# Nicholasli1995/SNVC

Hardware: AMD Instinct MI355X
Metric: stereo-pairs/sec (cost-volume build + 3D CNN fwd) (higher is better)
Workload: dtype f32 (split f16x3 operands, fp32 accumulate)

## Files before the change

snvc_amd/csrc/conv3d_f16.hip:

```cpp
#include <type_traits>

#include "common.hpp"
#include "elementwise_internal.hpp"

namespace snvc {
namespace {

typedef _Float16 h8 __attribute__((ext_vector_type(8)));
typedef float f32x16 __attribute__((ext_vector_type(16)));
typedef float f32x4 __attribute__((ext_vector_type(4)));

__device__ const unsigned g_zero16h[4] __attribute__((aligned(16))) = {0u, 0u, 0u, 0u};

struct F16Args {
    const _Float16 *x;
    const _Float16 *wp;
    const float *scale, *bias;
    const _Float16 *res;
    _Float16 *y;
    float *y_f32;
    const _Float16 *x_lo, *res_lo;
    _Float16 *y_lo;
    const float *head;
    float *y_head;
    float head_mul;
    float res_mul;
    int *overflow;
    const _Float16 *tail_w;
    float *t_out;
    float tail_mul;
    int64_t t_bs;
    const float *res_f32;
    double *stats;
    const float *x_mul;
    int CGin;
    int Cout;
    int Din, Hin, Win;
    int Dout, Hout, Wout;
    int nd, nh, nw;
    int osd, osh, osw, offd, offh, offw;
    int pad_d, pad_h, pad_w;
    int isd, ish, iod, ioh;
    int tiles_d, tiles_h, tiles_w;
    int nchunks, flags;
    int N, cls_mode;
    int64_t cls_wstride;
    int64_t x_bs, y_bs, r_bs, yf_bs;
};


template <int KD_, int KH_, int KW_, int STRIDE_, int DIL_, int MI_, int TD_, int TH_, int KCG_, int MODE_, bool DB_, int OCC_,
          int DILW_ = DIL_, int PL_ = 1, bool DYN_ = false>
struct F16Cfg {
    static constexpr bool DYN = DYN_;
    static constexpr int PL = PL_;
    static constexpr bool SPLIT = PL_ >= 2, SERIAL = PL_ == 3;
    static constexpr int RES_PL = PL_ == 2 ? 2 : 1;
    static constexpr int PASSES = SERIAL ? 2 : 1;
    static constexpr int PF = DYN_ ? 2 : (SPLIT ? 3 : 6);
    static constexpr int KD = KD_, KH = KH_, KW = KW_, STRIDE = STRIDE_, DIL = DIL_, DILW = DILW_, MI = MI_, TD = TD_, TH = TH_;
    static constexpr int KCG = KCG_, MODE = MODE_, OCC = OCC_;
    static constexpr bool DB = DB_;
    static constexpr int IN_D = (TD - 1) * STRIDE + (KD - 1) * DIL + 1;
    static constexpr int IN_H = (TH - 1) * STRIDE + (KH - 1) * DIL + 1;
    static constexpr int IN_W = 31 * STRIDE + (KW - 1) * DILW + 1;
    static constexpr int VOX = IN_D * IN_H * IN_W;
    static constexpr int GB = VOX * 16;
    static constexpr int ITEMS = RES_PL * KCG * VOX;
    static constexpr int PLANE_BYTES = KCG * GB;
    static constexpr int NIT = (ITEMS + 255) / 256;
    static constexpr int IMG_BYTES = NIT * 256 * 16;
    static constexpr int LDS_BYTES = IMG_BYTES * (DB ? 2 : 1);
    static constexpr int NB = TD * TH / 4;
    static constexpr bool UNROLL_D = KD <= 3;
    static constexpr int SEGS = UNROLL_D ? 1 : KD;
    static constexpr int TSEG = UNROLL_D ? KD * KH * KW : KH * KW;
    static constexpr int NPS = (TSEG + 1) / 2;
    static constexpr int NS = MODE == 0 ? TSEG * (KCG / 2) : NPS * KCG;
    static constexpr int STEPS = SEGS * NS;
    static constexpr int SEG_BYTES = DIL * IN_H * IN_W * 16;
    static_assert(TD * TH % 4 == 0, "rows split over 4 waves");
    static_assert(MODE == 1 || KCG % 2 == 0, "MODE 0 pairs channel groups");
    static_assert(NIT <= 32, "validity mask is one register");
    static_assert((TD * TH / 4) * 4 == TD * TH, "whole rows per wave");
    static constexpr int tapoff(int t) {
        const int kd = UNROLL_D ? t / (KH * KW) : 0, kh = (t / KW) % KH, kw = t % KW;
        return ((kd * DIL) * IN_H + kh * DIL) * IN_W + kw * DILW;
    }
};

__host__ __device__ constexpr int f16_row_channel(int i) { return 16 * ((i >> 2) & 1) + 4 * (i >> 3) + (i & 3); }

__device__ __forceinline__ int xcd_remap16(int b, int n) {
    const int q = n >> 3, r = n & 7, xcd = b & 7, k = b >> 3;
    const int base = xcd < r ? xcd * (q + 1) : r * (q + 1) + (xcd - r) * q;
    return base + k;
}

template <class Cfg, int EPI>
__global__ void __launch_bounds__(256, Cfg::OCC)
conv3d_f16_kernel(const F16Args a_) {
    F16Args a = a_;
    int cls = blockIdx.z / a.N;
    int tile_raw = blockIdx.x, tiles_launch = a.tiles_d * a.tiles_h * a.tiles_w;
    if (a.cls_mode == 1) {
        tiles_launch *= 2;
        tile_raw = xcd_remap16(blockIdx.x, tiles_launch);
        cls = (cls << 1) | (tile_raw & 1);
        tile_raw >>= 1;
        a.offd = (cls >> 2) & 1; a.offh = (cls >> 1) & 1; a.offw = cls & 1;
        a.wp += cls * a.cls_wstride;
    } else if (a.cls_mode == 2) {
        const int pd = (cls >> 1) & 1, ph = cls & 1;
        a.offd = a.iod = pd; a.offh = a.ioh = ph;
        a.nd = (a.Dout - pd + 1) / 2; a.nh = (a.Hout - ph + 1) / 2;
    }
    constexpr int S = Cfg::STRIDE, MI = Cfg::MI, TD = Cfg::TD, TH = Cfg::TH, NB = Cfg::NB, KCG = Cfg::KCG;
    constexpr int IN_H = Cfg::IN_H, IN_W = Cfg::IN_W, VOX = Cfg::VOX, GB = Cfg::GB, NIT = Cfg::NIT, ITEMS = Cfg::ITEMS;
    constexpr int PF = Cfg::PF, PL = Cfg::PL;
    constexpr bool SPLIT = Cfg::SPLIT, SERIAL = Cfg::SERIAL;
    extern __shared__ __attribute__((aligned(16))) char lds[];

    const int tid = threadIdx.x, lane = tid & 63, wave = tid >> 6, half = lane >> 5;
    const int ntiles = a.tiles_d * a.tiles_h * a.tiles_w;
    const int t = a.cls_mode == 1 ? tile_raw : xcd_remap16(blockIdx.x, ntiles);
    const int tw = t % a.tiles_w, th = (t / a.tiles_w) % a.tiles_h, td = t / (a.tiles_w * a.tiles_h);
    const int cb = blockIdx.y;
    const int64_t n = blockIdx.z % a.N;
    const int od0 = td * TD, oh0 = th * TH, ow0 = tw * 32;
    if (od0 >= a.nd || oh0 >= a.nh) return;
    const int id0 = od0 * S - a.pad_d, ih0 = oh0 * S - a.pad_h, iw0 = ow0 * S - a.pad_w;

    f32x16 acc[NB][MI];
#pragma unroll
    for (int nb = 0; nb < NB; ++nb)
#pragma unroll
        for (int m = 0; m < MI; ++m)
#pragma unroll
            for (int r = 0; r < 16; ++r) acc[nb][m][r] = 0.0f;

    const int in_hw = a.Hin * a.Win, in_dhw = in_hw * a.Din;
    unsigned off[NIT];
    unsigned vmask = 0, gmask = 0, pmask = 0;
#pragma unroll
    for (int it = 0; it < NIT; ++it) {
        const int i = it * 256 + tid;
        const int pg = i / VOX, r = i - pg * VOX;
        const int plane = pg / KCG, g = pg - plane * KCG;
        gmask |= (unsigned)(g & 1) << it;
        pmask |= (unsigned)(plane & 1) << it;
        const int dd = r / (IN_H * IN_W), r2 = r - dd * (IN_H * IN_W);
        const int hh = r2 / IN_W, ww = r2 - hh * IN_W;
        const int gd = (id0 + dd) * a.isd + a.iod, gh = (ih0 + hh) * a.ish + a.ioh, gw = iw0 + ww;
        const bool ok = i < ITEMS && (unsigned)gd < (unsigned)a.Din && (unsigned)gh < (unsigned)a.Hin &&
                        (unsigned)gw < (unsigned)a.Win;
        off[it] = ok ? (unsigned)(g * in_dhw + gd * in_hw + gh * a.Win + gw) : 0u;
        vmask |= (ok ? 1u : 0u) << it;
    }
    static_assert(KCG <= 2, "gmask holds one bit per piece");
    const _Float16 *xn = a.x + n * a.x_bs, *xn_lo = SPLIT ? a.x_lo + n * a.x_bs : nullptr;
    const int wbase = tid & ~63;
    auto issue = [&](int pass, int buf) {
        const int chunk = SERIAL ? pass >> 1 : pass;
        const bool lo_pass = SERIAL && (pass & 1);
        const int64_t coff = (int64_t)chunk * KCG * in_dhw * 8;
        const int cg_left = a.CGin - chunk * KCG;
        char *const ibuf = lds + buf * Cfg::IMG_BYTES;
#pragma unroll
        for (int it = 0; it < NIT; ++it) {
            const int i = it * 256 + tid;
            const bool ok = ((vmask >> it) & 1u) && (KCG == 1 || (int)((gmask >> it) & 1u) < cg_left);
            const _Float16 *xc = (((PL == 2 && ((pmask >> it) & 1u)) || lo_pass) ? xn_lo : xn) + coff;
            const void *src = ok ? static_cast<const void *>(xc + (size_t)off[it] * 8) : static_cast<const void *>(g_zero16h);
            if (ITEMS % 256 == 0 || i < ITEMS)
                __builtin_amdgcn_global_load_lds(static_cast<const float *>(src),
                                                 reinterpret_cast<float *>(ibuf + (it * 256 + wbase) * 16), 16, 0, 0);
        }
    };

    const int lanebase = (lane & 31) * S * 16;
    int rowoff[NB];
#pragma unroll
    for (int nb = 0; nb < NB; ++nb) {
        const int row = wave * NB + nb;
        rowoff[nb] = ((row / TH) * S * IN_H + (row % TH) * S) * IN_W * 16;
    }
    constexpr int D_SAME = Cfg::DILW;
    constexpr int D_ROW = Cfg::DIL * IN_W - (Cfg::KW - 1) * Cfg::DILW;
    constexpr int D_SLICE = Cfg::DIL * IN_H * IN_W - (Cfg::KH - 1) * Cfg::DIL * IN_W - (Cfg::KW - 1) * Cfg::DILW;
    const int b_grp = lanebase + half * GB;
    const int b_same = lanebase + half * D_SAME * 16;
    const int b_row = lanebase + half * D_ROW * 16;
    const int b_slice = lanebase + half * D_SLICE * 16;
    const int b_none = lanebase;

    constexpr int MA = MI * (SPLIT ? 2 : 1);
    int dyn_np = 0, dyn_toff[4] = {0, 0, 0, 0}, dyn_base[4] = {0, 0, 0, 0};
    if constexpr (Cfg::DYN) {
        const int nw = 1 + (cls & 1), nh = 1 + ((cls >> 1) & 1), ndp = 1 + ((cls >> 2) & 1);
        const int T = nw * nh * ndp;
// ... 238 lines not shown
                    }
                    tacc = __builtin_amdgcn_mfma_f32_32x32x16_f16(tw[m][j][1], o, tacc, 0, 0, 0);
                    tacc = __builtin_amdgcn_mfma_f32_32x32x16_f16(tw[m][j][0], ol, tacc, 0, 0, 0);
                    tacc = __builtin_amdgcn_mfma_f32_32x32x16_f16(tw[m][j][0], o, tacc, 0, 0, 0);
                }
            }
            if (okv[nb]) {
                const int64_t spc = ((int64_t)pd * a.nh + ph) * a.nw + pw_;
#pragma unroll
                for (int r = 0; r < 16; ++r) {
                    const int tap = (r & 3) + 8 * (r >> 2) + 4 * half;
                    if (tap < 27) tn[(int64_t)tap * 8 * cls_vox + spc] = tacc[r] * a.tail_mul;
                }
            }
        }
        if (vmax >= kHalfMax && a.overflow) atomicOr(a.overflow, 1);
    } else {
        const _Float16 *rn = a.res ? a.res + n * a.r_bs : nullptr;
        const _Float16 *rn_lo = (SPLIT && a.res) ? a.res_lo + n * a.r_bs : nullptr;
        constexpr bool C8OUT = EPI == 0 || EPI == 3, side = EPI == 3 && SPLIT && MI == 1;
        _Float16 *yn = C8OUT ? a.y + n * a.y_bs : nullptr;
        _Float16 *yn_lo = (C8OUT && SPLIT) ? a.y_lo + n * a.y_bs : nullptr;
        float *yf = EPI == 2 ? a.y_f32 + n * a.yf_bs : nullptr;
        const float *__restrict__ rf = (EPI == 2 && a.res_f32) ? a.res_f32 + n * a.yf_bs : nullptr;
        constexpr float kHalfMax = 65504.0f;
        const float lo_bound = relu ? 0.0f : -kHalfMax;
        float vmax = 0.0f;
        const bool want_stats = EPI == 2 && a.stats != nullptr;
        const float x_inv = (EPI == 2 && a.x_mul) ? 1.0f / a.x_mul[0] : 1.0f;
        auto run = [&](auto has_res_tag) {
            constexpr bool HAS_RES = decltype(has_res_tag)::value;
#pragma unroll
            for (int m = 0; m < MI; ++m) {
                if ((cb * MI + m) * 32 >= a.Cout) break;
                const int c0 = (cb * MI + m) * 32 + 16 * half;
                float hsum[NB];
#pragma unroll
                for (int nb = 0; nb < NB; ++nb) hsum[nb] = 0.0f;
                float st_s[2][8], st_q[2][8];
                if constexpr (EPI == 2) {
#pragma unroll
                    for (int j = 0; j < 2; ++j)
#pragma unroll
                        for (int e = 0; e < 8; ++e) st_s[j][e] = st_q[j][e] = 0.0f;
                }
#pragma unroll
                for (int j = 0; j < 2; ++j) {
                    const int cj = c0 + 8 * j;
                    f32x4 sc[2], bi[2], hw4[2];
#pragma unroll
                    for (int k = 0; k < 2; ++k) {
                        sc[k] = (a.scale ? *reinterpret_cast<const f32x4 *>(a.scale + cj + 4 * k) : f32x4(1.0f)) * x_inv;
                        bi[k] = a.scale ? *reinterpret_cast<const f32x4 *>(a.bias + cj + 4 * k) : f32x4(0.0f);
                        if constexpr (side) hw4[k] = *reinterpret_cast<const f32x4 *>(a.head + cj + 4 * k);
                    }
                    const int64_t gj = (int64_t)(cj >> 3) * out_dhw;
#pragma unroll
                    for (int nb = 0; nb < NB; ++nb) {
                        h8 rv = h8((_Float16)0.0f), rl = h8((_Float16)0.0f);
                        if constexpr (HAS_RES) {
                            rv = *reinterpret_cast<const h8 *>(rn + (gj + sp[nb]) * 8);
                            if (rn_lo) rl = *reinterpret_cast<const h8 *>(rn_lo + (gj + sp[nb]) * 8);
                        }
                        h8 o, ol;
                        float rfv[8];
                        if constexpr (EPI == 2) {
                            if (rf && okv[nb]) {
#pragma unroll
                                for (int e = 0; e < 8; ++e) rfv[e] = rf[(int64_t)(cj + e) * out_dhw + sp[nb]];
                            }
                        }
#pragma unroll
                        for (int e = 0; e < 8; ++e) {
                            float v = __builtin_fmaf(acc[nb][m][8 * j + e], sc[e >> 2][e & 3], bi[e >> 2][e & 3]);
                            if constexpr (HAS_RES) {
                                const float rr = ((float)rv[e] + (float)rl[e]) * a.res_mul;
                                if (add_pre) v += rr;
                                if (relu) v = __builtin_fmaxf(v, 0.0f);
                                if (add_post) v += rr;
                            }
                            if constexpr (EPI == 2) {
                                if constexpr (!HAS_RES) { if (relu) v = __builtin_fmaxf(v, 0.0f); }
                                if (okv[nb]) {
                                    const int64_t at = (int64_t)(cj + e) * out_dhw + sp[nb];
                                    yf[at] = rf ? __builtin_fmaf(v, a.head_mul, rfv[e]) : v * a.head_mul;
                                    if (want_stats) {
                                        const float sv = v * a.head_mul;
                                        st_s[j][e] += sv;
                                        st_q[j][e] = __builtin_fmaf(sv, sv, st_q[j][e]);
                                    }
                                }
                            } else {
                                if constexpr (SPLIT) {
                                    v = __builtin_amdgcn_fmed3f(v, HAS_RES ? -kHalfMax : lo_bound, kHalfMax);
                                    vmax = __builtin_fmaxf(vmax, okv[nb] ? __builtin_fabsf(v) : 0.0f);
                                } else if constexpr (!HAS_RES) {
                                    if (relu) v = __builtin_fmaxf(v, 0.0f);
                                }
                                if constexpr (side) hsum[nb] += hw4[e >> 2][e & 3] * v;
                                o[e] = (_Float16)v;
                                if constexpr (SPLIT) ol[e] = (_Float16)(v - (float)o[e]);
                            }
                        }
                        if constexpr (C8OUT) {
                            if (okv[nb]) {
                                *reinterpret_cast<h8 *>(yn + (gj + sp[nb]) * 8) = o;
                                if constexpr (SPLIT) *reinterpret_cast<h8 *>(yn_lo + (gj + sp[nb]) * 8) = ol;
                            }
                        }
                    }
                }
                if constexpr (EPI == 2) {
                    if (want_stats) {
                        const int zc = blockIdx.z / a.N, groups = (a.Cout + 31) >> 5;
                        const int64_t slots = (int64_t)(gridDim.z / a.N) * gridDim.x * 4;
                        const int64_t slot = ((int64_t)zc * gridDim.x + blockIdx.x) * 4 + wave;
                        double *dst = a.stats + ((((int64_t)n * slots + slot) * groups + (cb * MI + m)) * 32 + 16 * half) * 2;
#pragma unroll
                        for (int j = 0; j < 2; ++j)
#pragma unroll
                            for (int e = 0; e < 8; ++e) {
                                float s0 = st_s[j][e], s1 = st_q[j][e];
#pragma unroll
                                for (int o = 16; o >= 1; o >>= 1) {
                                    s0 += __shfl_xor(s0, o, 64);
                                    s1 += __shfl_xor(s1, o, 64);
                                }
                                if ((lane & 31) == 0) {
                                    dst[(8 * j + e) * 2] = (double)s0;
                                    dst[(8 * j + e) * 2 + 1] = (double)s1;
                                }
                            }
                    }
                }
                if constexpr (side) {
#pragma unroll
                    for (int nb = 0; nb < NB; ++nb) {
                        const float tot = hsum[nb] + __shfl_xor(hsum[nb], 32, 64);
                        if (okv[nb] && half == 0) a.y_head[n * out_dhw + sp[nb]] = tot * a.head_mul;
                    }
                }
            }
        };
        if (rn) run(std::true_type{});
        else run(std::false_type{});
        const bool clamped = vmax >= kHalfMax;
        if constexpr (C8OUT && SPLIT) {
            if (clamped && a.overflow) atomicOr(a.overflow, 1);
        }
    }
}

typedef float f32x4q __attribute__((ext_vector_type(4)));

struct X3QCfg {
    static constexpr int TD = 4, TH = 4, NB = 4, IN_D = 6, IN_H = 6, IN_W = 34, VOX = IN_D * IN_H * IN_W, GB = VOX * 16;
    static constexpr int ITEMS = 2 * VOX, PLANE_BYTES = GB, NIT = (ITEMS + 255) / 256;
    static constexpr int IMG_BYTES = NIT * 256 * 16, LDS_BYTES = 2 * IMG_BYTES;
    static constexpr int NQ = 7, PF = 2, FILL_STEP = NQ - PF;
};

template <int IMM>
__device__ __forceinline__ void lds_read_b128_to(h8 &v, unsigned addr) {
    asm volatile("ds_read_b128 %0, %1 offset:%2" : "=v"(v) : "v"(addr), "n"(IMM) : "memory");
}

template <int N>
__device__ __forceinline__ void wait_lgkm_for(h8 (&b)[8]) {
    asm volatile("s_waitcnt lgkmcnt(%8)"
                 : "+v"(b[0]), "+v"(b[1]), "+v"(b[2]), "+v"(b[3]), "+v"(b[4]), "+v"(b[5]), "+v"(b[6]), "+v"(b[7])
                 : "n"(N)
                 : "memory");
}

template <int EPI>
__global__ void __launch_bounds__(256, 2)
conv3d_x3q_kernel(const F16Args a) {
    using Cfg = X3QCfg;
    constexpr int NB = Cfg::NB, TH = Cfg::TH, IN_H = Cfg::IN_H, IN_W = Cfg::IN_W, VOX = Cfg::VOX, NIT = Cfg::NIT, NQ = Cfg::NQ;
    constexpr int ITEMS = Cfg::ITEMS, PF = Cfg::PF;
    extern __shared__ __attribute__((aligned(16))) char lds[];
    const int tid = threadIdx.x, lane = tid & 63, wave = tid >> 6, kb = lane >> 4, col = lane & 15;
    const int ntiles = a.tiles_d * a.tiles_h * a.tiles_w, cblocks = a.Cout >> 5;
    const int job = xcd_remap16(blockIdx.x, ntiles * cblocks);
    const int t = job / cblocks, cb = job - t * cblocks;
    const int tw = t % a.tiles_w, th = (t / a.tiles_w) % a.tiles_h, td = t / (a.tiles_w * a.tiles_h);
    const int64_t n = blockIdx.z;
    const int od0 = td * Cfg::TD, oh0 = th * TH, ow0 = tw * 32;
    const int id0 = od0 - a.pad_d, ih0 = oh0 - a.pad_h, iw0 = ow0 - a.pad_w;

    f32x4q acc[NB][2][2];
#pragma unroll
    for (int nb = 0; nb < NB; ++nb)
#pragma unroll
        for (int ph = 0; ph < 2; ++ph)
#pragma unroll
            for (int h = 0; h < 2; ++h) acc[nb][ph][h] = f32x4q{0.0f, 0.0f, 0.0f, 0.0f};

    const int in_hw = a.Hin * a.Win, in_dhw = in_hw * a.Din;
    unsigned off[NIT];
    unsigned vmask = 0, pmask = 0;
#pragma unroll
    for (int it = 0; it < NIT; ++it) {
        const int i = it * 256 + tid;
        const int plane = i / VOX, r = i - plane * VOX;
        pmask |= (unsigned)(plane & 1) << it;
        const int dd = r / (IN_H * IN_W), r2 = r - dd * (IN_H * IN_W);
        const int hh = r2 / IN_W, ww = r2 - hh * IN_W;
        const int gd = id0 + dd, gh = ih0 + hh, gw = iw0 + ww;
        const bool ok = i < ITEMS && (unsigned)gd < (unsigned)a.Din && (unsigned)gh < (unsigned)a.Hin && (unsigned)gw < (unsigned)a.Win;
        off[it] = ok ? (unsigned)(gd * in_hw + gh * a.Win + gw) : 0u;
        vmask |= (ok ? 1u : 0u) << it;
    }
    const _Float16 *xn = a.x + n * a.x_bs, *xn_lo = a.x_lo + n * a.x_bs;
    const int wbase = tid & ~63;
    auto issue = [&](int chunk, int buf) {
        const int64_t coff = (int64_t)chunk * in_dhw * 8;
        char *const ibuf = lds + buf * Cfg::IMG_BYTES;
#pragma unroll
        for (int it = 0; it < NIT; ++it) {
            const _Float16 *xc = (((pmask >> it) & 1u) ? xn_lo : xn) + coff;
            const void *src = ((vmask >> it) & 1u) ? static_cast<const void *>(xc + (size_t)off[it] * 8) : static_cast<const void *>(g_zero16h);
            __builtin_amdgcn_global_load_lds(static_cast<const float *>(src), reinterpret_cast<float *>(ibuf + (it * 256 + wbase) * 16), 16, 0, 0);
        }
    };
    int qoff[NQ];
#pragma unroll
    for (int q = 0; q < NQ; ++q) {
        int tp = 4 * q + kb;
        tp = tp < 27 ? tp : 26;
        qoff[q] = (((tp / 9) * IN_H + (tp / 3) % 3) * IN_W + tp % 3 + col) * 16;
    }
    int rowoff[NB];
#pragma unroll
    for (int nb = 0; nb < NB; ++nb) {
        const int row = wave * NB + nb;
        rowoff[nb] = ((row / TH) * IN_H + (row % TH)) * IN_W * 16;
    }
    const int64_t steps_total = (int64_t)a.nchunks * NQ;
    const h8 *wq = reinterpret_cast<const h8 *>(a.wp) + ((int64_t)cb * steps_total * 4) * 64 + lane;
    const int c0 = cb * 32 + 8 * kb;
    const bool has_aff = a.scale != nullptr;
    h8 q_[PF][4];
#pragma unroll
    for (int i = 0; i < PF; ++i) {
#pragma unroll
        for (int m = 0; m < 4; ++m) q_[i][m] = wq[m * 64];
        wq += 4 * 64;
    }

    const unsigned lds_base = (unsigned)(uintptr_t)(__attribute__((address_space(3))) char *)lds;
    issue(0, 0);
    __syncthreads();
    h8 epc[6];
    auto run_chunk = [&](const int chunk, auto last_tag) {
        constexpr bool LAST = decltype(last_tag)::value;
        const unsigned img = lds_base + (unsigned)((chunk & 1) * Cfg::IMG_BYTES);
        h8 bfr[2][8];
        auto load_b = [&](int buf, int hs) {
#pragma unroll
            for (int rr = 0; rr < 2; ++rr) {
                const unsigned addr = img + (unsigned)(qoff[hs >> 1] + rowoff[2 * (hs & 1) + rr]);
                lds_read_b128_to<0>(bfr[buf][rr * 4 + 0], addr);
                lds_read_b128_to<Cfg::PLANE_BYTES>(bfr[buf][rr * 4 + 1], addr);
                lds_read_b128_to<256>(bfr[buf][rr * 4 + 2], addr);
                lds_read_b128_to<Cfg::PLANE_BYTES + 256>(bfr[buf][rr * 4 + 3], addr);
            }
        };
        load_b(0, 0);
        h8 af[4];
#pragma unroll
        for (int hs = 0; hs < 2 * NQ; ++hs) {
            const int cur = hs & 1, nx = cur ^ 1;
            if ((hs & 1) == 0) {
                if (hs == 2 * Cfg::FILL_STEP) {
#pragma unroll
                    for (int i = 0; i < PF; ++i) asm volatile("" ::"v"(q_[i][0]), "v"(q_[i][1]), "v"(q_[i][2]), "v"(q_[i][3]));
                    if constexpr (!LAST) issue(chunk + 1, (chunk + 1) & 1);
                }
#pragma unroll
                for (int m = 0; m < 4; ++m) af[m] = q_[0][m];
#pragma unroll
                for (int i = 0; i + 1 < PF; ++i)
#pragma unroll
                    for (int m = 0; m < 4; ++m) q_[i][m] = q_[i + 1][m];
                if constexpr (!LAST) {
#pragma unroll
                    for (int m = 0; m < 4; ++m) q_[PF - 1][m] = wq[m * 64];
                    wq += 4 * 64;
                } else if (hs < 2 * Cfg::FILL_STEP) {
#pragma unroll
                    for (int m = 0; m < 4; ++m) q_[PF - 1][m] = wq[m * 64];
                    wq += 4 * 64;
                } else if (hs == 2 * Cfg::FILL_STEP) {
                    if (has_aff) {
#pragma unroll
                        for (int k = 0; k < 2; ++k) {
                            epc[k] = *reinterpret_cast<const h8 *>(a.scale + c0 + 4 * k);
                            epc[2 + k] = *reinterpret_cast<const h8 *>(a.bias + c0 + 4 * k);
                        }
                    }
                    if constexpr (EPI == 3) {
#pragma unroll
                        for (int k = 0; k < 2; ++k) epc[4 + k] = *reinterpret_cast<const h8 *>(a.head + c0 + 4 * k);
                    }
                }
            }
            if (hs + 1 < 2 * NQ) {
                load_b(nx, hs + 1);
                wait_lgkm_for<8>(bfr[cur]);
            } else {
                wait_lgkm_for<0>(bfr[cur]);
            }
            __builtin_amdgcn_sched_barrier(0);
#pragma unroll
            for (int term = 0; term < 3; ++term)
#pragma unroll
                for (int rr = 0; rr < 2; ++rr)
#pragma unroll
                    for (int ph = 0; ph < 2; ++ph)
#pragma unroll
                        for (int h = 0; h < 2; ++h) {
                            const h8 aw = term == 0 ? af[2 * h + 1] : af[2 * h];
                            const h8 bx = bfr[cur][rr * 4 + ph * 2 + (term == 1 ? 1 : 0)];
                            acc[2 * (hs & 1) + rr][ph][h] =
                                __builtin_amdgcn_mfma_f32_16x16x32_f16(aw, bx, acc[2 * (hs & 1) + rr][ph][h], 0, 0, 0);
                        }
            __builtin_amdgcn_sched_barrier(0);
        }
        __syncthreads();
    };
    for (int chunk = 0; chunk + 1 < a.nchunks; ++chunk) run_chunk(chunk, std::false_type{});
    run_chunk(a.nchunks - 1, std::true_type{});
    if (has_aff) asm volatile("" ::"v"(epc[0]), "v"(epc[1]), "v"(epc[2]), "v"(epc[3]));
    if constexpr (EPI == 3) asm volatile("" ::"v"(epc[4]), "v"(epc[5]));

    const int out_hw = a.Hout * a.Wout;
    const int64_t out_dhw = (int64_t)out_hw * a.Dout;
    const bool relu = (a.flags & SNVC_EPI_RELU) != 0;
    float sc[8], bi[8], hw8[8];
    const float x_inv = (EPI == 2 && a.x_mul) ? 1.0f / a.x_mul[0] : 1.0f;
#pragma unroll
    for (int e = 0; e < 8; ++e) {
        sc[e] = (has_aff ? __builtin_bit_cast(f32x4q, epc[e >> 2])[e & 3] : 1.0f) * x_inv;
        bi[e] = has_aff ? __builtin_bit_cast(f32x4q, epc[2 + (e >> 2)])[e & 3] : 0.0f;
        hw8[e] = (EPI == 3) ? __builtin_bit_cast(f32x4q, epc[4 + (e >> 2)])[e & 3] : 0.0f;
    }
    if constexpr (EPI == 2) {
        float *yf = a.y_f32 + n * a.yf_bs + (int64_t)c0 * out_dhw;
        const float *__restrict__ rf = a.res_f32 ? a.res_f32 + n * a.yf_bs + (int64_t)c0 * out_dhw : nullptr;
        const bool want_stats = a.stats != nullptr;
        float st_s[8], st_q[8];
#pragma unroll
        for (int e = 0; e < 8; ++e) st_s[e] = st_q[e] = 0.0f;
#pragma unroll
        for (int nb = 0; nb < NB; ++nb) {
            const int row = wave * NB + nb;
            const int pd = od0 + row / TH, phh = oh0 + row % TH;
#pragma unroll
            for (int ph = 0; ph < 2; ++ph) {
                const int pw = ow0 + 16 * ph + col;
                const bool ok = pd < a.nd && phh < a.nh && pw < a.nw;
                const int64_t sp = ok ? ((int64_t)pd * out_hw + phh * a.Wout + pw) : 0;
                float rfv[8];
                if (rf && ok) {
#pragma unroll
                    for (int e = 0; e < 8; ++e) rfv[e] = rf[(int64_t)e * out_dhw + sp];
                }
#pragma unroll
                for (int e = 0; e < 8; ++e) {
                    float v = __builtin_fmaf(acc[nb][ph][e >> 2][e & 3], sc[e], bi[e]);
                    if (relu) v = __builtin_fmaxf(v, 0.0f);
                    const float sv = v * a.head_mul;
                    if (ok) {
                        yf[(int64_t)e * out_dhw + sp] = rf ? sv + rfv[e] : sv;
                        if (want_stats) {
                            st_s[e] += sv;
                            st_q[e] = __builtin_fmaf(sv, sv, st_q[e]);
                        }
                    }
                }
            }
        }
        if (want_stats) {
            const int groups = a.Cout >> 5;
            double *dst = a.stats + ((((int64_t)n * ntiles * 4 + (int64_t)t * 4 + wave) * groups + cb) * 32 + 8 * kb) * 2;
#pragma unroll
            for (int e = 0; e < 8; ++e) {
                float s0 = st_s[e], s1 = st_q[e];
#pragma unroll
                for (int o = 8; o >= 1; o >>= 1) {
                    s0 += __shfl_xor(s0, o, 64);
                    s1 += __shfl_xor(s1, o, 64);
                }
                if (col == 0) {
                    dst[e * 2] = (double)s0;
                    dst[e * 2 + 1] = (double)s1;
                }
            }
        }
        return;
    }
    _Float16 *yn = a.y + n * a.y_bs + (int64_t)(cb * 4 + kb) * out_dhw * 8;
    _Float16 *yn_lo = a.y_lo + n * a.y_bs + (int64_t)(cb * 4 + kb) * out_dhw * 8;
    constexpr float kHalfMax = 65504.0f;
    const float lo_bound = relu ? 0.0f : -kHalfMax;
    float vmax = 0.0f;
#pragma unroll
    for (int nb = 0; nb < NB; ++nb) {
        const int row = wave * NB + nb;
        const int pd = od0 + row / TH, phh = oh0 + row % TH;
#pragma unroll
        for (int ph = 0; ph < 2; ++ph) {
            const int pw = ow0 + 16 * ph + col;
            const bool ok = pd < a.nd && phh < a.nh && pw < a.nw;
            const int64_t sp = ok ? ((int64_t)pd * out_hw + phh * a.Wout + pw) : 0;
            h8 o, ol;
            float hsum = 0.0f;
#pragma unroll
            for (int e = 0; e < 8; ++e) {
                float v = __builtin_fmaf(acc[nb][ph][e >> 2][e & 3], sc[e], bi[e]);
                v = __builtin_amdgcn_fmed3f(v, lo_bound, kHalfMax);
                vmax = __builtin_fmaxf(vmax, ok ? __builtin_fabsf(v) : 0.0f);
                if constexpr (EPI == 3) hsum += hw8[e] * v;
                o[e] = (_Float16)v;
                ol[e] = (_Float16)(v - (float)o[e]);
            }
            if (ok) {
                *reinterpret_cast<h8 *>(yn + sp * 8) = o;
                *reinterpret_cast<h8 *>(yn_lo + sp * 8) = ol;
            }
            if constexpr (EPI == 3) {
                float tot = hsum + __shfl_xor(hsum, 16, 64);
                tot += __shfl_xor(tot, 32, 64);
                if (ok && kb == 0) a.y_head[n * out_dhw + sp] = tot * a.head_mul;
            }
        }
    }
    if (vmax >= kHalfMax && a.overflow) atomicOr(a.overflow, 1);
}

template <int KH_, int KW_>
struct X2QCfg {
    static constexpr int KH = KH_, KW = KW_, TH = 16, NB = 4, IN_H = TH + KH - 1, IN_W = 32 + KW - 1, VOX = IN_H * IN_W, GB = VOX * 16;
    static constexpr int ITEMS = 2 * VOX, PLANE_BYTES = GB, NIT = (ITEMS + 255) / 256;
    static constexpr int IMG_BYTES = NIT * 256 * 16, LDS_BYTES = 2 * IMG_BYTES;
    static constexpr int TAPS = KH * KW, NQ = (TAPS + 3) / 4, PF = 2, FILL_STEP = NQ - PF;
    static_assert(NQ > PF, "the refill is issued PF k-steps before the chunk ends");
};

template <class Cfg>
__global__ void __launch_bounds__(256, 2)
conv2d_x3q_kernel(const F16Args a) {
    constexpr int NB = Cfg::NB, IN_W = Cfg::IN_W, VOX = Cfg::VOX, NIT = Cfg::NIT, NQ = Cfg::NQ;
    constexpr int ITEMS = Cfg::ITEMS, PF = Cfg::PF;
    extern __shared__ __attribute__((aligned(16))) char lds[];
    const int tid = threadIdx.x, lane = tid & 63, wave = tid >> 6, kb = lane >> 4, col = lane & 15;
    const int ntiles = a.tiles_h * a.tiles_w, cblocks = a.Cout >> 5;
    const int job = xcd_remap16(blockIdx.x, ntiles * cblocks);
    const int t = job / cblocks, cb = job - t * cblocks;
    const int tw = t % a.tiles_w, th = t / a.tiles_w;
    const int64_t n = blockIdx.z;
    const int oh0 = th * Cfg::TH, ow0 = tw * 32;
    const int ih0 = oh0 - a.pad_h, iw0 = ow0 - a.pad_w;

    f32x4q acc[NB][2][2];
#pragma unroll
    for (int nb = 0; nb < NB; ++nb)
#pragma unroll
        for (int ph = 0; ph < 2; ++ph)
#pragma unroll
            for (int h = 0; h < 2; ++h) acc[nb][ph][h] = f32x4q{0.0f, 0.0f, 0.0f, 0.0f};

    const int in_hw = a.Hin * a.Win;
    unsigned off[NIT];
    unsigned vmask = 0, pmask = 0;
#pragma unroll
    for (int it = 0; it < NIT; ++it) {
        const int i = it * 256 + tid;
        const int plane = i / VOX, r = i - plane * VOX;
        pmask |= (unsigned)(plane & 1) << it;
        const int hh = r / IN_W, ww = r - hh * IN_W;
        const int gh = ih0 + hh, gw = iw0 + ww;
        const bool ok = i < ITEMS && (unsigned)gh < (unsigned)a.Hin && (unsigned)gw < (unsigned)a.Win;
        off[it] = ok ? (unsigned)(gh * a.Win + gw) : 0u;
        vmask |= (ok ? 1u : 0u) << it;
    }
    const _Float16 *xn = a.x + n * a.x_bs, *xn_lo = a.x_lo + n * a.x_bs;
    const int wbase = tid & ~63;
    auto issue = [&](int chunk, int buf) {
        const int64_t coff = (int64_t)chunk * in_hw * 8;
        char *const ibuf = lds + buf * Cfg::IMG_BYTES;
#pragma unroll
        for (int it = 0; it < NIT; ++it) {
            const _Float16 *xc = (((pmask >> it) & 1u) ? xn_lo : xn) + coff;
            const void *src = ((vmask >> it) & 1u) ? static_cast<const void *>(xc + (size_t)off[it] * 8) : static_cast<const void *>(g_zero16h);
            __builtin_amdgcn_global_load_lds(static_cast<const float *>(src), reinterpret_cast<float *>(ibuf + (it * 256 + wbase) * 16), 16, 0, 0);
        }
    };
    int qoff[NQ];
#pragma unroll
    for (int q = 0; q < NQ; ++q) {
        int tp = 4 * q + kb;
        tp = tp < Cfg::TAPS ? tp : Cfg::TAPS - 1;
        qoff[q] = ((tp / Cfg::KW) * IN_W + tp % Cfg::KW + col) * 16;
    }
    int rowoff[NB];
#pragma unroll
    for (int nb = 0; nb < NB; ++nb) rowoff[nb] = (wave * NB + nb) * IN_W * 16;
    const int64_t steps_total = (int64_t)a.nchunks * NQ;
    const h8 *wq = reinterpret_cast<const h8 *>(a.wp) + ((int64_t)cb * steps_total * 4) * 64 + lane;
    h8 q_[PF][4];
#pragma unroll
    for (int i = 0; i < PF; ++i) {
#pragma unroll
        for (int m = 0; m < 4; ++m) q_[i][m] = wq[m * 64];
        wq += 4 * 64;
    }

    const unsigned lds_base = (unsigned)(uintptr_t)(__attribute__((address_space(3))) char *)lds;
    issue(0, 0);
    __syncthreads();
    for (int chunk = 0; chunk < a.nchunks; ++chunk) {
        const unsigned img = lds_base + (unsigned)((chunk & 1) * Cfg::IMG_BYTES);
        const bool more = chunk + 1 < a.nchunks;
        h8 bfr[2][8];
        auto load_b = [&](int buf, int hs) {
#pragma unroll
            for (int rr = 0; rr < 2; ++rr) {
                const unsigned addr = img + (unsigned)(qoff[hs >> 1] + rowoff[2 * (hs & 1) + rr]);
                lds_read_b128_to<0>(bfr[buf][rr * 4 + 0], addr);
                lds_read_b128_to<Cfg::PLANE_BYTES>(bfr[buf][rr * 4 + 1], addr);
                lds_read_b128_to<256>(bfr[buf][rr * 4 + 2], addr);
                lds_read_b128_to<Cfg::PLANE_BYTES + 256>(bfr[buf][rr * 4 + 3], addr);
            }
        };
        load_b(0, 0);
        h8 af[4];
#pragma unroll
        for (int hs = 0; hs < 2 * NQ; ++hs) {
            const int cur = hs & 1, nx = cur ^ 1;
            if ((hs & 1) == 0) {
                if (hs == 2 * Cfg::FILL_STEP) {
#pragma unroll
                    for (int i = 0; i < PF; ++i) asm volatile("" ::"v"(q_[i][0]), "v"(q_[i][1]), "v"(q_[i][2]), "v"(q_[i][3]));
                    if (more) issue(chunk + 1, (chunk + 1) & 1);
                }
#pragma unroll
                for (int m = 0; m < 4; ++m) af[m] = q_[0][m];
#pragma unroll
                for (int i = 0; i + 1 < PF; ++i)
#pragma unroll
                    for (int m = 0; m < 4; ++m) q_[i][m] = q_[i + 1][m];
#pragma unroll
                for (int m = 0; m < 4; ++m) q_[PF - 1][m] = wq[m * 64];
                wq += 4 * 64;
            }
            if (hs + 1 < 2 * NQ) {
                load_b(nx, hs + 1);
                wait_lgkm_for<8>(bfr[cur]);
            } else {
                wait_lgkm_for<0>(bfr[cur]);
            }
            __builtin_amdgcn_sched_barrier(0);
#pragma unroll
            for (int term = 0; term < 3; ++term)
#pragma unroll
                for (int rr = 0; rr < 2; ++rr)
#pragma unroll
                    for (int ph = 0; ph < 2; ++ph)
#pragma unroll
                        for (int h = 0; h < 2; ++h) {
                            const h8 aw = term == 0 ? af[2 * h + 1] : af[2 * h];
                            const h8 bx = bfr[cur][rr * 4 + ph * 2 + (term == 1 ? 1 : 0)];
                            acc[2 * (hs & 1) + rr][ph][h] =
                                __builtin_amdgcn_mfma_f32_16x16x32_f16(aw, bx, acc[2 * (hs & 1) + rr][ph][h], 0, 0, 0);
                        }
            __builtin_amdgcn_sched_barrier(0);
        }
        __syncthreads();
    }

    const int64_t out_hw = (int64_t)a.Hout * a.Wout;
    const bool relu = (a.flags & SNVC_EPI_RELU) != 0;
    const int c0 = cb * 32 + 8 * kb;
    const float xm = a.x_mul ? a.head_mul / a.x_mul[0] : a.head_mul;
    float sc[8], bi[8];
#pragma unroll
    for (int e = 0; e < 8; ++e) {
        sc[e] = (a.scale ? a.scale[c0 + e] : 1.0f) * xm;
        bi[e] = a.scale ? a.bias[c0 + e] : 0.0f;
    }
    float *yn = a.y_f32 + n * a.yf_bs + (int64_t)c0 * out_hw;
#pragma unroll
    for (int nb = 0; nb < NB; ++nb) {
        const int phh = oh0 + wave * NB + nb;
#pragma unroll
        for (int ph = 0; ph < 2; ++ph) {
            const int pw = ow0 + 16 * ph + col;
            if (phh < a.nh && pw < a.nw) {
                float *yp = yn + (int64_t)phh * a.Wout + pw;
#pragma unroll
                for (int e = 0; e < 8; ++e) {
                    float v = __builtin_fmaf(acc[nb][ph][e >> 2][e & 3], sc[e], bi[e]);
                    if (relu) v = __builtin_fmaxf(v, 0.0f);
                    yp[e * out_hw] = v;
                }
            }
        }
    }
}

struct X3S2Cfg {
    static constexpr int TD = 2, TH = 4, NB = 2, IN_D = 5, IN_H = 9, IN_W = 65, VOX = IN_D * IN_H * IN_W;
    static constexpr int THREADS = 512, NIT = (VOX + THREADS - 1) / THREADS, SLOT_BYTES = NIT * THREADS * 16, LDS_BYTES = 3 * SLOT_BYTES;
    static constexpr int NQ = 7;
};

template <int N>
__device__ __forceinline__ void wait_lgkm_for4(h8 (&b)[4]) {
    asm volatile("s_waitcnt lgkmcnt(%4)" : "+v"(b[0]), "+v"(b[1]), "+v"(b[2]), "+v"(b[3]) : "n"(N) : "memory");
}

__global__ void __launch_bounds__(512, 1)
conv3d_x3s2q_kernel(const F16Args a, const int total_jobs) {
    using Cfg = X3S2Cfg;
    constexpr int NB = Cfg::NB, TH = Cfg::TH, IN_H = Cfg::IN_H, IN_W = Cfg::IN_W, VOX = Cfg::VOX, NIT = Cfg::NIT, NQ = Cfg::NQ;
    extern __shared__ __attribute__((aligned(16))) char lds[];
    const int tid = threadIdx.x, lane = tid & 63, wave = (tid >> 6) & 3, chalf = tid >> 8, kb = lane >> 4, col = lane & 15;
    const int ntiles = a.tiles_d * a.tiles_h * a.tiles_w, cblocks = a.Cout >> 6;
    const int in_hw = a.Hin * a.Win, in_dhw = in_hw * a.Din;
    const int wbase = tid & ~63;

    struct Job { int od0, oh0, ow0, cb; int64_t n; };
    auto decode = [&](int b) {
        const int j = xcd_remap16(b, total_jobs);
        const int cb = j % cblocks, r = j / cblocks, t = r % ntiles;
        Job jb;
        jb.n = r / ntiles; jb.cb = cb;
        const int tw = t % a.tiles_w, th = (t / a.tiles_w) % a.tiles_h, td = t / (a.tiles_w * a.tiles_h);
        jb.od0 = td * Cfg::TD; jb.oh0 = th * TH; jb.ow0 = tw * 32;
        return jb;
    };
    unsigned off[NIT];
    unsigned vmask = 0;
    auto geometry = [&](const Job &jb) {
        const int id0 = 2 * jb.od0 - a.pad_d, ih0 = 2 * jb.oh0 - a.pad_h, iw0 = 2 * jb.ow0 - a.pad_w;
        vmask = 0;
        int tid_ = tid;
        asm volatile("" : "+v"(tid_));
#pragma unroll
        for (int it = 0; it < NIT; ++it) {
            const int i = it * 512 + tid_;
            const int dd = i / (IN_H * IN_W), r2 = i - dd * (IN_H * IN_W);
            const int hh = r2 / IN_W, pp = r2 - hh * IN_W;
            const int blk = pp >> 5, rr_ = pp & 31;
            const int ww = pp == 64 ? 64 : (rr_ < 16 ? 2 * (16 * blk + rr_) : 2 * (16 * blk + rr_ - 16) + 1);
            const int gd = id0 + dd, gh = ih0 + hh, gw = iw0 + ww;
            const bool ok = i < VOX && (unsigned)gd < (unsigned)a.Din && (unsigned)gh < (unsigned)a.Hin && (unsigned)gw < (unsigned)a.Win;
            off[it] = ok ? (unsigned)(gd * in_hw + gh * a.Win + gw) : 0u;
            vmask |= (ok ? 1u : 0u) << it;
        }
    };
    auto issue = [&](int64_t n, int chunk, bool lo_plane, int slot) {
        const _Float16 *xc = (lo_plane ? a.x_lo : a.x) + n * a.x_bs + (int64_t)chunk * in_dhw * 8;
        char *const ibuf = lds + slot * Cfg::SLOT_BYTES;
#pragma unroll
        for (int it = 0; it < NIT; ++it) {
            const void *src = ((vmask >> it) & 1u) ? static_cast<const void *>(xc + (size_t)off[it] * 8) : static_cast<const void *>(g_zero16h);
            __builtin_amdgcn_global_load_lds(static_cast<const float *>(src), reinterpret_cast<float *>(ibuf + (it * 512 + wbase) * 16), 16, 0, 0);
        }
    };
    int qoff[NQ];
#pragma unroll
    for (int q = 0; q < NQ; ++q) {
        int tp = 4 * q + kb;
        tp = tp < 27 ? tp : 26;
        const int kd = tp / 9, kh = (tp / 3) % 3, kw = tp % 3;
        const int pos = kw == 0 ? col : (kw == 1 ? 16 + col : (col == 15 ? 32 : col + 1));
        qoff[q] = ((kd * IN_H + kh) * IN_W + pos) * 16;
    }
    int rowoff[NB];
#pragma unroll
    for (int nb = 0; nb < NB; ++nb) {
        const int row = wave * NB + nb;
        rowoff[nb] = ((2 * (row / TH)) * IN_H + 2 * (row % TH)) * IN_W * 16;
    }
    const h8 *const wall = reinterpret_cast<const h8 *>(a.wp);
    const int64_t wchunk = (int64_t)NQ * 8 * 64;

    int b = blockIdx.x;
    Job cur = decode(b);
    geometry(cur);
    h8 WH[NQ][2], WL[NQ][2];
    {
        const h8 *wc = wall + (int64_t)cur.cb * a.nchunks * wchunk;
#pragma unroll
        for (int q = 0; q < NQ; ++q)
#pragma unroll
            for (int h = 0; h < 2; ++h) {
                WH[q][h] = wc[(q * 8 + (2 * chalf + h) * 2) * 64 + lane];
                WL[q][h] = wc[(q * 8 + (2 * chalf + h) * 2 + 1) * 64 + lane];
            }
    }
    f32x4q acc[NB][2][2];
#pragma unroll
    for (int nb = 0; nb < NB; ++nb)
#pragma unroll
        for (int ph = 0; ph < 2; ++ph)
#pragma unroll
            for (int h = 0; h < 2; ++h) acc[nb][ph][h] = f32x4q{0.0f, 0.0f, 0.0f, 0.0f};

    const unsigned lds_base = (unsigned)(uintptr_t)(__attribute__((address_space(3))) char *)lds;
    int s_hi = 0, s_sp = 2;
    issue(cur.n, 0, false, 0);
    issue(cur.n, 0, true, 1);
    __syncthreads();
    const int gstride = gridDim.x;
    constexpr float kHalfMax = 65504.0f;
    const bool has_aff = a.scale != nullptr;
    float vmax = 0.0f;
    int chunk = 0;
    while (true) {
        const bool last_chunk = chunk + 1 == a.nchunks;
        const bool next_job = last_chunk && b + gstride < total_jobs;
        const bool more = !last_chunk || next_job;
        Job nxt = cur;
        if (next_job) {
            nxt = decode(b + gstride);
            geometry(nxt);
        }
        const int nchunk = last_chunk ? 0 : chunk + 1;
        if (more) issue(nxt.n, nchunk, false, s_sp);
        h8 bfr[2][4];
        auto load_b = [&](int buf, unsigned img, int q) {
#pragma unroll
            for (int rr = 0; rr < 2; ++rr) {
                const unsigned addr = img + (unsigned)(qoff[q] + rowoff[rr]);
                lds_read_b128_to<0>(bfr[buf][rr * 2 + 0], addr);
                lds_read_b128_to<512>(bfr[buf][rr * 2 + 1], addr);
            }
        };
        {
            const unsigned img = lds_base + (unsigned)Cfg::SLOT_BYTES;
            load_b(0, img, 0);
#pragma unroll
            for (int q = 0; q < NQ; ++q) {
                const int cb_ = q & 1, nx = cb_ ^ 1;
                if (q + 1 < NQ) {
                    load_b(nx, img, q + 1);
                    wait_lgkm_for4<4>(bfr[cb_]);
                } else {
                    wait_lgkm_for4<0>(bfr[cb_]);
                }
                __builtin_amdgcn_sched_barrier(0);
#pragma unroll
                for (int rr = 0; rr < 2; ++rr)
#pragma unroll
                    for (int ph = 0; ph < 2; ++ph)
// ... 754 lines not shown
            weight, reinterpret_cast<_Float16 *>(packed), d->Cout, d->Cin, 27, 1, 4 * X3S2Cfg::NQ, X3S2Cfg::NQ, p.nchunks, 4, 2, 1, wmul, p.block_halves);
        return check_launch(who);
    }
    if (p.kind == FK3XQ) {
        pack_q16s_weights_kernel<<<(unsigned)ceil_div<int64_t>(p.block_halves, 256), 256, 0, as_stream(stream)>>>(
            weight, reinterpret_cast<_Float16 *>(packed), d->Cout, d->Cin, 27, 1, 4 * X3QCfg::NQ, X3QCfg::NQ, p.nchunks, 2, 2, 1, wmul, p.block_halves);
        return check_launch(who);
    }
    for (int c = 0; c < classes; ++c) {
        PackArgs a;
        a.w = weight;
        a.out = reinterpret_cast<_Float16 *>(packed) + c * f16_class_stride(p);
        a.Cout = d->Cout; a.Cin = d->Cin; a.K = d->ksize;
        a.transposed = d->transposed; a.pd = (c >> 2) & 1; a.ph = (c >> 1) & 1; a.pw = c & 1;
        a.KD = p.KD; a.KH = p.KH; a.KW = p.KW; a.KCG = p.KCG; a.MODE = p.MODE; a.MI = p.MI; a.SEGS = p.SEGS;
        a.TSEG = p.TSEG; a.NPS = p.NPS; a.NS = p.NS; a.unroll_d = p.unroll_d;
        a.nchunks = p.nchunks; a.cblocks = p.cblocks; a.total = p.block_halves;
        a.PL = p.PL; a.PASSES = p.PASSES; a.wmul = wmul;
        a.dyn = p.dyn;
        if (p.dyn) {
            const int T = (1 + a.pd) * (1 + a.ph) * (1 + a.pw);
            a.NS = 2 * (T > 1 ? T / 2 : 1);
            a.total = (int64_t)p.cblocks * p.nchunks * a.NS * p.MI * 2 * 64 * 8;
        }
        pack_f16_weights_kernel<<<(unsigned)ceil_div<int64_t>(a.total, 256), 256, 0, as_stream(stream)>>>(a);
    }
    return check_launch(who);
}

int snvc_f16_conv3d_pack_weights(const snvc_conv3d_desc *d, const float *weight, void *packed, void *stream) {
    return f16_pack_common(d, weight, packed, false, 1.0f, stream, "snvc_f16_conv3d_pack_weights");
}

int64_t snvc_f16x3_conv3d_packed_weight_bytes(const snvc_conv3d_desc *d) {
    using namespace snvc;
    F16Plan p;
    if (!d || make_f16_plan(*d, p, true) != SNVC_OK) return -1;
    return 2 * f16_class_stride(p) * (d->transposed ? 8 : 1);
}

int snvc_f16x3_conv3d_pack_weights(const snvc_conv3d_desc *d, const float *weight, void *packed, float wmul, void *stream) {
    return f16_pack_common(d, weight, packed, true, wmul, stream, "snvc_f16x3_conv3d_pack_weights");
}

int snvc_f16_conv3d_forward(const snvc_conv3d_desc *d, const void *x, const void *packed_weight, const float *scale,
                            const float *bias, const void *residual, void *y, float *y_f32, void *stream) {
    using namespace snvc;
    F16Plan p;
    if (!d) return fail(SNVC_ERR_INVALID_ARGUMENT, "snvc_f16_conv3d_forward: null desc");
    int rc = make_f16_plan(*d, p);
    if (rc) return rc;
    if (d->N == 0) return SNVC_OK;
    const bool plane = d->Cout == 1;
    if (!x || !packed_weight || (plane ? !y_f32 : !y))
        return fail(SNVC_ERR_INVALID_ARGUMENT, "snvc_f16_conv3d_forward: null pointer");
    if ((scale == nullptr) != (bias == nullptr))
        return fail(SNVC_ERR_INVALID_ARGUMENT, "snvc_f16_conv3d_forward: scale and bias must both be given or both be NULL");
    const int resflags = d->flags & (SNVC_EPI_ADD_PRE | SNVC_EPI_ADD_POST);
    if (resflags && (!residual || plane))
        return fail(SNVC_ERR_INVALID_ARGUMENT, "snvc_f16_conv3d_forward: residual flag without a C8 residual");
    if (resflags == (SNVC_EPI_ADD_PRE | SNVC_EPI_ADD_POST))
        return fail(SNVC_ERR_INVALID_ARGUMENT, "snvc_f16_conv3d_forward: ADD_PRE and ADD_POST are exclusive");
    if (!plane && (d->flags & SNVC_EPI_SIGMOID))
        return fail(SNVC_ERR_UNSUPPORTED, "snvc_f16_conv3d_forward: Sigmoid is built for the one-channel fp32 output only");
    const int64_t in_sp = (int64_t)d->Din * d->Hin * d->Win, out_sp = (int64_t)d->Dout * d->Hout * d->Wout;
    if ((int64_t)(d->Cin / 8 + 2) * in_sp >= ((int64_t)1 << 31) || out_sp >= ((int64_t)1 << 31))
        return fail(SNVC_ERR_UNSUPPORTED, "snvc_f16_conv3d_forward: one sample must stay below 2^31 pieces");
    if ((reinterpret_cast<uintptr_t>(x) | reinterpret_cast<uintptr_t>(y) | reinterpret_cast<uintptr_t>(residual) |
         reinterpret_cast<uintptr_t>(packed_weight)) & 15)
        return fail(SNVC_ERR_INVALID_ARGUMENT, "snvc_f16_conv3d_forward: C8 tensors must be 16-byte aligned");
    if ((d->x_batch_stride | d->y_batch_stride | d->res_batch_stride) % 8)
        return fail(SNVC_ERR_INVALID_ARGUMENT, "snvc_f16_conv3d_forward: batch strides must be multiples of 8 elements");

    F16Args a{};
    a.x = reinterpret_cast<const _Float16 *>(x);
    a.scale = scale; a.bias = bias;
    a.res = resflags ? reinterpret_cast<const _Float16 *>(residual) : nullptr;
    a.y = reinterpret_cast<_Float16 *>(y); a.y_f32 = y_f32;
    a.res_mul = 1.0f;
    a.CGin = d->Cin / 8;
    a.Cout = d->Cout;
    a.Din = d->Din; a.Hin = d->Hin; a.Win = d->Win;
    a.Dout = d->Dout; a.Hout = d->Hout; a.Wout = d->Wout;
    a.nchunks = p.nchunks; a.flags = d->flags;
    a.x_bs = d->x_batch_stride ? d->x_batch_stride : (int64_t)d->Cin * in_sp;
    a.y_bs = d->y_batch_stride ? d->y_batch_stride : (int64_t)d->Cout * out_sp;
    a.r_bs = d->res_batch_stride ? d->res_batch_stride : (int64_t)d->Cout * out_sp;
    a.yf_bs = out_sp;
    hipStream_t st = as_stream(stream);
    const bool subgrid = p.kind == FK5D2 || p.kind == FK5D2N || p.kind == FK5D2Q || p.kind == FK5D2QN;
    const int classes = d->transposed ? 8 : (subgrid ? 4 : 1);
    a.wp = reinterpret_cast<const _Float16 *>(packed_weight);
    a.N = d->N; a.cls_mode = d->transposed ? 1 : (subgrid ? 2 : 0); a.cls_wstride = f16_class_stride(p);
    a.isd = a.ish = 1; a.iod = a.ioh = 0; a.offd = a.offh = a.offw = 0;
    if (d->transposed) {
        a.nd = d->Din; a.nh = d->Hin; a.nw = d->Win;
        a.osd = a.osh = a.osw = 2;
        a.pad_d = a.pad_h = a.pad_w = 0;
    } else if (subgrid) {
        a.nd = (d->Dout + 1) / 2; a.nh = (d->Hout + 1) / 2; a.nw = d->Wout;
        a.osd = a.osh = 2; a.osw = 1;
        a.isd = a.ish = 2;
        a.pad_d = a.pad_h = d->pad / 2; a.pad_w = d->pad;
    } else {
        a.nd = d->Dout; a.nh = d->Hout; a.nw = d->Wout;
        a.osd = a.osh = a.osw = 1;
        a.pad_d = a.pad_h = a.pad_w = d->pad;
    }
    a.tiles_d = ceil_div(a.nd, p.TD); a.tiles_h = ceil_div(a.nh, p.TH); a.tiles_w = ceil_div(a.nw, 32);
    const int64_t ntiles = (int64_t)a.tiles_d * a.tiles_h * a.tiles_w;
    if (ntiles >= ((int64_t)1 << 30) || (int64_t)d->N * classes > 65535)
        return fail(SNVC_ERR_UNSUPPORTED, "snvc_f16_conv3d_forward: too many tiles or samples");
    dim3 grid((unsigned)(d->transposed ? 2 * ntiles : ntiles), (unsigned)p.cblocks, (unsigned)(d->N * (d->transposed ? 4 : classes)));
    switch (p.kind) {
        case FK7QN: case FK5D2QN: case FK5QN: {
            using C7 = Q16SCfg<7, 1, 1, 1>; using C5D = Q16SCfg<5, 2, 1, 1>; using C5 = Q16SCfg<5, 1, 1, 1>;
            if (p.kind == FK7QN) launch_lds<conv3d_q16s_kernel<C7>>(grid, 256, C7::LDS_BYTES, st, a);
            else if (p.kind == FK5QN) launch_lds<conv3d_q16s_kernel<C5>>(grid, 256, C5::LDS_BYTES, st, a);
            else launch_lds<conv3d_q16s_kernel<C5D>>(grid, 256, C5D::LDS_BYTES, st, a);
            break;
        }
        case FK7Q: case FK5D2Q: case FK5Q: {
            if (plane) return fail(SNVC_ERR_UNSUPPORTED, "snvc_f16_conv3d_forward: the 16x16x32 form writes C8 tensors");
            using C7 = Q16SCfg<7, 1, 1, 2>; using C5D = Q16SCfg<5, 2, 1, 2>; using C5 = Q16SCfg<5, 1, 1, 2>;
            if (p.kind == FK7Q) launch_lds<conv3d_q16s_kernel<C7>>(grid, 256, C7::LDS_BYTES, st, a);
            else if (p.kind == FK5Q) launch_lds<conv3d_q16s_kernel<C5>>(grid, 256, C5::LDS_BYTES, st, a);
            else launch_lds<conv3d_q16s_kernel<C5D>>(grid, 256, C5D::LDS_BYTES, st, a);
            break;
        }
        case FK1: launch_f16<F16K1, 0>(a, grid, st); break;
        case FK3: launch_f16<F16K3, 0>(a, grid, st); break;
        case FK3H: launch_f16<F16K3H, 1>(a, grid, st); break;
        case FK3S2: launch_f16<F16K3S2, 0>(a, grid, st); break;
        case FK5: launch_f16<F16K5, 0>(a, grid, st); break;
        case FK5D2: launch_f16<F16K5D2, 0>(a, grid, st); break;
        case FK7: launch_f16<F16K7, 0>(a, grid, st); break;
        case FDC: launch_f16<F16DC, 0>(a, grid, st); break;
        case FK1N: launch_f16<F16K1N, 0>(a, grid, st); break;
        case FK3N: launch_f16<F16K3H, 0>(a, grid, st); break;
        case FK3S2N: launch_f16<F16K3S2N, 0>(a, grid, st); break;
        case FK5N: launch_f16<F16K5N, 0>(a, grid, st); break;
        case FK5D2N: launch_f16<F16K5D2N, 0>(a, grid, st); break;
        case FK7N: launch_f16<F16K7N, 0>(a, grid, st); break;
        case FDCN: launch_f16<F16DCN, 0>(a, grid, st); break;
        default: return fail(SNVC_ERR_UNSUPPORTED, "snvc_f16_conv3d_forward: no kernel");
    }
    return check_launch("snvc_f16_conv3d_forward");
}

static int f16x3_forward(const snvc_conv3d_desc *d, const void *x_hi, const void *x_lo, const void *packed_weight,
                         const float *scale, const float *bias, const void *res_hi, const void *res_lo, void *y_hi,
                         void *y_lo, float *y_f32, const float *head, float *y_head, float head_mul, float res_mul,
                         int *overflow, const void *tail_w, float *t_out, float tail_mul, void *stream, double *stats = nullptr,
                         int64_t *stats_slots = nullptr, const float *x_mul = nullptr) {
    using namespace snvc;
    F16Plan p;
    if (!d) return fail(SNVC_ERR_INVALID_ARGUMENT, "snvc_f16x3_conv3d_forward: null desc");
    int rc = make_f16_plan(*d, p, true);
    if (rc) return rc;
    if (d->N == 0) return SNVC_OK;
    const bool tail = tail_w != nullptr;
    if (tail && (!t_out || !d->transposed || p.cblocks != 1 || d->Cout != 32 * p.MI || (reinterpret_cast<uintptr_t>(tail_w) & 15)))
        return fail(SNVC_ERR_UNSUPPORTED, "snvc_f16x3_deconv3d_tail_forward: a transposed split layer whose 32 or 64 output channels sit in one block");
    const bool plane = d->Cout == 1;
    const bool to_f32 = y_f32 != nullptr;
    if (plane && !to_f32) return fail(SNVC_ERR_INVALID_ARGUMENT, "snvc_f16x3_conv3d_forward: a one-channel layer writes y_f32");
    if (!x_hi || !x_lo || !packed_weight || (!tail && !to_f32 && (!y_hi || !y_lo)))
        return fail(SNVC_ERR_INVALID_ARGUMENT, "snvc_f16x3_conv3d_forward: null pointer");
    if ((scale == nullptr) != (bias == nullptr))
        return fail(SNVC_ERR_INVALID_ARGUMENT, "snvc_f16x3_conv3d_forward: scale and bias must both be given or both be NULL");
    int resflags = d->flags & (SNVC_EPI_ADD_PRE | SNVC_EPI_ADD_POST);
    const float *res_f32 = nullptr;
    if (resflags == SNVC_EPI_ADD_POST && to_f32 && !plane && res_hi && !res_lo && !tail_w) {
        if (d->res_batch_stride && d->res_batch_stride != (d->y_batch_stride ? d->y_batch_stride : (int64_t)d->Cout * d->Dout * d->Hout * d->Wout))
            return fail(SNVC_ERR_INVALID_ARGUMENT, "snvc_f16x3_conv3d_forward: a float32 residual shares the result's batch stride");
        res_f32 = reinterpret_cast<const float *>(res_hi);
        res_hi = nullptr;
        resflags = 0;
    }
    if (resflags && (!res_hi || !res_lo || plane))
        return fail(SNVC_ERR_INVALID_ARGUMENT, "snvc_f16x3_conv3d_forward: residual flag without a split residual");
    if (resflags == (SNVC_EPI_ADD_PRE | SNVC_EPI_ADD_POST))
        return fail(SNVC_ERR_INVALID_ARGUMENT, "snvc_f16x3_conv3d_forward: ADD_PRE and ADD_POST are exclusive");
    if (d->flags & ~(SNVC_EPI_RELU | SNVC_EPI_ADD_PRE | SNVC_EPI_ADD_POST | (plane ? SNVC_EPI_SIGMOID : 0)))
        return fail(SNVC_ERR_UNSUPPORTED, "snvc_f16x3_conv3d_forward: RELU / ADD_PRE / ADD_POST only (SIGMOID with the one-channel output)");
    if ((head != nullptr) != (y_head != nullptr))
        return fail(SNVC_ERR_INVALID_ARGUMENT, "snvc_f16x3_conv3d_forward: head and y_head go together");
    if (head && ((p.kind != FK3X && p.kind != FK3XS && p.kind != FK3XT && p.kind != FK3XQ) || d->Cout != 32 || to_f32))
        return fail(SNVC_ERR_UNSUPPORTED, "snvc_f16x3_conv3d_forward: the side head is built for 32-channel stride-1 layers with a split output");
    const int64_t in_sp = (int64_t)d->Din * d->Hin * d->Win, out_sp = (int64_t)d->Dout * d->Hout * d->Wout;
    if ((int64_t)(d->Cin / 8 + 2) * in_sp >= ((int64_t)1 << 31) || out_sp >= ((int64_t)1 << 31))
        return fail(SNVC_ERR_UNSUPPORTED, "snvc_f16x3_conv3d_forward: one sample must stay below 2^31 pieces");
    if ((reinterpret_cast<uintptr_t>(x_hi) | reinterpret_cast<uintptr_t>(x_lo) | reinterpret_cast<uintptr_t>(y_hi) |
         reinterpret_cast<uintptr_t>(y_lo) | reinterpret_cast<uintptr_t>(res_hi) | reinterpret_cast<uintptr_t>(res_lo) |
         reinterpret_cast<uintptr_t>(packed_weight) | reinterpret_cast<uintptr_t>(scale) | reinterpret_cast<uintptr_t>(bias) |
         reinterpret_cast<uintptr_t>(head)) & 15)
        return fail(SNVC_ERR_INVALID_ARGUMENT, "snvc_f16x3_conv3d_forward: C8 tensors and the per-channel vectors must be 16-byte aligned");
    if ((d->x_batch_stride | (res_f32 ? 0 : d->res_batch_stride)) % 8 || (!to_f32 && d->y_batch_stride % 8))
        return fail(SNVC_ERR_INVALID_ARGUMENT, "snvc_f16x3_conv3d_forward: batch strides must be multiples of 8 elements");
    F16Args a{};
    a.x = reinterpret_cast<const _Float16 *>(x_hi); a.x_lo = reinterpret_cast<const _Float16 *>(x_lo);
    a.scale = scale; a.bias = bias;
    a.res = resflags ? reinterpret_cast<const _Float16 *>(res_hi) : nullptr;
    a.res_lo = resflags ? reinterpret_cast<const _Float16 *>(res_lo) : nullptr;
    a.y = reinterpret_cast<_Float16 *>(y_hi); a.y_lo = reinterpret_cast<_Float16 *>(y_lo); a.y_f32 = y_f32;
    a.head = head; a.y_head = y_head; a.head_mul = head_mul; a.res_mul = res_mul; a.overflow = overflow;
    a.res_f32 = res_f32;
    a.stats = stats;
    a.x_mul = to_f32 ? x_mul : nullptr;
    a.tail_w = reinterpret_cast<const _Float16 *>(tail_w); a.t_out = t_out; a.tail_mul = tail_mul;
    a.t_bs = (int64_t)27 * 8 * d->Din * d->Hin * d->Win;
    a.CGin = d->Cin / 8; a.Cout = d->Cout;
    a.Din = d->Din; a.Hin = d->Hin; a.Win = d->Win;
    a.Dout = d->Dout; a.Hout = d->Hout; a.Wout = d->Wout;
    a.nchunks = p.nchunks; a.flags = res_f32 ? (d->flags & ~SNVC_EPI_ADD_POST) : d->flags;
    a.x_bs = d->x_batch_stride ? d->x_batch_stride : 2 * (int64_t)d->Cin * in_sp;
    a.y_bs = d->y_batch_stride ? d->y_batch_stride : 2 * (int64_t)d->Cout * out_sp;
    a.r_bs = d->res_batch_stride ? d->res_batch_stride : 2 * (int64_t)d->Cout * out_sp;
    a.yf_bs = plane ? out_sp : (d->y_batch_stride ? d->y_batch_stride : (int64_t)d->Cout * out_sp);
    a.wp = reinterpret_cast<const _Float16 *>(packed_weight);
    const bool subgrid = p.kind == FK5D2X || p.kind == FK5D2XQ;
    const int classes = d->transposed ? 8 : (subgrid ? 4 : 1);
    a.N = d->N; a.cls_mode = d->transposed ? 1 : (subgrid ? 2 : 0); a.cls_wstride = f16_class_stride(p);
    a.isd = a.ish = 1; a.iod = a.ioh = 0; a.offd = a.offh = a.offw = 0;
    if (d->transposed) {
        a.nd = d->Din; a.nh = d->Hin; a.nw = d->Win;
        a.osd = a.osh = a.osw = 2;
        a.pad_d = a.pad_h = a.pad_w = 0;
    } else if (subgrid) {
        a.nd = (d->Dout + 1) / 2; a.nh = (d->Hout + 1) / 2; a.nw = d->Wout;
        a.osd = a.osh = 2; a.osw = 1;
        a.isd = a.ish = 2;
        a.pad_d = a.pad_h = d->pad / 2; a.pad_w = d->pad;
    } else {
        a.nd = d->Dout; a.nh = d->Hout; a.nw = d->Wout;
        a.osd = a.osh = a.osw = 1;
        a.pad_d = a.pad_h = a.pad_w = d->pad;
    }
    a.tiles_d = ceil_div(a.nd, p.TD); a.tiles_h = ceil_div(a.nh, p.TH); a.tiles_w = ceil_div(a.nw, 32);
    const int64_t ntiles = (int64_t)a.tiles_d * a.tiles_h * a.tiles_w;
    if (ntiles >= ((int64_t)1 << 30) || (int64_t)d->N * classes > 65535)
        return fail(SNVC_ERR_UNSUPPORTED, "snvc_f16x3_conv3d_forward: too many tiles or samples");
    dim3 grid((unsigned)(d->transposed ? 2 * ntiles : ntiles), (unsigned)p.cblocks, (unsigned)(d->N * (d->transposed ? 4 : classes)));
    hipStream_t st = as_stream(stream);
    if (stats_slots) {
        const bool form_ok = to_f32 && !plane && !tail && (p.kind == FK3XQ || p.kind == FK3X || p.kind == FK3X2 || p.kind == FK3XS || p.kind == FK3X2S || p.kind == FK3XT ||
                                                            p.kind == FK3S2X || p.kind == FK3S2XT || p.kind == FDCX || p.kind == FDCXT || p.kind == FDCXN);
        if (!form_ok) return fail(SNVC_ERR_UNSUPPORTED, "snvc_f16x3_conv3d_forward_stats: this layer's kernel form has no statistics epilogue");
        *stats_slots = p.kind == FK3XQ ? ntiles * 4 : (int64_t)(grid.z / d->N) * grid.x * 4;
        if (!stats) return fail(SNVC_ERR_INVALID_ARGUMENT, "snvc_f16x3_conv3d_forward_stats: null workspace");
        if (classes > 1) {
            const hipError_t e = hipMemsetAsync(stats, 0, (size_t)d->N * *stats_slots * ((d->Cout + 31) / 32) * 64 * sizeof(double), st);
            if (e != hipSuccess) return fail(SNVC_ERR_HIP, "snvc_f16x3_conv3d_forward_stats: hipMemsetAsync failed");
        }
    }
#define SNVC_X3_LAUNCH(CFG) do { if (to_f32) launch_f16<CFG, 2>(a, grid, st); else launch_f16<CFG, 0>(a, grid, st); } while (0)
    switch (p.kind) {
        case FK3X:
            if (to_f32) launch_f16<F16K3X, 2>(a, grid, st);
            else if (head) launch_f16<F16K3X, 3>(a, grid, st);
            else launch_f16<F16K3X, 0>(a, grid, st);
            break;
        case FK3X2: SNVC_X3_LAUNCH(F16K3X2); break;
        case FK3XS:
            if (to_f32) launch_f16<F16K3XS, 2>(a, grid, st);
            else if (head) launch_f16<F16K3XS, 3>(a, grid, st);
            else launch_f16<F16K3XS, 0>(a, grid, st);
            break;
        case FK3X2S: SNVC_X3_LAUNCH(F16K3X2S); break;
        case FK3XT:
            if (to_f32) launch_f16<F16K3XT, 2>(a, grid, st);
            else if (head) launch_f16<F16K3XT, 3>(a, grid, st);
            else launch_f16<F16K3XT, 0>(a, grid, st);
            break;
        case FK3S2X: SNVC_X3_LAUNCH(F16K3S2X); break;
        case FK3S2XT: SNVC_X3_LAUNCH(F16K3S2XT); break;
        case FDCX: if (tail) launch_f16<F16DCX, 4>(a, grid, st); else SNVC_X3_LAUNCH(F16DCX); break;
        case FDCXT: if (tail) launch_f16<F16DCXT, 4>(a, grid, st); else SNVC_X3_LAUNCH(F16DCXT); break;
        case FDCXN: if (tail) launch_f16<F16DCXN, 4>(a, grid, st); else SNVC_X3_LAUNCH(F16DCXN); break;
        case FK1X: SNVC_X3_LAUNCH(F16K1X); break;
        case FK5X: SNVC_X3_LAUNCH(F16K5X); break;
        case FK5D2X: SNVC_X3_LAUNCH(F16K5D2X); break;
        case FK7X: SNVC_X3_LAUNCH(F16K7X); break;
        case FK3XH: launch_f16<F16K3X, 1>(a, grid, st); break;
        case FK5XQ: case FK5D2XQ: case FK7XQ: {
            if (to_f32 || head) return fail(SNVC_ERR_UNSUPPORTED, "snvc_f16x3_conv3d_forward: the 16x16x32 form writes a split C8 tensor, no side head");
            using C5 = Q16SCfg<5, 1>; using C5D = Q16SCfg<5, 2>; using C7 = Q16SCfg<7, 1>;
            if (p.kind == FK5XQ) launch_lds<conv3d_q16s_kernel<C5>>(grid, 256, C5::LDS_BYTES, st, a);
            else if (p.kind == FK5D2XQ) launch_lds<conv3d_q16s_kernel<C5D>>(grid, 256, C5D::LDS_BYTES, st, a);
            else launch_lds<conv3d_q16s_kernel<C7>>(grid, 256, C7::LDS_BYTES, st, a);
            break;
        }
        case FK3S2XQ: {
            if (to_f32 || resflags || head) return fail(SNVC_ERR_UNSUPPORTED, "snvc_f16x3_conv3d_forward: the stride-2 16x16x32 form writes a split C8 tensor, no residual / head");
            const int64_t total = ntiles * p.cblocks * d->N;
            if (total >= ((int64_t)1 << 30)) return fail(SNVC_ERR_UNSUPPORTED, "snvc_f16x3_conv3d_forward: too many tiles");
            int g = device_cu_count();
            if (g <= 0) g = 256;
            if (total < g) g = total >= 8 ? (int)(total & ~(int64_t)7) : (int)total;
            launch_lds<conv3d_x3s2q_kernel>(dim3((unsigned)g), X3S2Cfg::THREADS, X3S2Cfg::LDS_BYTES, st, a, (int)total);
            break;
        }
        case FK3XQ: {
            if (resflags || (to_f32 && head)) return fail(SNVC_ERR_UNSUPPORTED, "snvc_f16x3_conv3d_forward: the 16x16x32 form has no split residual, no side head beside a float32 result");
            if (ntiles * p.cblocks >= ((int64_t)1 << 30)) return fail(SNVC_ERR_UNSUPPORTED, "snvc_f16x3_conv3d_forward: too many tiles");
            grid = dim3((unsigned)(ntiles * p.cblocks), 1, (unsigned)d->N);
            if (to_f32) launch_lds<conv3d_x3q_kernel<2>>(grid, 256, X3QCfg::LDS_BYTES, st, a);
            else if (head) launch_lds<conv3d_x3q_kernel<3>>(grid, 256, X3QCfg::LDS_BYTES, st, a);
            else launch_lds<conv3d_x3q_kernel<0>>(grid, 256, X3QCfg::LDS_BYTES, st, a);
            break;
        }
        default: return fail(SNVC_ERR_UNSUPPORTED, "snvc_f16x3_conv3d_forward: no kernel");
    }
#undef SNVC_X3_LAUNCH
    return check_launch("snvc_f16x3_conv3d_forward");
}

int snvc_f16x3_conv3d_forward(const snvc_conv3d_desc *d, const void *x_hi, const void *x_lo, const void *packed_weight,
                              const float *scale, const float *bias, const void *res_hi, const void *res_lo, void *y_hi,
                              void *y_lo, float *y_f32, const float *head, float *y_head, float head_mul, float res_mul,
                              int *overflow, void *stream) {
    return f16x3_forward(d, x_hi, x_lo, packed_weight, scale, bias, res_hi, res_lo, y_hi, y_lo, y_f32, head, y_head, head_mul, res_mul,
                         overflow, nullptr, nullptr, 0.0f, stream);
}

static int64_t f16x3_stats_slots(const snvc_conv3d_desc &d, const snvc::F16Plan &p) {
    using namespace snvc;
    const bool subgrid = p.kind == FK5D2X || p.kind == FK5D2XQ;
    int nd, nh, nw;
    if (d.transposed) { nd = d.Din; nh = d.Hin; nw = d.Win; }
    else if (subgrid) { nd = (d.Dout + 1) / 2; nh = (d.Hout + 1) / 2; nw = d.Wout; }
    else { nd = d.Dout; nh = d.Hout; nw = d.Wout; }
    const int64_t ntiles = (int64_t)ceil_div(nd, p.TD) * ceil_div(nh, p.TH) * ceil_div(nw, 32);
    if (p.kind == FK3XQ) return ntiles * 4;
    return (d.transposed ? 4 * 2 * ntiles : (subgrid ? 4 : 1) * ntiles) * 4;
}

int64_t snvc_f16x3_conv3d_stats_workspace_bytes(const snvc_conv3d_desc *d) {
    using namespace snvc;
    F16Plan p;
    if (!d || d->N < 0 || make_f16_plan(*d, p, true)) return -1;
    const int64_t groups = (d->Cout + 31) / 32;
    const int64_t slots = f16x3_stats_slots(*d, p);
    return (d->N * slots * groups * 64 + conv_stats_fold_scratch_doubles(d->N, (int)groups, slots) + d->N * (int64_t)d->Cout * 2) * (int64_t)sizeof(double);
}

int snvc_f16x3_conv3d_forward_f32(const snvc_conv3d_desc *d, const void *x_hi, const void *x_lo, const void *packed_weight,
                                  const float *scale, const float *bias, const float *x_mul, const float *res_f32, float *y_f32,
                                  float out_mul, void *stream) {
    using namespace snvc;
    if (!d || !y_f32) return fail(SNVC_ERR_INVALID_ARGUMENT, "snvc_f16x3_conv3d_forward_f32: null pointer");
    if (d->flags & (SNVC_EPI_ADD_PRE | SNVC_EPI_ADD_POST)) return fail(SNVC_ERR_INVALID_ARGUMENT, "snvc_f16x3_conv3d_forward_f32: the residual is res_f32 (added after the activation), no flag");
    snvc_conv3d_desc dd = *d;
    if (res_f32) dd.flags |= SNVC_EPI_ADD_POST;
    return f16x3_forward(&dd, x_hi, x_lo, packed_weight, scale, bias, res_f32, nullptr, nullptr, nullptr, y_f32, nullptr, nullptr, out_mul, 1.0f,
                         nullptr, nullptr, nullptr, 0.0f, stream, nullptr, nullptr, x_mul);
}

int snvc_f16x3_conv3d_forward_stats(const snvc_conv3d_desc *d, const void *x_hi, const void *x_lo, const void *packed_weight,
                                    const float *scale, const float *bias, const float *x_mul, float *y_f32, float head_mul, const float *gamma,
                                    const float *beta, float *bn_scale, float *bn_shift, float *mean, float *var, void *workspace,
                                    float eps, void *stream) {
    using namespace snvc;
    if (!d || !y_f32 || !bn_scale || !bn_shift || !workspace)
        return fail(SNVC_ERR_INVALID_ARGUMENT, "snvc_f16x3_conv3d_forward_stats: null pointer");
    if (d->N <= 0 || d->flags || d->Cout % 32) return fail(SNVC_ERR_UNSUPPORTED, "snvc_f16x3_conv3d_forward_stats: whole 32-channel groups, no epilogue flags");
    double *stats = static_cast<double *>(workspace);
    int64_t slots = 0;
    int rc = f16x3_forward(d, x_hi, x_lo, packed_weight, scale, bias, nullptr, nullptr, nullptr, nullptr, y_f32, nullptr, nullptr, head_mul, 1.0f,
                           nullptr, nullptr, nullptr, 0.0f, stream, stats, &slots, x_mul);
    if (rc) return rc;
    const int groups = d->Cout / 32;
    double *scratch = stats + d->N * slots * groups * 64;
    double *partial = scratch + conv_stats_fold_scratch_doubles(d->N, groups, slots);
    launch_conv_stats_fold(stats, scratch, partial, d->N, d->Cout, groups, slots, as_stream(stream));
    rc = check_launch("snvc_f16x3_conv3d_forward_stats(fold)");
    if (rc) return rc;
    launch_norm_finalize(partial, gamma, beta, bn_scale, bn_shift, mean, var, d->N, d->Cout, (int64_t)d->Dout * d->Hout * d->Wout, 1, eps,
                         as_stream(stream));
    return check_launch("snvc_f16x3_conv3d_forward_stats(finalize)");
}

int snvc_f16x3_split_scale(const float *x, int64_t n, void *scratch8, float *out_mul, void *stream) {
    using namespace snvc;
    if (n < 0) return fail(SNVC_ERR_INVALID_ARGUMENT, "snvc_f16x3_split_scale: negative size");
    if (!out_mul || !scratch8 || (n > 0 && !x)) return fail(SNVC_ERR_INVALID_ARGUMENT, "snvc_f16x3_split_scale: null pointer");
    if (reinterpret_cast<uintptr_t>(x) & 15) return fail(SNVC_ERR_INVALID_ARGUMENT, "snvc_f16x3_split_scale: x must be 16-byte aligned");
    int blocks = (int)ceil_div<int64_t>(n > 0 ? n : 1, 256 * 4 * 16);
    blocks = blocks < 1 ? 1 : (blocks > 48 ? 48 : blocks);
    split_scale_kernel<<<blocks, 256, 0, as_stream(stream)>>>(x, n, reinterpret_cast<unsigned *>(scratch8), out_mul);
    return check_launch("snvc_f16x3_split_scale");
}

static int x2q_nq(int kh, int kw) { return (kh * kw + 3) / 4; }

int64_t snvc_f16x3_conv2d_packed_weight_bytes(int cout, int cin, int kh, int kw) {
    if (cout <= 0 || cin <= 0 || cout % 32 || cin % 8 || kh != 3 || (kw != 3 && kw != 7)) return -1;
    return 2 * ((int64_t)(cout / 32) * (cin / 8) * x2q_nq(kh, kw) + 2) * 4 * 64 * 8;
}

int snvc_f16x3_conv2d_pack_weights(const float *weight, int cout, int cin, int kh, int kw, void *packed, float wmul, void *stream) {
    using namespace snvc;
    const int64_t bytes = snvc_f16x3_conv2d_packed_weight_bytes(cout, cin, kh, kw);
    if (bytes < 0) return fail(SNVC_ERR_UNSUPPORTED, "snvc_f16x3_conv2d: 3x7 or 3x3 kernels, Cin % 8 == 0, Cout % 32 == 0");
    if (!weight || !packed) return fail(SNVC_ERR_INVALID_ARGUMENT, "snvc_f16x3_conv2d_pack_weights: null pointer");
    if (hipMemsetAsync(packed, 0, (size_t)bytes, as_stream(stream)) != hipSuccess)
        return fail(SNVC_ERR_HIP, "snvc_f16x3_conv2d_pack_weights: hipMemsetAsync failed");
    const int nq = x2q_nq(kh, kw);
    const int64_t total = (int64_t)(cout / 32) * (cin / 8) * nq * 4 * 64 * 8;
    pack_q16s_weights_kernel<<<(unsigned)ceil_div<int64_t>(total, 256), 256, 0, as_stream(stream)>>>(
        weight, reinterpret_cast<_Float16 *>(packed), cout, cin, kh * kw, 1, 4 * nq, nq, cin / 8, 2, 2, 1, wmul, total);
    return check_launch("snvc_f16x3_conv2d_pack_weights");
}

int snvc_f16x3_conv2d_forward(const void *x_hi, const void *x_lo, const void *packed_weight, const float *scale, const float *bias,
                              float *y, int64_t N, int64_t Cin, int64_t Cout, int64_t H, int64_t W, int kh, int kw, float out_mul,
                              const float *x_mul_dev, int flags, void *stream) {
    using namespace snvc;
    if (N < 0 || H <= 0 || W <= 0 || snvc_f16x3_conv2d_packed_weight_bytes((int)Cout, (int)Cin, kh, kw) < 0)
        return fail(SNVC_ERR_UNSUPPORTED, "snvc_f16x3_conv2d_forward: 3x7 or 3x3 kernels, Cin % 8 == 0, Cout % 32 == 0");
    if (N == 0) return SNVC_OK;
    if (!x_hi || !x_lo || !packed_weight || !y) return fail(SNVC_ERR_INVALID_ARGUMENT, "snvc_f16x3_conv2d_forward: null pointer");
    if ((scale == nullptr) != (bias == nullptr))
        return fail(SNVC_ERR_INVALID_ARGUMENT, "snvc_f16x3_conv2d_forward: scale and bias must both be given or both be NULL");
    if (flags & ~SNVC_EPI_RELU) return fail(SNVC_ERR_UNSUPPORTED, "snvc_f16x3_conv2d_forward: only SNVC_EPI_RELU");
    if ((reinterpret_cast<uintptr_t>(x_hi) | reinterpret_cast<uintptr_t>(x_lo) | reinterpret_cast<uintptr_t>(packed_weight)) & 15)
        return fail(SNVC_ERR_INVALID_ARGUMENT, "snvc_f16x3_conv2d_forward: C8 tensors must be 16-byte aligned");
    const int64_t hw = H * W;
    if ((Cin / 8 + 2) * hw >= ((int64_t)1 << 31) || N > 65535) return fail(SNVC_ERR_UNSUPPORTED, "snvc_f16x3_conv2d_forward: tensor too large");
    F16Args a{};
    a.x = reinterpret_cast<const _Float16 *>(x_hi); a.x_lo = reinterpret_cast<const _Float16 *>(x_lo);
    a.wp = reinterpret_cast<const _Float16 *>(packed_weight);
    a.scale = scale; a.bias = bias; a.y_f32 = y; a.head_mul = out_mul; a.x_mul = x_mul_dev;
    a.CGin = (int)(Cin / 8); a.Cout = (int)Cout; a.nchunks = (int)(Cin / 8); a.flags = flags;
    a.Din = a.Dout = 1; a.Hin = a.Hout = (int)H; a.Win = a.Wout = (int)W;
    a.nd = 1; a.nh = (int)H; a.nw = (int)W;
    a.pad_d = 0; a.pad_h = (kh - 1) / 2; a.pad_w = (kw - 1) / 2;
    a.tiles_d = 1; a.tiles_h = (int)ceil_div<int64_t>(H, 16); a.tiles_w = (int)ceil_div<int64_t>(W, 32);
    a.x_bs = 2 * Cin * hw; a.yf_bs = Cout * hw; a.N = (int)N;
    const int64_t jobs = (int64_t)a.tiles_h * a.tiles_w * (Cout / 32);
    if (jobs >= ((int64_t)1 << 30)) return fail(SNVC_ERR_UNSUPPORTED, "snvc_f16x3_conv2d_forward: too many tiles");
    const dim3 grid((unsigned)jobs, 1, (unsigned)N);
    hipStream_t st = as_stream(stream);
    if (kw == 7) {
        using C = X2QCfg<3, 7>;
        launch_lds<conv2d_x3q_kernel<C>>(grid, 256, C::LDS_BYTES, st, a);
    } else {
        using C = X2QCfg<3, 3>;
        launch_lds<conv2d_x3q_kernel<C>>(grid, 256, C::LDS_BYTES, st, a);
    }
    return check_launch("snvc_f16x3_conv2d_forward");
}

extern "C" int snvc_sheared_upsample_split(const float *, void *, void *, const float *, int64_t, int64_t, int64_t, int64_t, int, int64_t, int, void *);
int snvc_sheared_prep_x3(const float *right, int64_t N, int64_t C, int64_t H, int64_t W, int q, int64_t WU, int off, int64_t WU2, int off2,
                         const void *packed_g, const void *packed_col, int64_t Cout3, float out_mul_g, float out_mul_col, void *rq_split,
                         void *rq2_split, void *scratch8, float *mul_dev, float *g, float *gcol, void *stream) {
    using namespace snvc;
    if (!right || !packed_g || !packed_col || !rq_split || !rq2_split || !scratch8 || !mul_dev || !g || !gcol)
        return fail(SNVC_ERR_INVALID_ARGUMENT, "snvc_sheared_prep_x3: null pointer");
    if (N <= 0 || C % 8 || Cout3 % 32) return fail(SNVC_ERR_UNSUPPORTED, "snvc_sheared_prep_x3: C % 8 == 0, 3 * Cout % 32 == 0");
    int rc = snvc_f16x3_split_scale(right, N * C * H * W, scratch8, mul_dev, stream);
    if (rc) return rc;
    const int64_t G = C / 8;
    _Float16 *a = reinterpret_cast<_Float16 *>(rq_split), *b = reinterpret_cast<_Float16 *>(rq2_split);
    rc = snvc_sheared_upsample_split(right, a, a + G * H * WU * 8, mul_dev, N, C, H, W, q, WU, off, stream);
    if (rc) return rc;
    rc = snvc_f16x3_conv2d_forward(a, a + G * H * WU * 8, packed_g, nullptr, nullptr, g, N, C, Cout3, H, WU, 3, 7, out_mul_g, mul_dev, 0, stream);
    if (rc) return rc;
    rc = snvc_sheared_upsample_split(right, b, b + G * H * WU2 * 8, mul_dev, N, C, H, W, q, WU2, off2, stream);
    if (rc) return rc;
    return snvc_f16x3_conv2d_forward(b, b + G * H * WU2 * 8, packed_col, nullptr, nullptr, gcol, N, C, Cout3, H, WU2, 3, 7, out_mul_col, mul_dev, 0,
                                     stream);
}

extern "C" int snvc_f16x3_from_ncdhw(const float *, void *, void *, int64_t, int64_t, int64_t, int64_t, int64_t, float, const float *, void *);
int snvc_f16x3_conv2d_from_f32(const float *x, int64_t N, int64_t C, int64_t H, int64_t W, int kh, int kw, int n_layers,
                               const void *const *packed, const int64_t *cout, const float *out_mul, float *const *y, void *ws_split,
                               void *scratch8, float *mul_dev, void *stream) {
    using namespace snvc;
    if (!x || !packed || !cout || !out_mul || !y || !ws_split || !scratch8 || !mul_dev || n_layers < 1 || n_layers > 8)
        return fail(SNVC_ERR_INVALID_ARGUMENT, "snvc_f16x3_conv2d_from_f32: null pointer or layer count outside 1..8");
    if (N <= 0 || C % 8) return fail(SNVC_ERR_UNSUPPORTED, "snvc_f16x3_conv2d_from_f32: C % 8 == 0");
    int rc = snvc_f16x3_split_scale(x, N * C * H * W, scratch8, mul_dev, stream);
    if (rc) return rc;
    _Float16 *a = reinterpret_cast<_Float16 *>(ws_split);
    rc = snvc_f16x3_from_ncdhw(x, a, a + C * H * W, N, C, H * W, 0, 0, 1.0f, mul_dev, stream);
    if (rc) return rc;
    for (int i = 0; i < n_layers; ++i) {
        rc = snvc_f16x3_conv2d_forward(a, a + C * H * W, packed[i], nullptr, nullptr, y[i], N, C, cout[i], H, W, kh, kw, out_mul[i], mul_dev, 0, stream);
        if (rc) return rc;
    }
    return SNVC_OK;
}

int64_t snvc_f16x3_tail_packed_weight_bytes(int cin) {
    return cin > 0 && cin % 32 == 0 ? (int64_t)(cin / 32) * 2 * 2 * 64 * 8 * 2 : -1;
}

int snvc_f16x3_tail_pack_weights(const float *weight, int cin, void *packed, float wmul, void *stream) {
    using namespace snvc;
    if (!weight || !packed || cin <= 0 || cin % 32 != 0)
        return fail(SNVC_ERR_INVALID_ARGUMENT, "snvc_f16x3_tail_pack_weights: weight [Cin][27] with Cin % 32 == 0");
    const int total = (cin / 32) * 2 * 2 * 64 * 8;
    pack_tail_weights_kernel<<<(unsigned)ceil_div(total, 256), 256, 0, as_stream(stream)>>>(weight, reinterpret_cast<_Float16 *>(packed), cin, wmul, total);
    return check_launch("snvc_f16x3_tail_pack_weights");
}

int snvc_f16x3_deconv3d_tail_forward(const snvc_conv3d_desc *d, const void *x_hi, const void *x_lo, const void *packed_weight,
                                     const float *scale, const float *bias, const void *res_hi, const void *res_lo, float res_mul,
                                     const void *tail_packed, float *t_out, float tail_mul, int *overflow, void *stream) {
    using namespace snvc;
    if (!tail_packed || !t_out) return fail(SNVC_ERR_INVALID_ARGUMENT, "snvc_f16x3_deconv3d_tail_forward: null pointer");
    return f16x3_forward(d, x_hi, x_lo, packed_weight, scale, bias, res_hi, res_lo, nullptr, nullptr, nullptr, nullptr, nullptr, 1.0f, res_mul,
                         overflow, tail_packed, t_out, tail_mul, stream);
}

int snvc_deconv_tail_gather(const float *t, const float *bias, const float *residual, float *y, int64_t n, int64_t nd, int64_t nh,
                            int64_t nw, void *stream) {
    using namespace snvc;
    if (n < 0 || nd <= 0 || nh <= 0 || nw <= 0) return fail(SNVC_ERR_INVALID_ARGUMENT, "snvc_deconv_tail_gather: sizes must be positive");
    if (n == 0) return SNVC_OK;
    if (!t || !y) return fail(SNVC_ERR_INVALID_ARGUMENT, "snvc_deconv_tail_gather: null pointer");
    if ((reinterpret_cast<uintptr_t>(y) | reinterpret_cast<uintptr_t>(residual)) & 15)
        return fail(SNVC_ERR_INVALID_ARGUMENT, "snvc_deconv_tail_gather: y / residual must be 16-byte aligned");
    const int64_t threads = 16 * nd * nh * nw, out_vox = 64 * nd * nh * nw;
    if (threads >= ((int64_t)1 << 31) * 255 || n > 65535 || 27 * 8 * nd * nh * nw >= ((int64_t)1 << 40))
        return fail(SNVC_ERR_UNSUPPORTED, "snvc_deconv_tail_gather: tensor too large");
    const dim3 grid((unsigned)ceil_div<int64_t>(threads, 256), (unsigned)n);
    deconv_tail_gather_kernel<<<grid, 256, 0, as_stream(stream)>>>(t, bias, residual, y, (int)nd, (int)nh, (int)nw, 27 * 8 * nd * nh * nw,
                                                                   out_vox, out_vox);
    return check_launch("snvc_deconv_tail_gather");
}

}
```

snvc_amd/models/stereo_volume.py:

```python
import itertools
import warnings
import weakref

import torch
import torch.nn as nn

from ..extension.build_cost_volume import _BuildCostVolume, build_cost_volume
from .. import ops
from .._derived import derived, fresh, stamp
from .submodule import (_ROUTES, SCRATCH_ATTRS, WORKSPACE_ATTRS, X3_GROUP_NORM, ConvBNReLU3d, HipConv3d, SplitModePolicy, SplitOverflow,
                        SplitT, _FactoredFirstConvFn, _ShearedFirstConvBNFn, _ShearedFirstConvFn, _folded_bn,
                        _is_channel_head as _is_head_conv, _Plan, convbn_3d, folded_head_weights, hourglass, overflow_guard, plan_for,
                        sheared_geometry, sheared_kernels, x3_exponent, x3_norm_bound, EPI_RELU, SHEAR_CLASS_KDS)

_PREP_EPOCH = itertools.count(1)


def _factored_plans(conv: nn.Module, c: int) -> dict:
    plans = conv.__dict__.get("_snvc_factored")
    if plans is None or not fresh(plans["stamp"], (conv.weight,)):
        w = conv.weight
        plans = conv.__dict__["_snvc_factored"] = {"stamp": stamp((w,)), "plan": _Plan(),
                                                   "right": ops.Conv3dLayer(w.detach()[:, c:].contiguous(), 3, 1, 1, 1, False)}
    return plans


def _mark(timing, name, which):
    if timing is not None and name in timing:
        timing[name][which].record()


def _run(gen):
    try:
        while True:
            next(gen)
    except StopIteration as done:
        return done.value


class GlobalStack(SplitModePolicy, nn.Module):
    def __init__(self, c=32, gn=False):
        super().__init__()
        self.conv1 = ConvBNReLU3d(convbn_3d(2 * c, c, 3, 1, 1, gn=gn), nn.ReLU(inplace=True))
        self.conv2 = ConvBNReLU3d(convbn_3d(c, c, 3, 1, 1, gn=gn), nn.ReLU(inplace=True))
        self.hg_conv3d = hourglass(c, gn=gn)
        self.classifier = HipConv3d(c, 1, kernel_size=1, padding=0, stride=1, bias=False)
        for m in self.modules():
            if isinstance(m, nn.Conv3d):
                nn.init.kaiming_normal_(m.weight, mode="fan_out", nonlinearity="relu")
            elif isinstance(m, nn.BatchNorm3d):
                nn.init.constant_(m.weight, 1)
                nn.init.constant_(m.bias, 0)

    def _buffer(self, name, shape, device, dtype=torch.float32):
        ws = self.__dict__.setdefault("_snvc_ws", {})
        key = (name, tuple(shape), device)
        buf = ws.get(key)
        if buf is None:
            for k in [k for k in ws if k[0] == name and k[2] == device]:
                del ws[k]
            buf = ws[key] = torch.empty(shape, dtype=dtype, device=device)
        return buf

    prep_streams = False

    def _side_streams(self, device):
        st = self.__dict__.setdefault("_snvc_streams", {})
        if device not in st:
            st[device] = (torch.cuda.Stream(device), torch.cuda.Stream(device))
        return st[device]

    def last_first_layer(self) -> torch.Tensor:
        ws = self.__dict__.get("_snvc_ws", {})
        which = self.__dict__.get("_snvc_last_v1", "v1")
        for k, v in ws.items():
            if k[0] == which:
                return ops.from_split(v, self.__dict__["_snvc_x3"]["exp"]["v1"]) if which == "v1s" else v
        raise RuntimeError("no first-layer result in the workspace")

    def release_workspace(self):
        for name in WORKSPACE_ATTRS:
            self.__dict__.pop(name, None)

    def train(self, mode: bool = True):
        if mode:
            self.release_workspace()
        return super().train(mode)

    def __getstate__(self):
        state = self.__dict__.copy()
        for name in SCRATCH_ATTRS:
            state.pop(name, None)
        return state

    arithmetic = "auto"
    stream_out = False
    split_prep = True
    fused_tail = True

    def _x3_state(self, device):
        hg = self.hg_conv3d
        seqs = {"conv2": self.conv2[0], "h1": hg.conv1[0], "h2": hg.conv2, "h3": hg.conv3[0], "h4": hg.conv4[0], "h5": hg.conv5}
        c = self.conv2[0][0].out_channels
        if c != 32 or self.conv2[0][0].in_channels != 32 or not _is_head_conv(self.classifier, c):
            return None
        norms = [self.conv1[0][1]] + [sq[1] for sq in seqs.values()]
        for nm in norms:
            if not isinstance(nm, nn.BatchNorm3d) or nm.training or nm.running_mean is None:
                return None
        tensors = [t for sq in list(seqs.values()) + [hg.conv6] for t in (sq[0].weight, sq[1].weight, sq[1].bias, sq[1].running_mean, sq[1].running_var)]
        tensors.append(self.classifier.weight)
        tensors += [self.conv1[0][1].weight, self.conv1[0][1].bias, self.conv1[0][1].running_mean, self.conv1[0][1].running_var]
        st = self.__dict__.get("_snvc_x3")
        if st is not None and fresh(st["stamp"], tensors, (device,)):
            return st
        e = {k: x3_exponent(x3_norm_bound(sq[1], plan_for(sq[0], "_x3", device))) for k, sq in [("v1", self.conv1[0])] + list(seqs.items())}
        st = {"stamp": stamp(tensors, (device,)), "exp": e, "layers": {}, "affine": {}}
        geo = {"conv2": (1, False), "h1": (2, False), "h2": (1, False), "h3": (2, False), "h4": (1, False), "h5": (2, True)}
        for k, sq in seqs.items():
            w = sq[0].weight.detach().to(device)
            st["layers"][k] = ops.Conv3dLayerX3(w, 3, geo[k][0], 1, 1, geo[k][1])
            st["affine"][k] = _folded_bn(sq[1], plan_for(sq[0], "", device))
        w5 = hg.conv5[0].weight.detach().double().abs()
        sets = ([1], [0, 2])
        l1 = None
        for pd in range(2):
            for ph in range(2):
                for pw in range(2):
                    t = w5[:, :, sets[pd]][:, :, :, sets[ph]][:, :, :, :, sets[pw]].sum(dim=(0, 2, 3, 4))
                    l1 = t if l1 is None else torch.maximum(l1, t)
        sc5, bi5 = st["affine"]["h5"]
        hard = float(((sc5.double().abs() * l1.to(sc5.device) * (65504.0 / 2.0 ** st["exp"]["h4"]) + bi5.double().abs()).max()
                      + 65504.0 / 2.0 ** st["exp"]["h2"]).item())
        st["exp"]["post"] = min(x3_exponent(hard), st["exp"]["h2"])
        st["tail"] = st["tail_bias"] = None
        if isinstance(hg.conv6[1], nn.BatchNorm3d) and not hg.conv6[1].training and hg.conv6[0].in_channels % 32 == 0:
            wf, fb = folded_head_weights(hg.conv6[0], hg.conv6[1], self.classifier)
            st["tail"] = ops.TailWeightsX3(wf.float().to(device))
            st["tail_bias"] = fb.float().reshape(1).to(device)
        st["guard"] = overflow_guard(self, device)
        st["flag"] = st["guard"].flag
        self.__dict__["_snvc_x3"] = st
        return st

    @staticmethod
    def _x3_v1_affine(st, scale, bias):
        e1 = st["exp"]["v1"]
        return derived(st, "v1_affine", (scale, bias), lambda: ((scale * 2.0 ** e1).contiguous(), (bias * 2.0 ** e1).contiguous()))

    def _x3_select(self, device, arithmetic=None):
        mode = arithmetic or self.arithmetic
        if mode == "fp32" or torch.is_grad_enabled() or self.training or self.split_off:
            if mode == "x3":
                raise RuntimeError("arithmetic='x3' needs inference (no autograd, eval mode) and no earlier overflow")
            return None
        st = self._x3_state(device)
        if st is None:
            if mode == "x3":
                raise RuntimeError("arithmetic='x3': the stack does not qualify (32 channels, eval-mode BatchNorm3d everywhere)")
            return None
        return st if self.split_guard(device, mode) is not None else None

    def _tail_x3(self, st, v1s, timing=None):
        L, A, E, flag = st["layers"], st["affine"], st["exp"], st["flag"]
        n, dev = v1s.size(0), v1s.device
        d, h, w = v1s.shape[3:6]
        hg = self.hg_conv3d
        _mark(timing, "conv2", 0)
        v2s, hv = L["conv2"](v1s, E["v1"], *A["conv2"], flags=EPI_RELU, out_exp=E["conv2"], head=self.classifier.weight, overflow=flag,
                             out=self._buffer("v2s", (n, 2, 4, d, h, w, 8), dev, torch.float16))
        _mark(timing, "conv2", 1)
        _ROUTES["side_head"] += 1
        o = L["h1"](v2s, E["conv2"], *A["h1"], flags=EPI_RELU, out_exp=E["h1"], overflow=flag)
        pre = L["h2"](o, E["h1"], *A["h2"], flags=EPI_RELU, out_exp=E["h2"], overflow=flag)
        o = L["h3"](pre, E["h2"], *A["h3"], flags=EPI_RELU, out_exp=E["h3"], overflow=flag)
        o = L["h4"](o, E["h3"], *A["h4"], flags=EPI_RELU, out_exp=E["h4"], overflow=flag)
        st["guard"].post()
        if st["tail"] is not None and self.fused_tail:
            t = L["h5"].forward_tail(o, E["h4"], *A["h5"], st["tail"], residual=pre, res_exp=E["h2"], flags=EPI_RELU | ops.EPI_ADD_PRE,
                                     out_exp=E["post"], overflow=flag, out=self._buffer("tail_t", (n, 27, 8) + tuple(o.shape[3:6]), dev))
            cost = ops.deconv_tail_gather(t, st["tail_bias"], hv)
            _ROUTES["x3_fused_tail"] += 1
        else:
            post = L["h5"](o, E["h4"], *A["h5"], residual=pre, flags=EPI_RELU | ops.EPI_ADD_PRE, out_exp=E["h2"], to_f32=True)
            cost = hg.conv6.fused(post, residual=None, head=self.classifier, head_residual=hv)
        _ROUTES["x3_tail"] += 1
        if self.overflow_check == "call" and st["guard"].wait():
            raise SplitOverflow()
        return cost

    def _tail(self, v, hv=None):
        cost, _, _ = self.hg_conv3d(v, None, None, residual=v, head=self.classifier, head_residual=hv)
        return cost

    def _gn_qualifies(self, device, arithmetic=None):
        mode = arithmetic or self.arithmetic
        norms = [m for m in self.modules() if isinstance(m, (nn.GroupNorm, nn.modules.batchnorm._BatchNorm))]
        if (not norms or not all(isinstance(m, nn.GroupNorm) for m in norms) or not X3_GROUP_NORM[0] or mode == "fp32"
                or torch.is_grad_enabled() or self.training or self.split_off or device.type != "cuda"
                or self.conv1[0][0].out_channels % 32 != 0):
            return None
        return self.split_guard(device, mode)

    def _gn_tail_x3(self, v1, timing=None, arithmetic=None):
        if isinstance(v1, SplitT):
            v1s, guard = v1, self.__dict__["_snvc_x3_guard"][v1.t.device]
        else:
            if not (v1.is_cuda and v1.dtype == torch.float32):
                return None
            guard = self._gn_qualifies(v1.device, arithmetic)
            if guard is None:
                return None
            norm1 = self.conv1[0][1]
            b1 = x3_norm_bound(norm1, plan_for(self.conv1[0][0], "_x3", v1.device))
            e1 = x3_exponent(b1)
            n, c = v1.size(0), v1.size(1)
            v1s = SplitT(ops.to_split(v1, e1, out=self._buffer("v1s", (n, 2, c // 8) + tuple(v1.shape[2:]) + (8,), v1.device, torch.float16)), e1, b1)
        _mark(timing, "conv2", 0)
        v2 = self.conv2.fused_x3(v1s, flag=guard.flag)
        _mark(timing, "conv2", 1)
        out, _, _ = self.hg_conv3d.forward_x3(v2, residual=v2, flag=guard.flag)
        guard.post()
        cost = self.classifier(ops.from_split(out.t, out.exp))
        _ROUTES["x3_gn_tail"] += 1
        if self.overflow_check == "call" and guard.wait():
            raise SplitOverflow()
        return cost

    @staticmethod
    def _sheared_geometry4(m0: int, d: int, w: int):
        off = 8
        wu = (off + 4 * (w - 1) + 1 + 5 + 5 + 3) // 4 * 4
        u_lo = 4 * (w - 1) - (d - 1) - m0 - 5
        return off, wu, 8 - u_lo, (d + 10 + 8 + 3) // 4 * 4

    @staticmethod
    def _sheared_layer4(plans, wr):
        if "sheared4" not in plans:
            w = wr.detach().double()
            cout, c = w.shape[0], w.shape[1]
            k = torch.zeros((3, 3, cout, c, 3, 3), dtype=torch.float64, device=w.device)
            for cls, kds in enumerate(SHEAR_CLASS_KDS):
                for kd in kds:
                    for kw in (-1, 0, 1):
                        k[kw + 1, cls, :, :, :, 1 - kd] += w[:, :, kd + 1, :, kw + 1]
            plans["sheared4"] = ops.Conv3dLayer(k.reshape(9 * cout, c, 3, 3).float().contiguous(), 3, 1, 1, 1, False, planar=True)
        return plans["sheared4"]

    def _sheared4_inputs(self, plans, wr, rq_src, q_up, m0, d, w):
        lay = self._sheared_layer4(plans, wr)
        off, wu, off_col, wu_col = self._sheared_geometry4(m0, d, w)
        out = []
        for width, o_, last in ((wu, off, False), (wu_col, off_col, True)):
            p = lay(ops.sheared_upsample(rq_src, q_up, width, o_).unsqueeze(2)).squeeze(2)
            n, c9, h, _ = p.shape
            p = p.view(n, 3, c9 // 3, h, width)
            g = p[:, 1].clone()
            g[..., 4:] += p[:, 0][..., :-4]
            if not last:
                g[..., :-4] += p[:, 2][..., 4:]
            out.append(g.contiguous())
        return out[0], out[1], off, off_col

    def _ds_sheared_first_layer(self, left, right, shift, ds, arithmetic=None):
        conv, bn = self.conv1[0][0], self.conv1[0][1]
        nonneg, structure = self._shift_structure(shift)
        assert nonneg
        if structure is None or structure[0] * ds not in (2, 4):
            return None
        q_up, m0 = structure
        phases = q_up * ds
        n, c = left.size(0), left.size(1)
        h, w, d = left.size(2) // ds, left.size(3) // ds, shift.size(1)
        if w % 8 or w > 512:
            return None
        if phases == 2:
            if not self._sheared_fits(2, m0, d, w, False):
                return None
        else:
            _, wu4, _, _ = self._sheared_geometry4(m0, d, w)
            if 4 * ((wu4 + 3) // 4 * 4 + 16 + d) > 150 * 1024:
                return None
        st = self._x3_select(left.device, arithmetic)
        left_s = left[:, :, ::ds, ::ds].contiguous()
        right_r = right[:, :, ::ds, :].contiguous()
        wt = conv.weight
        plans = _factored_plans(conv, c)
        scale, bias = _folded_bn(bn, plans["plan"])
        planes = self._left_planes_layer(plans, wt.detach()[:, :c])(left_s.unsqueeze(2)).view(n, c, 3, h, w)
        if phases == 2:
            lay_g, lay_col = self._sheared_layers(plans, wt.detach()[:, c:], 2)
            off, wu, off_col, wu_col = sheared_geometry(2, m0, d, w)
            g = lay_g(ops.sheared_upsample(right_r, 1, wu, off).unsqueeze(2)).squeeze(2)
            gcol = lay_col(ops.sheared_upsample(right_r, 1, wu_col, off_col).unsqueeze(2)).squeeze(2)
        else:
            g, gcol, off, off_col = self._sheared4_inputs(plans, wt.detach()[:, c:], right_r, q_up, m0, d, w)
        shape = (n, c, d, h, w)
        try:
            if st is not None:
                v1s = self._buffer("v1s", (n, 2, c // 8, d, h, w, 8), left.device, torch.float16)
                ops.sheared_expand_split(g, gcol, planes, *self._x3_v1_affine(st, scale, bias), v1s, phases, m0, off, off_col, ops.EPI_RELU,
                                         st["flag"])
                _ROUTES["ds_sheared_first_conv"] += 1
                self.__dict__["_snvc_last_v1"] = "v1s"
                return self._tail_x3(st, v1s, None)
            v = self._buffer("v1", shape, left.device)
            ops.sheared_expand(g, gcol, planes, scale, bias, v, phases, m0, off, off_col, ops.EPI_RELU)
        except ops.Unsupported:
            return None
        _ROUTES["ds_sheared_first_conv"] += 1
        return self._conv2_tail(v, shape, None, arithmetic)

    def _gn_sheared_first_layer(self, left, right, shift, arithmetic=None):
        conv, norm = self.conv1[0][0], self.conv1[0][1]
        guard = self._gn_qualifies(left.device, arithmetic)
        if guard is None:
            return None
        nonneg, structure = self._shift_structure(shift)
        assert nonneg
        n, c, h, w = left.shape
        d = shift.size(1)
        if structure is None or not self._sheared_fits(structure[0], structure[1], d, w, True):
            return None
# ... 137 lines not shown
        return True

    def _sheared_layers(self, plans, wr, q):
        cache = plans.setdefault("sheared", {})
        if q not in cache:
            k = sheared_kernels(wr, q)
            cout, c = k.shape[2], k.shape[3]
            cache[q] = tuple(ops.Conv3dLayer(k[i].reshape(3 * cout, c, 3, 7).float().contiguous(), 7, 1, 3, 1, False, planar=True,
                                             ksize_h=3) for i in range(2))
        return cache[q]

    def _sheared_layers_x3(self, plans, wr, q):
        cache = plans.setdefault("sheared_x3", {})
        if q not in cache:
            k = sheared_kernels(wr, q)
            cout, c = k.shape[2], k.shape[3]
            cache[q] = tuple(ops.Conv2dLayerX3(k[i].reshape(3 * cout, c, 3, 7).float().contiguous()) for i in range(2))
        return cache[q]

    @staticmethod
    def _left_planes_weight(wl):
        w = wl.detach().double()
        k = torch.stack([w[:, :, 1:].sum(2), w.sum(2), w[:, :, :2].sum(2)], dim=1)
        return k.reshape(-1, w.shape[1], 3, 3).float().contiguous()

    @staticmethod
    def _left_planes_layer(plans, wl):
        if "left2d" not in plans:
            plans["left2d"] = ops.Conv3dLayer(GlobalStack._left_planes_weight(wl), 3, 1, 1, 1, False, planar=True)
        return plans["left2d"]

    @staticmethod
    def _commuted_weights(wr):
        w = wr.detach()
        cout, c = w.shape[0], w.shape[1]
        wk = w.permute(2, 0, 1, 3, 4).contiguous()
        kq = torch.zeros_like(wk)
        kq[..., 1] = wk[..., 2]
        ke = torch.zeros((3, 3, cout, c, 3, 3), dtype=w.dtype, device=w.device)
        for kw in range(3):
            ke[:, kw, :, :, :, 1] = wk[..., kw]
        return tuple(t.reshape(-1, c, 3, 3).contiguous() for t in (wk, kq, ke))

    @staticmethod
    def _commuted_layers_x3(plans, wr):
        if "commuted_x3" not in plans:
            plans["commuted_x3"] = tuple(ops.Conv2dLayerX3(t.float()) for t in GlobalStack._commuted_weights(wr))
        return plans["commuted_x3"]

    @staticmethod
    def _commuted_layers(plans, wr):
        if "commuted" not in plans:
            w = wr.detach()
            cout, c = w.shape[0], w.shape[1]
            wk = w.permute(2, 0, 1, 3, 4).contiguous()
            kq = torch.zeros_like(wk)
            kq[..., 1] = wk[..., 2]
            ke = torch.zeros((3, 3, cout, c, 3, 3), dtype=w.dtype, device=w.device)
            for kw in range(3):
                ke[:, kw, :, :, :, 1] = wk[..., kw]
            mk = lambda t: ops.Conv3dLayer(t.reshape(-1, c, 3, 3).contiguous(), 3, 1, 1, 1, False, planar=True)
            plans["commuted"] = (mk(wk), mk(kq), mk(ke))
        return plans["commuted"]

    def forward_pair(self, left, right, shift, downsample=1, factored=True, timing=None, shift_checked=False, sheared=True,
                     fused_bn=True, spacing="unknown", commuted=True, arithmetic=None):
        return self._checked(self._forward_pair_unchecked, arithmetic, left, right, shift, downsample, factored, timing, shift_checked,
                             sheared, fused_bn, spacing, commuted)
    forward_pair.__doc__ = "see _forward_pair_unchecked"

    def _forward_pair_unchecked(self, *args, **kw):
        return _run(self._forward_pair_steps(*args, **kw))

    def _forward_pair_steps(self, left, right, shift, downsample=1, factored=True, timing=None, shift_checked=False, sheared=True,
                            fused_bn=True, spacing="unknown", commuted=True, arithmetic=None, pause=False):
        conv, bn = self.conv1[0][0], self.conv1[0][1]
        training_graph = torch.is_grad_enabled() and (left.requires_grad or right.requires_grad or conv.weight.requires_grad)
        if (training_graph and factored and timing is None and downsample == 1 and left.dtype == torch.float32
                and left.size(3) % 4 == 0 and (left.size(2) * left.size(3)) % 4 == 0 and shift.size(1) >= 2):
            structure = None
            if sheared and left.size(0) > 0 and shift.size(1) >= 4 and shift.dtype == torch.float32 and left.size(1) <= 32:
                nonneg, structure = self._shift_structure(shift)
                assert nonneg
            else:
                assert torch.all(shift >= 0.)
            plan = plan_for(conv, "", left.device)
            if structure is not None and not self._sheared_fits(structure[0], structure[1], shift.size(1), left.size(3), True):
                structure = None
            if (structure is not None and isinstance(bn, nn.BatchNorm3d) and bn.training and left.size(3) % 8 == 0
                    and left.size(3) <= 512 and fused_bn):
                v = _ShearedFirstConvBNFn.apply(left, right, conv.weight, bn.weight, bn.bias, conv, bn, plan, structure[0], structure[1],
                                                shift.size(1))
                return self._tail(self.conv2(v))
            if structure is not None:
                v = _ShearedFirstConvFn.apply(left, right, conv.weight, bn.weight, bn.bias, conv, bn, EPI_RELU, plan, structure[0],
                                              structure[1], shift.size(1))
                return self._tail(self.conv2(v))
            v = _FactoredFirstConvFn.apply(left, right, shift, conv.weight, bn.weight, bn.bias, conv, bn, EPI_RELU, plan, commuted)
            return self._tail(self.conv2(v))
        usable = (factored and downsample == 1 and not torch.is_grad_enabled() and isinstance(bn, nn.BatchNorm3d)
                  and not bn.training and left.dtype == torch.float32 and left.size(3) % 4 == 0 and shift.size(1) >= 2)
        if (downsample in (2, 4) and factored and sheared and timing is None and not torch.is_grad_enabled() and isinstance(bn, nn.BatchNorm3d)
                and not bn.training and left.is_cuda and left.dtype == torch.float32 and left.size(2) % downsample == 0
                and left.size(3) % downsample == 0 and shift.size(1) >= 4 and shift.dtype == torch.float32 and left.size(0) > 0
                and left.size(1) % 8 == 0 and left.size(1) * 2 == conv.in_channels and left.shape == right.shape):
            cost = self._ds_sheared_first_layer(left, right, shift, downsample, arithmetic)
            if cost is not None:
                return cost
        if (not usable and factored and sheared and downsample == 1 and timing is None and not torch.is_grad_enabled() and not self.training
                and isinstance(bn, nn.GroupNorm) and bn.num_groups == conv.out_channels and left.is_cuda and left.dtype == torch.float32
                and left.size(3) % 8 == 0 and left.size(3) <= 512 and shift.size(1) >= 4 and shift.dtype == torch.float32
                and left.size(0) > 0 and left.size(1) % 8 == 0 and left.size(1) * 2 == conv.in_channels):
            cost = self._gn_sheared_first_layer(left, right, shift, arithmetic)
            if cost is not None:
                return cost
        if not usable:
            if timing is None:
                vol = _BuildCostVolume.apply(left, right, shift, downsample)
                if torch.is_grad_enabled() or not vol.is_cuda:
                    return self.forward(vol)
                return self._forward_volume(vol, None, arithmetic, scale_from=(left, right) if downsample == 1 else None)
            assert torch.all(shift >= 0.)
            _mark(timing, "volume", 0)
            vol = ops.cost_volume_forward(left, right, shift, downsample)
            _mark(timing, "volume", 1)
            if torch.is_grad_enabled():
                _mark(timing, "conv1", 0)
                v = self.conv1(vol)
                _mark(timing, "conv1", 1)
                del vol
                return self._tail(self.conv2(v))
            return self._forward_volume(vol, timing, arithmetic, scale_from=(left, right))
        ticket = None
        known = shift_checked and spacing != "unknown"
        if known and not sheared:
            spacing = None
        if not known and left.size(0) > 0 and shift.size(1) >= 4 and shift.dtype == torch.float32:
            ticket = ops.shift_structure_begin(shift.detach())
        elif not shift_checked:
            assert torch.all(shift >= 0.)
        c = left.size(1)
        w = conv.weight
        plans = _factored_plans(conv, c)
        scale, bias = _folded_bn(bn, plans["plan"])
        split_prep = bool(self.split_prep and c % 8 == 0 and (3 * conv.out_channels) % 32 == 0 and right.is_contiguous()
                          and (not left.is_contiguous() or left.data_ptr() % 16 == 0) and right.data_ptr() % 16 == 0
                          and self._x3_select(left.device, arithmetic) is not None)
        prep_ws = self.__dict__.setdefault("_snvc_prep_ws", {})
        epoch = self.__dict__["_snvc_prep_epoch"] = next(_PREP_EPOCH)
        if split_prep:
            lx = plans.get("left2d_x3")
            if lx is None:
                lx = plans["left2d_x3"] = ops.Conv2dLayerX3(self._left_planes_weight(w.detach()[:, :c]))
            planes = ops.conv2d_x3_from_f32(left, [lx], prep_ws.setdefault("planes", {}))[0]
        else:
            planes = self._left_planes_layer(plans, w.detach()[:, :c])(left.unsqueeze(2))
        planes = planes.view(left.size(0), c, 3, left.size(2), left.size(3))
        shape = (left.size(0), c, shift.size(1)) + tuple(left.shape[2:])

        def sheared_inputs(q, m0):
            off, wu, off_col, wu_col = sheared_geometry(q, m0, shift.size(1), left.size(3))
            if split_prep:
                lx_g, lx_col = self._sheared_layers_x3(plans, w.detach()[:, c:], q)
                g, gcol = ops.sheared_prep_x3(right, q, wu, off, wu_col, off_col, lx_g, lx_col, prep_ws.setdefault("sheared", {}))
                _ROUTES["sheared_prep_x3"] += 1
                return g, gcol, off, off_col
            lay_g, lay_col = self._sheared_layers(plans, w.detach()[:, c:], q)
            if not self.prep_streams:
                g = lay_g(ops.sheared_upsample(right, q, wu, off).unsqueeze(2)).squeeze(2)
                gcol = lay_col(ops.sheared_upsample(right, q, wu_col, off_col).unsqueeze(2)).squeeze(2)
                return g, gcol, off, off_col
            cur = torch.cuda.current_stream(left.device)
            s1, s2 = self._side_streams(left.device)
            start = torch.cuda.Event()
            start.record(cur)
            out = []
            for st_, lay, wu_, off_ in ((s1, lay_g, wu, off), (s2, lay_col, wu_col, off_col)):
                with torch.cuda.stream(st_):
                    st_.wait_event(start)
                    t = lay(ops.sheared_upsample(right, q, wu_, off_).unsqueeze(2)).squeeze(2)
                    t.record_stream(cur)
                    done = torch.cuda.Event()
                    done.record(st_)
                out.append((t, done))
            for _, done in out:
                cur.wait_event(done)
            return out[0][0], out[1][0], off, off_col

        def commuted_inputs():
            if split_prep and (9 * conv.out_channels) % 32 == 0:
                lx_p, lx_q, lx_e = self._commuted_layers_x3(plans, w.detach()[:, c:])
                p_, q_ = ops.conv2d_x3_from_f32(right, [lx_p, lx_q], prep_ws.setdefault("commuted", {}))
                e_ = ops.conv2d_x3_from_f32(right[:, :, :, :4], [lx_e], prep_ws.setdefault("commuted_e", {}))[0]
                _ROUTES["commuted_prep_x3"] += 1
            else:
                lay_p, lay_q, lay_e = self._commuted_layers(plans, w.detach()[:, c:])
                r5 = right.unsqueeze(2)
                p_, q_ = lay_p(r5).squeeze(2), lay_q(r5).squeeze(2)
                e_ = lay_e(right[:, :, :, :4].contiguous().unsqueeze(2)).squeeze(2)
            return p_, q_, e_

        can_commute = commuted and shift.dtype == torch.float32 and left.size(3) <= 2048
        structure, guess, ready, ready_general = (spacing if known else None), None, None, None
        if ticket is not None:
            guess = plans.get("spacing_seen")
            _mark(timing, "volume", 0)
            dims = (shift.size(1), left.size(3))
            if sheared and guess is not None and guess[0] != "general" and guess[2:] == dims:
                ready = sheared_inputs(guess[0], guess[1])
            elif can_commute and (not sheared or (guess is not None and guess[0] == "general" and guess[1:] == dims)):
                ready_general = commuted_inputs()
            nonneg, structure = self._shift_structure_end(ticket, shift.size(1))
            assert nonneg
            if sheared:
                plans["spacing_seen"] = structure + dims if structure is not None else ("general",) + dims
            else:
                structure = None
        if pause:
            yield "shift checked; planes and speculative prep queued"
            if not (self.__dict__.get("_snvc_prep_epoch") == epoch and conv.__dict__.get("_snvc_factored") is plans
                    and fresh(plans["stamp"], (conv.weight,)) and all(a is b for a, b in zip(_folded_bn(bn, plans["plan"]), (scale, bias)))):
                _ROUTES["lazy_prefetch_stale"] += 1
                return (yield from self._forward_pair_steps(left, right, shift, downsample, factored, timing, True, sheared, fused_bn,
                                                            structure, commuted, arithmetic, pause=False))
        if structure is not None and not self._sheared_fits(structure[0], structure[1], shift.size(1), left.size(3), False):
            structure = None
        if structure is not None:
            q, m0 = structure
            if ready is None or tuple(guess[:2]) != tuple(structure):
                _mark(timing, "volume", 0)
                ready = sheared_inputs(q, m0)
            g, gcol, off, off_col = ready
            _mark(timing, "volume", 1)
            _mark(timing, "conv1", 0)
            st = self._x3_select(left.device, arithmetic)
            if st is not None and c % 8 == 0:
                v1s = self._buffer("v1s", (shape[0], 2, c // 8) + tuple(shape[2:]) + (8,), left.device, torch.float16)
                try:
                    ops.sheared_expand_split(g, gcol, planes, *self._x3_v1_affine(st, scale, bias), v1s, q, m0, off, off_col,
                                             ops.EPI_RELU | (ops.EPI_STREAM_OUT if self.stream_out else 0), st["flag"])
                except ops.Unsupported:
                    st = None
                else:
                    _mark(timing, "conv1", 1)
                    _ROUTES["sheared_first_conv"] += 1
                    self.__dict__["_snvc_last_v1"] = "v1s"
                    return self._tail_x3(st, v1s, timing)
            v = self._buffer("v1", shape, left.device)
            try:
                ops.sheared_expand(g, gcol, planes, scale, bias, v, q, m0, off, off_col, ops.EPI_RELU)
            except ops.Unsupported:
                structure = None
            else:
                _mark(timing, "conv1", 1)
                _ROUTES["sheared_first_conv"] += 1
                return self._conv2_tail(v, shape, timing, arithmetic)
        if can_commute:
            if ready_general is None:
                _mark(timing, "volume", 0)
                ready_general = commuted_inputs()
            p_, q_, e_ = ready_general
            _mark(timing, "volume", 1)
            _mark(timing, "conv1", 0)
            st = self._x3_select(left.device, arithmetic)
            if st is not None and c % 8 == 0:
                v1s = self._buffer("v1s", (shape[0], 2, c // 8) + tuple(shape[2:]) + (8,), left.device, torch.float16)
                try:
                    ops.warped_expand_split(p_, q_, e_, planes, shift, *self._x3_v1_affine(st, scale, bias), v1s,
                                            ops.EPI_RELU | (ops.EPI_STREAM_OUT if self.stream_out else 0), st["flag"])
                except ops.Unsupported:
                    pass
                else:
                    _mark(timing, "conv1", 1)
                    _ROUTES["commuted_first_conv"] += 1
                    self.__dict__["_snvc_last_v1"] = "v1s"
                    return self._tail_x3(st, v1s, timing)
            v = self._buffer("v1", shape, left.device)
            try:
                ops.warped_expand(p_, q_, e_, planes, shift, scale, bias, v, ops.EPI_RELU)
            except ops.Unsupported:
                pass
            else:
                _mark(timing, "conv1", 1)
                _ROUTES["commuted_first_conv"] += 1
                return self._conv2_tail(v, shape, timing, arithmetic)
        _mark(timing, "volume", 0)
        try:
            vol_r = ops.cost_volume_forward_right(right, shift, out=self._buffer("vol_r", shape, left.device))
        except ops.Unsupported:
            return self.forward_pair(left, right, shift, downsample, factored=False, timing=timing, arithmetic=arithmetic)
        _mark(timing, "volume", 1)
        _mark(timing, "conv1", 0)
        v = plans["right"](vol_r, scale, bias, None, ops.EPI_RELU, self._buffer("v1", shape, left.device), depth_planes=planes)
        _mark(timing, "conv1", 1)
        return self._conv2_tail(v, shape, timing, arithmetic)
```

snvc_amd/ops.py:

```python
import contextlib
import ctypes
import math
import threading
import time
from typing import Optional, Tuple

import torch

from . import _derived, _lib
from ._lib import (EPI_ADD_POST, EPI_ADD_PRE, EPI_RELU, EPI_SIGMOID, EPI_STREAM_OUT, F32, F64, Conv3dDesc,
                   Unsupported, check)

__all__ = [
    "cost_volume_forward", "cost_volume_forward_right", "cost_volume_backward", "cost_volume_backward_right", "depth_class_sums", "voxel_gather_forward", "voxel_gather_backward",
    "Conv3dLayer", "conv_variant", "conv3d_wgrad", "Conv3dLayerF16", "to_c8", "from_c8", "voxel_gather_forward_f16",
    "mul_broadcast_c8", "avgpool_depth4_c8", "volume_resample", "rect_to_psv_grid", "act_backward_reduce", "act_backward_apply", "bn_backward_coefs", "norm_stats", "affine_act", "mul_broadcast", "avgpool_depth4", "zero_stuff2x",
    "disparity_regression", "argmax_rows", "roiaware_pool3d_forward", "roiaware_pool3d_backward",
    "points_in_boxes_gpu", "points_in_boxes_cpu",
    "EPI_RELU", "EPI_ADD_PRE", "EPI_ADD_POST", "EPI_SIGMOID", "EPI_STREAM_OUT",
]


_variant_bits = 0


@contextlib.contextmanager
def conv_variant(algo_bits: int):
    global _variant_bits
    prev = _variant_bits
    _variant_bits = int(algo_bits)
    try:
        yield
    finally:
        _variant_bits = prev


def _algo(exact: bool = False) -> int:
    return (_variant_bits | _lib.ALGO_DIRECT) if exact else _variant_bits


def _gpu(t: torch.Tensor, name: str):
    if not t.is_cuda:
        raise RuntimeError(f"{name} must be a GPU tensor: Not implemented on the CPU")


def _ptr(t: Optional[torch.Tensor]):
    return ctypes.c_void_p(t.data_ptr()) if t is not None and t.numel() > 0 else ctypes.c_void_p(0)


def _stream(t: torch.Tensor):
    return ctypes.c_void_p(torch.cuda.current_stream(t.device).cuda_stream)


def _dtype_tag(t: torch.Tensor, what: str) -> int:
    if t.dtype == torch.float32:
        return F32
    if t.dtype == torch.float64:
        return F64
    raise RuntimeError(f'"{what}" not implemented for {t.dtype}')


def cost_volume_forward(left, right, shift, downsample: int):
    _gpu(left, "left"); _gpu(right, "right"); _gpu(shift, "shift")
    if left.dim() != 4 or tuple(left.shape) != tuple(right.shape):
        raise RuntimeError("Left image and right image should match their size.")
    if shift.dim() != 2 or left.size(0) != shift.size(0):
        raise RuntimeError("Image and shift should of same batch.")
    tag = _dtype_tag(left, "BuildCostVolume_forward")
    if right.dtype != left.dtype or shift.dtype != left.dtype:
        raise RuntimeError("left, right and shift must share one dtype")
    downsample = int(downsample)
    if downsample < 1:
        raise RuntimeError("downsample must be >= 1")
    n, c, hi, wi = left.shape
    d = shift.size(1)
    if hi % downsample or wi % downsample:
        raise RuntimeError("feature height and width must be multiples of downsample")
    out = torch.empty((n, 2 * c, d, hi // downsample, wi // downsample), dtype=left.dtype, device=left.device)
    if out.numel() == 0:
        return out
    left, right, shift = left.contiguous(), right.contiguous(), shift.contiguous()
    with torch.cuda.device(left.device):
        check(_lib.lib().snvc_cost_volume_forward(_ptr(left), _ptr(right), _ptr(shift), _ptr(out), n, c, hi, wi, d,
                                                  downsample, tag, _stream(left)), "build_cost_volume_forward")
    return out


def cost_volume_forward_right(right, shift, out=None):
    _gpu(right, "right"); _gpu(shift, "shift")
    if right.dtype != torch.float32 or shift.dtype != torch.float32:
        raise RuntimeError("cost_volume_forward_right is fp32 only")
    n, c, h, w = right.shape
    d = shift.size(1)
    if out is None:
        out = torch.empty((n, c, d, h, w), dtype=torch.float32, device=right.device)
    elif tuple(out.shape) != (n, c, d, h, w) or out.dtype != torch.float32 or not out.is_contiguous():
        raise RuntimeError("cost_volume_forward_right `out` must be a contiguous float32 [N,C,D,H,W] tensor")
    else:
        _written(out)
    if out.numel() == 0:
        return out
    right, shift = right.contiguous(), shift.contiguous()
    with torch.cuda.device(right.device):
        check(_lib.lib().snvc_cost_volume_forward_right(_ptr(right), _ptr(shift), _ptr(out), n, c, h, w, d, 1,
                                                        _stream(right)), "snvc_cost_volume_forward_right")
    return out


def cost_volume_backward(grad, shift, downsample: int):
    _gpu(grad, "grad"); _gpu(shift, "shift")
    tag = _dtype_tag(grad, "BuildCostVolume_backward")
    if shift.dtype != grad.dtype:
        raise RuntimeError("grad and shift must share one dtype")
    downsample = int(downsample)
    n, c2, _, h, w = grad.shape
    c, d = c2 // 2, shift.size(1)
    if grad.numel() != n * c * 2 * d * h * w:
        raise RuntimeError("grad shape is wrong")
    gl = torch.empty((n, c, h * downsample, w * downsample), dtype=grad.dtype, device=grad.device)
    gr = torch.empty_like(gl)
    if gl.numel() == 0:
        return gl, gr
    grad, shift = grad.contiguous(), shift.contiguous()
    with torch.cuda.device(grad.device):
        check(_lib.lib().snvc_cost_volume_backward(_ptr(grad), _ptr(shift), _ptr(gl), _ptr(gr), n, c, h, w, d,
                                                   downsample, tag, _stream(grad)), "build_cost_volume_backward")
    return gl, gr


def cost_volume_backward_right(grad_r, shift):
    _gpu(grad_r, "grad"); _gpu(shift, "shift")
    if grad_r.dtype != torch.float32 or shift.dtype != torch.float32 or grad_r.dim() != 5:
        raise RuntimeError("cost_volume_backward_right needs float32 [N,C,D,H,W]")
    grad_r, shift = grad_r.contiguous(), shift.contiguous()
    n, c, d, h, w = grad_r.shape
    out = torch.empty((n, c, h, w), dtype=torch.float32, device=grad_r.device)
    with torch.cuda.device(grad_r.device):
        check(_lib.lib().snvc_cost_volume_backward_right(_ptr(grad_r), _ptr(shift), _ptr(out), n, c, h, w, d, _stream(grad_r)),
              "snvc_cost_volume_backward_right")
    return out


def depth_class_sums(g):
    _gpu(g, "g")
    g = g.contiguous()
    n, c, d, h, w = g.shape
    out = torch.empty((n, c, 3, h, w), dtype=torch.float32, device=g.device)
    with torch.cuda.device(g.device):
        check(_lib.lib().snvc_depth_class_sums(_ptr(g), _ptr(out), n * c, d, h * w, _stream(g)), "snvc_depth_class_sums")
    return out


def _check_gather(left, right, l_pts, r_pts):
    for t, nm in ((left, "left"), (right, "right"), (l_pts, "grid_proj_left"), (r_pts, "grid_proj_right")):
        _gpu(t, nm)
        if t.dtype != torch.float32:
            raise RuntimeError(f"{nm} must be float32")
    if left.dim() != 4 or tuple(left.shape) != tuple(right.shape):
        raise RuntimeError("left and right feature maps must have the same [N,F,H,W] shape")
    if l_pts.dim() != 3 or l_pts.size(1) != 2 or tuple(l_pts.shape) != tuple(r_pts.shape) or l_pts.size(0) != left.size(0):
        raise RuntimeError("grid projections must be [N,2,V] for the same batch as the features")

# ... 1108 lines not shown
        if tuple(residual.shape) != shape:
            raise RuntimeError("residual must have the result's shape (split C8)")
    for t in (scale, shift):
        if t.dtype != torch.float32 or tuple(t.shape) != ((n if per_sample else 1), c) or not t.is_contiguous():
            raise RuntimeError("scale / shift must be contiguous float32 [N or 1, C]")
    if raw.numel() == 0:
        return out
    null = ctypes.c_void_p(0)
    with torch.cuda.device(raw.device):
        check(_lib.lib().snvc_f16x3_affine_from_ncdhw(
            _ptr(raw), _ptr(scale), _ptr(shift), _ptr(residual) if residual is not None else null,
            _lo_ptr(residual) if residual is not None else null, _ptr(out), _lo_ptr(out), _ptr(overflow), n, c, math.prod(sp),
            _batch_stride(raw), _batch_stride(out), _batch_stride(residual) if residual is not None else 0, 1 if per_sample else 0,
            int(flags), float(2.0 ** out_exp), float(2.0 ** -res_exp), _stream(raw)), "snvc_f16x3_affine_from_ncdhw")
    return out


def split_scale_for(*tensors) -> torch.Tensor:
    if tensors and all(t.is_cuda and t.dtype == torch.float32 and t.is_contiguous() and t.data_ptr() % 16 == 0 and t.numel() > 0
                       for t in tensors):
        out = None
        for t in tensors:
            s_ = split_scale_of(t.detach())
            out = s_ if out is None else torch.minimum(out, s_)
        return out
    amax = None
    for t in tensors:
        lo, hi = torch.aminmax(t.detach())
        a = torch.maximum(-lo, hi)
        amax = a if amax is None else torch.maximum(amax, a)
    amax = amax.float().reshape(1)
    e = torch.floor(torch.log2(16384.0 / amax))
    e = torch.where(torch.isfinite(e), e, torch.zeros_like(e)).clamp_(-24, 40)
    return torch.exp2(e)


_SCALE_SCRATCH = {}
_SCALE_SCRATCH_LOCK = threading.Lock()


def _scale_scratch(device) -> torch.Tensor:
    key = (device, torch.cuda.current_stream(device).cuda_stream)
    scratch = _SCALE_SCRATCH.get(key)
    if scratch is None:
        with _SCALE_SCRATCH_LOCK:
            scratch = _SCALE_SCRATCH.get(key)
            if scratch is None:
                scratch = _SCALE_SCRATCH[key] = torch.zeros(2, dtype=torch.int32, device=device)
    return scratch


def split_scale_of(t: torch.Tensor) -> torch.Tensor:
    _gpu(t, "t")
    if t.dtype != torch.float32 or not t.is_contiguous() or t.data_ptr() % 16:
        return split_scale_for(t)
    scratch = _scale_scratch(t.device)
    out = torch.empty(1, dtype=torch.float32, device=t.device)
    with torch.cuda.device(t.device):
        check(_lib.lib().snvc_f16x3_split_scale(_ptr(t), t.numel(), _ptr(scratch), _ptr(out), _stream(t)), "snvc_f16x3_split_scale")
    return out


def sheared_upsample_split(right, q: int, wu: int, off: int, mul_dev: torch.Tensor):
    _gpu(right, "right")
    if right.dtype != torch.float32 or right.dim() != 4:
        raise RuntimeError("sheared_upsample_split needs a float32 [N,C,H,W] tensor")
    right = right.contiguous()
    n, c, h, w = right.shape
    out = torch.empty((n, 2, (c + 7) // 8, 1, h, wu, 8), dtype=torch.float16, device=right.device)
    if out.numel():
        with torch.cuda.device(right.device):
            check(_lib.lib().snvc_sheared_upsample_split(_ptr(right), _ptr(out), _lo_ptr(out), _ptr(mul_dev), n, c, h, w, int(q), int(wu), int(off),
                                                         _stream(right)), "snvc_sheared_upsample_split")
    return out


class Conv2dLayerX3:

    def __init__(self, weight: torch.Tensor):
        _gpu(weight, "weight")
        if weight.dtype != torch.float32 or weight.dim() != 4:
            raise RuntimeError("Conv2dLayerX3 needs a float32 [Cout,Cin,kh,kw] weight")
        self.cout, self.cin, self.kh, self.kw = (int(v) for v in weight.shape)
        nbytes = _lib.lib().snvc_f16x3_conv2d_packed_weight_bytes(self.cout, self.cin, self.kh, self.kw)
        if nbytes < 0:
            raise Unsupported("Conv2dLayerX3: 3x7 or 3x3 kernels, Cin % 8 == 0, Cout % 32 == 0")
        w = weight.detach().contiguous()
        wmax = float(w.abs().max().item()) if w.numel() else 1.0
        self.w_exp = 14 - math.frexp(wmax)[1] if wmax > 0 and math.isfinite(wmax) else 0
        self.packed = torch.empty(nbytes, dtype=torch.uint8, device=w.device)
        with torch.cuda.device(w.device):
            check(_lib.lib().snvc_f16x3_conv2d_pack_weights(_ptr(w), self.cout, self.cin, self.kh, self.kw, _ptr(self.packed),
                                                            float(2.0 ** self.w_exp), _stream(w)), "snvc_f16x3_conv2d_pack_weights")

    def __call__(self, x, x_mul_dev=None, scale=None, bias=None, flags: int = 0, x_exp: int = 0):
        _split_check(x, "x")
        if x.size(2) * 8 != self.cin or x.size(3) != 1:
            raise RuntimeError(f"Conv2dLayerX3 input must be a split pair [N,2,{self.cin // 8},1,H,W,8]")
        n, h, w = x.size(0), x.size(4), x.size(5)
        y = torch.empty((n, self.cout, h, w), dtype=torch.float32, device=x.device)
        if y.numel():
            with torch.cuda.device(x.device):
                check(_lib.lib().snvc_f16x3_conv2d_forward(_ptr(x), _lo_ptr(x), _ptr(self.packed), _ptr(scale), _ptr(bias), _ptr(y), n, self.cin,
                                                           self.cout, h, w, self.kh, self.kw, float(2.0 ** -(self.w_exp + x_exp)), _ptr(x_mul_dev),
                                                           int(flags), _stream(x)), "snvc_f16x3_conv2d_forward")
        return y


def sheared_prep_x3(right, q: int, wu: int, off: int, wu_col: int, off_col: int, lay_g: "Conv2dLayerX3", lay_col: "Conv2dLayerX3", ws: dict):
    _gpu(right, "right")
    right = right.contiguous()
    n, c, h, w = right.shape
    key = (n, c, h, w, wu, wu_col, right.device)
    if ws.get("key") != key:
        dev = right.device
        ws.clear()
        ws.update(key=key, rq=torch.empty(n * 2 * c * h * wu, dtype=torch.float16, device=dev),
                  rq2=torch.empty(n * 2 * c * h * wu_col, dtype=torch.float16, device=dev), mul=torch.empty(1, dtype=torch.float32, device=dev),
                  g=torch.empty((n, lay_g.cout, h, wu), dtype=torch.float32, device=dev),
                  gcol=torch.empty((n, lay_col.cout, h, wu_col), dtype=torch.float32, device=dev))
    scratch = _scale_scratch(right.device)
    with torch.cuda.device(right.device):
        check(_lib.lib().snvc_sheared_prep_x3(_ptr(right), n, c, h, w, int(q), int(wu), int(off), int(wu_col), int(off_col), _ptr(lay_g.packed),
                                              _ptr(lay_col.packed), lay_g.cout, float(2.0 ** -lay_g.w_exp), float(2.0 ** -lay_col.w_exp),
                                              _ptr(ws["rq"]), _ptr(ws["rq2"]), _ptr(scratch), _ptr(ws["mul"]), _ptr(ws["g"]), _ptr(ws["gcol"]),
                                              _stream(right)), "snvc_sheared_prep_x3")
    return ws["g"], ws["gcol"]


def conv2d_x3_from_f32(x, layers, ws: dict):
    _gpu(x, "x")
    x = x.contiguous()
    if x.dtype != torch.float32 or x.dim() != 4:
        raise RuntimeError("conv2d_x3_from_f32 needs a float32 [N,C,H,W] tensor")
    n, c, h, w = x.shape
    key = (n, c, h, w, tuple(id(l) for l in layers), x.device)
    if ws.get("key") != key:
        ws.clear()
        ws.update(key=key, split=torch.empty(n * 2 * c * h * w, dtype=torch.float16, device=x.device),
                  mul=torch.empty(1, dtype=torch.float32, device=x.device),
                  y=[torch.empty((n, l.cout, h, w), dtype=torch.float32, device=x.device) for l in layers])
        k = len(layers)
        ws["c_packed"] = (ctypes.c_void_p * k)(*[l.packed.data_ptr() for l in layers])
        ws["c_cout"] = (ctypes.c_int64 * k)(*[l.cout for l in layers])
        ws["c_mul"] = (ctypes.c_float * k)(*[2.0 ** -l.w_exp for l in layers])
        ws["c_y"] = (ctypes.c_void_p * k)(*[t.data_ptr() for t in ws["y"]])
        ws["layers"] = list(layers)
    scratch = _scale_scratch(x.device)
    with torch.cuda.device(x.device):
        check(_lib.lib().snvc_f16x3_conv2d_from_f32(_ptr(x), n, c, h, w, layers[0].kh, layers[0].kw, len(layers), ws["c_packed"], ws["c_cout"],
                                                    ws["c_mul"], ws["c_y"], _ptr(ws["split"]), _ptr(scratch), _ptr(ws["mul"]), _stream(x)),
              "snvc_f16x3_conv2d_from_f32")
    return ws["y"]


def from_split(x: torch.Tensor, exp: int = 0, channels: Optional[int] = None) -> torch.Tensor:
    _split_check(x, "x")
    n, g = x.shape[0], x.shape[2]
    sp = tuple(x.shape[3:6])
    c = channels if channels is not None else 8 * g
    y = torch.empty((n, c) + sp, dtype=torch.float32, device=x.device)
    if y.numel() == 0:
        return y
    with torch.cuda.device(x.device):
        check(_lib.lib().snvc_f16x3_to_ncdhw(_ptr(x), _lo_ptr(x), _ptr(y), n, c, math.prod(sp), _batch_stride(x), 0, float(2.0 ** -exp),
                                             _stream(x)), "snvc_f16x3_to_ncdhw")
    return y


X3_SMALL_BELOW = {"stride2": 0, "transposed": 4096}


_ONES_ZEROS = {}


def _ones_zeros(c: int, device):
    key = (c, device)
    hit = _ONES_ZEROS.get(key)
    if hit is None:
        hit = _ONES_ZEROS[key] = (torch.ones(c, device=device), torch.zeros(c, device=device))
    return hit


def x3_form(cout: int, ksize: int, stride: int, dilation: int, transposed: bool, n: int, out_sp, plain: bool, split_out: bool,
            forced: Optional[int]) -> int:
    if forced is None and stride == 1 and not transposed and ksize in (5, 7) and cout % 32 == 0:
        tiles5 = n * -(-out_sp[0] // 4) * -(-out_sp[1] // 4) * -(-out_sp[2] // 32) * (cout // 32)
        q16 = X3_Q16[0] and split_out and tiles5 >= 512 and (ksize == 7 or dilation == 2 or X3_Q16_K5[0])
        return _lib.ALGO_X3_Q16 if q16 else 0
    if forced is None and ksize == 3 and cout % 64 == 0 and (stride == 2 or transposed):
        if transposed:
            wgs = 8 * n * -(-out_sp[0] // 8) * -(-out_sp[1] // 8) * -(-out_sp[2] // 64)
            return _lib.ALGO_X3_SMALL if wgs < X3_SMALL_BELOW["transposed"] else 0
        wgs = n * -(-out_sp[0] // 2) * -(-out_sp[1] // 4) * -(-out_sp[2] // 32)
        if X3_Q16_S2[0] and plain and split_out:
            return _lib.ALGO_X3_Q16
        return _lib.ALGO_X3_SMALL if wgs < X3_SMALL_BELOW["stride2"] else 0
    if forced is not None or stride != 1 or transposed or ksize != 3 or cout == 1:
        return forced if forced is not None else 0
    tiles = n * -(-out_sp[0] // 4) * -(-out_sp[1] // 4) * -(-out_sp[2] // 32)
    if plain and X3_Q16[0] and cout % 32 == 0 and tiles * (cout // 32) >= X3_Q16_MIN_JOBS[0]:
        return _lib.ALGO_X3_Q16
    if cout % 64 == 0 and tiles * (cout // 64) >= 1024:
        return _lib.ALGO_X3_SERIAL
    if tiles * (cout // 32) >= 1024 or cout == 32 and tiles >= 512:
        return _lib.ALGO_X3_NARROW if cout != 32 else 0
    return _lib.ALGO_X3_SMALL


def _residual_f32_check(residual_f32, y) -> None:
    if (residual_f32.dtype != torch.float32 or tuple(residual_f32.shape) != tuple(y.shape) or not _dense_inner(residual_f32)
            or _batch_stride(residual_f32) != _batch_stride(y)):
        raise RuntimeError("residual_f32 must be a float32 tensor of the result's shape and layout")


class Conv3dLayerX3(_ConvGeometry):

    def __init__(self, weight: torch.Tensor, ksize: int = 3, stride: int = 1, pad: int = 1, dilation: int = 1, transposed: bool = False,
                 algo: Optional[int] = None, w_mul_dev: Optional[torch.Tensor] = None):
        _gpu(weight, "weight")
        if weight.dtype != torch.float32:
            raise RuntimeError("conv3d weights must be float32")
        super().__init__(weight, ksize, stride, pad, dilation, transposed)
        self.forced_algo = algo
        self.algo = int(algo or 0)
        self.w_mul_dev = w_mul_dev
        self._sc_w = self._bi_0 = None
        if w_mul_dev is not None:
            self.weight = (weight.detach() * w_mul_dev).contiguous()
            self.w_exp = 0
        else:
            self.weight = weight.detach().contiguous()
            wmax = float(self.weight.abs().max().item()) if weight.numel() else 1.0
            self.w_exp = 14 - math.frexp(wmax)[1] if wmax > 0 and math.isfinite(wmax) else 0
        self._packed = {}
        self.packed = self._pack(self.algo) if w_mul_dev is None else None
        self._affine = {}

    def _pack(self, algo: int):
        hit = self._packed.get(algo)
        if hit is None:
            probe = self._desc(1, (16, 16, 32), 0, algo)
            nbytes = _lib.lib().snvc_f16x3_conv3d_packed_weight_bytes(ctypes.byref(probe))
            if nbytes < 0:
                check(2, "snvc_f16x3_conv3d_packed_weight_bytes")
            hit = torch.empty(nbytes, dtype=torch.uint8, device=self.weight.device)
            with torch.cuda.device(self.weight.device):
                check(_lib.lib().snvc_f16x3_conv3d_pack_weights(ctypes.byref(probe), _ptr(self.weight), _ptr(hit), float(2.0 ** self.w_exp),
                                                                _stream(self.weight)), "snvc_f16x3_conv3d_pack_weights")
            self._packed[algo] = hit
        return hit

    def _launch(self, x, plain: bool = False, split_out: bool = False):
        n, in_sp = x.size(0), tuple(x.shape[3:6])
        out_sp = self.out_spatial(in_sp)
        algo = self.algo = x3_form(self.cout, self.ksize, self.stride, self.dilation, self.transposed, n, out_sp, plain, split_out,
                                   self.forced_algo)
        return n, in_sp, out_sp, algo, self._pack(algo)

    def _unit_affine(self, device):
        if self._sc_w is None:
            self._sc_w, self._bi_0 = _ones_zeros(self.cout, device)[0] / self.w_mul_dev, _ones_zeros(self.cout, device)[1]
        return self._sc_w, self._bi_0

    def folded(self, scale, bias, x_exp: int, out_exp: int):
        def build():
            dev = self.weight.device
            sc = (scale.detach().float() if scale is not None else torch.ones(self.cout, device=dev)) * (2.0 ** (out_exp - x_exp - self.w_exp))
            bi = (bias.detach().float() if bias is not None else torch.zeros(self.cout, device=dev)) * (2.0 ** out_exp)
            return sc.contiguous(), bi.contiguous()
        return _derived.derived(self._affine, (x_exp, out_exp), (scale, bias), build)

    def __call__(self, x, x_exp: int = 0, scale=None, bias=None, residual=None, flags: int = 0, out=None, out_exp: int = 0,
                 out_f32=None, to_f32: bool = False, head=None, overflow=None, x_mul_dev=None, res_exp: Optional[int] = None,
                 residual_f32: Optional[torch.Tensor] = None):
        _split_check(x, "x")
        if x.size(2) * 8 != self.cin:
            raise RuntimeError(f"conv3d input must have {self.cin} channels (split C8), got {x.size(2) * 8}")
        f32 = to_f32 or out_f32 is not None or self.cout == 1
        n, in_sp, out_sp, algo, packed = self._launch(x, plain=residual is None and (not f32 or (self.w_mul_dev is not None and head is None)),
                                                      split_out=not f32 and head is None)
        split_shape = (n, 2, self.cout // 8) + out_sp + (8,)
        if f32:
            out_f32 = _result(out_f32, (n, self.cout) + out_sp, torch.float32, x.device,
                              "out_f32 must be a float32 [N,Cout,D,H,W] tensor, dense below dim 0")
        else:
            out = _result(out, split_shape, torch.float16, x.device, "conv3d `out` must be a split C8 tensor of the output shape", _split_check)
        residual = _residual(residual, split_shape, "residual must have the output's shape (split C8)", _split_check)
        if residual_f32 is not None:
            if not f32 or residual is not None or flags & (EPI_ADD_PRE | EPI_ADD_POST) or self.cout == 1:
                raise RuntimeError("residual_f32 goes with a float32 result and no other residual")
            _residual_f32_check(residual_f32, out_f32)
            flags = flags | EPI_ADD_POST
        y_head = None
        if head is not None:
            head = head.detach().reshape(-1).float().contiguous()
            y_head = torch.empty((n, 1) + out_sp, dtype=torch.float32, device=x.device)
        if self.w_mul_dev is not None and scale is None and bias is None and x_exp == 0 and out_exp == 0:
            sc, bi = self._unit_affine(x.device)
            if x_mul_dev is not None:
                sc = sc / x_mul_dev
        else:
            sc, bi = self.folded(scale, bias, x_exp, out_exp)
            if x_mul_dev is not None:
                sc = (sc / x_mul_dev).contiguous()
            if self.w_mul_dev is not None:
                sc = (sc / self.w_mul_dev).contiguous()
        if n == 0:
            return out_f32 if f32 else ((out, y_head) if head is not None else out)
        d = self._desc(n, in_sp, flags, algo, _batch_stride(x), _batch_stride(out_f32 if f32 else out),
                       _batch_stride(residual) if residual is not None else 0)
        null = ctypes.c_void_p(0)
        with torch.cuda.device(x.device):
            check(_lib.lib().snvc_f16x3_conv3d_forward(ctypes.byref(d), _ptr(x), _lo_ptr(x), _ptr(packed), _ptr(sc), _ptr(bi),
                                                       _ptr(residual if residual_f32 is None else residual_f32),
                                                       _lo_ptr(residual) if residual is not None else null,
                                                       null if f32 else _ptr(out), null if f32 else _lo_ptr(out),
                                                       _ptr(out_f32) if f32 else null, _ptr(head), _ptr(y_head), float(2.0 ** -out_exp),
                                                       float(2.0 ** (out_exp - (out_exp if res_exp is None else res_exp))),
                                                       _ptr(overflow), _stream(x)), "snvc_f16x3_conv3d_forward")
        if f32:
            return out_f32
        return (out, y_head) if head is not None else out

    def forward_f32(self, x, x_mul_dev, residual_f32: Optional[torch.Tensor] = None, relu: bool = False):
        _split_check(x, "x")
        if self.w_mul_dev is None or x.size(2) * 8 != self.cin:
            raise RuntimeError("forward_f32: a device-scaled layer (w_mul_dev) and an input of its channel count")
        n, in_sp, out_sp, algo, packed = self._launch(x, plain=True, split_out=False)
        sc, bi = self._unit_affine(x.device)
        y = torch.empty((n, self.cout) + out_sp, dtype=torch.float32, device=x.device)
        if residual_f32 is not None:
            _residual_f32_check(residual_f32, y)
        if n == 0:
            return y
        d = self._desc(n, in_sp, EPI_RELU if relu else 0, algo, _batch_stride(x), _batch_stride(y), 0)
        with torch.cuda.device(x.device):
            check(_lib.lib().snvc_f16x3_conv3d_forward_f32(ctypes.byref(d), _ptr(x), _lo_ptr(x), _ptr(packed), _ptr(sc), _ptr(bi),
                                                           _ptr(x_mul_dev), _ptr(residual_f32), _ptr(y), 1.0, _stream(x)),
                  "snvc_f16x3_conv3d_forward_f32")
        return y

    def forward_stats(self, x, x_mul_dev, gamma, beta, eps: float):
        _split_check(x, "x")
        if self.w_mul_dev is None or x.size(2) * 8 != self.cin or self.cout % 32:
            return None
        n, in_sp, out_sp, algo, packed = self._launch(x, plain=True, split_out=False)
        sc, bi = self._unit_affine(x.device)
        raw = torch.empty((n, self.cout) + out_sp, dtype=torch.float32, device=x.device)
        d = self._desc(n, in_sp, 0, algo, _batch_stride(x), _batch_stride(raw), 0)
        nbytes = _lib.lib().snvc_f16x3_conv3d_stats_workspace_bytes(ctypes.byref(d))
        if nbytes < 0:
            return None
        ws = torch.empty(nbytes, dtype=torch.uint8, device=x.device)
        out = torch.empty((4, self.cout), dtype=torch.float32, device=x.device)
        with torch.cuda.device(x.device):
            rc = _lib.lib().snvc_f16x3_conv3d_forward_stats(ctypes.byref(d), _ptr(x), _lo_ptr(x), _ptr(packed), _ptr(sc), _ptr(bi),
                                                            _ptr(x_mul_dev), _ptr(raw), 1.0, _ptr(gamma), _ptr(beta), _ptr(out[0]), _ptr(out[1]), _ptr(out[2]),
                                                            _ptr(out[3]), _ptr(ws), float(eps), _stream(x))
        if rc == 2:
            return None
        check(rc, "snvc_f16x3_conv3d_forward_stats")
        return raw, out[0:1], out[1:2], out[2:3], out[3:4]

    def forward_tail(self, x, x_exp: int, scale, bias, tail: "TailWeightsX3", residual=None, flags: int = 0, out_exp: int = 0,
                     overflow=None, res_exp: Optional[int] = None, out=None):
        _split_check(x, "x")
        if not self.transposed or self.stride != 2 or x.size(2) * 8 != self.cin or tail.cin != self.cout:
            raise RuntimeError("forward_tail: a ConvTranspose3d(k3,s2,p1,op1) layer whose Cout equals the tail's Cin")
        n, in_sp, out_sp, algo, packed = self._launch(x)
        shape = (n, 27, 8) + in_sp
        if out is None:
            out = torch.empty(shape, dtype=torch.float32, device=x.device)
        elif tuple(out.shape) != shape or out.dtype != torch.float32 or not out.is_contiguous():
            raise RuntimeError("forward_tail `out` must be a contiguous float32 [N, 27, 8, Din, Hin, Win] tensor")
        else:
            _written(out)
        residual = _residual(residual, (n, 2, self.cout // 8) + out_sp + (8,), "residual must have the layer's output shape (split C8)", _split_check)
        sc, bi = self.folded(scale, bias, x_exp, out_exp)
        if n == 0:
            return out
        d = self._desc(n, in_sp, flags, algo, _batch_stride(x), 0, _batch_stride(residual) if residual is not None else 0)
        null = ctypes.c_void_p(0)
        with torch.cuda.device(x.device):
            check(_lib.lib().snvc_f16x3_deconv3d_tail_forward(
                ctypes.byref(d), _ptr(x), _lo_ptr(x), _ptr(packed), _ptr(sc), _ptr(bi), _ptr(residual),
                _lo_ptr(residual) if residual is not None else null, float(2.0 ** (out_exp - (out_exp if res_exp is None else res_exp))),
                _ptr(tail.packed), _ptr(out), float(2.0 ** -(out_exp + tail.w_exp)), _ptr(overflow), _stream(x)),
                "snvc_f16x3_deconv3d_tail_forward")
        return out


class TailWeightsX3:

    def __init__(self, weight: torch.Tensor):
        _gpu(weight, "weight")
        w = weight.detach().reshape(weight.shape[0], -1).float().contiguous()
        if w.shape[1] != 27 or w.shape[0] % 32 != 0:
            raise RuntimeError("tail weights must be [Cin, 27] (or [Cin, 1, 3, 3, 3]) with Cin % 32 == 0")
        self.cin = int(w.shape[0])
        wmax = float(w.abs().max().item()) if w.numel() else 1.0
        self.w_exp = 14 - math.frexp(wmax)[1] if wmax > 0 and math.isfinite(wmax) else 0
        nbytes = _lib.lib().snvc_f16x3_tail_packed_weight_bytes(self.cin)
        self.packed = torch.empty(nbytes, dtype=torch.uint8, device=w.device)
        with torch.cuda.device(w.device):
            check(_lib.lib().snvc_f16x3_tail_pack_weights(_ptr(w), self.cin, _ptr(self.packed), float(2.0 ** self.w_exp), _stream(w)),
                  "snvc_f16x3_tail_pack_weights")


def deconv_tail_gather(t: torch.Tensor, bias: Optional[torch.Tensor] = None, residual: Optional[torch.Tensor] = None, out=None):
    _gpu(t, "t")
    if t.dtype != torch.float32 or t.dim() != 6 or t.size(1) != 27 or t.size(2) != 8 or not t.is_contiguous():
        raise RuntimeError("t must be a contiguous float32 [N, 27, 8, nd, nh, nw] tensor")
    n, nd, nh, nw = t.size(0), t.size(3), t.size(4), t.size(5)
    shape = (n, 1, 4 * nd, 4 * nh, 4 * nw)
    if out is None:
        out = torch.empty(shape, dtype=torch.float32, device=t.device)
    elif tuple(out.shape) != shape or out.dtype != torch.float32 or not out.is_contiguous():
        raise RuntimeError("out must be a contiguous float32 tensor of the output shape")
    else:
        _written(out)
    if residual is not None:
        _gpu(residual, "residual")
        if residual.dtype != torch.float32 or residual.numel() != out.numel() or not residual.is_contiguous():
            raise RuntimeError("residual must be a contiguous float32 tensor of the output shape")
    if bias is not None:
        bias = bias.detach().reshape(-1)[:1].float().contiguous()
    with torch.cuda.device(t.device):
        check(_lib.lib().snvc_deconv_tail_gather(_ptr(t), _ptr(bias), _ptr(residual), _ptr(out), n, nd, nh, nw, _stream(t)),
              "snvc_deconv_tail_gather")
    return out


def mul_broadcast_split(feat, occ, out=None):
    _split_check(feat, "feat")
    _gpu(occ, "occ")
    occ = occ.contiguous()
    n, g = feat.shape[0], feat.shape[2]
    s_ = math.prod(feat.shape[3:6])
    if occ.dtype != torch.float32 or occ.numel() != n * s_:
        raise RuntimeError("occupancy must be float32 [N,1,D,H,W] matching the feature volume")
    if out is None:
        out = torch.empty(feat.shape, dtype=torch.float16, device=feat.device)
    else:
        _split_check(out, "out")
        if tuple(out.shape) != tuple(feat.shape):
            raise RuntimeError("mul_broadcast_split `out` must have feat's shape")
        _written(out)
    if feat.numel() == 0:
        return out
    with torch.cuda.device(feat.device):
        check(_lib.lib().snvc_f16x3_mul_broadcast(_ptr(feat), _lo_ptr(feat), _ptr(occ), _ptr(out), _lo_ptr(out), n, 8 * g, s_,
                                                  _batch_stride(feat), _batch_stride(out), _stream(feat)), "snvc_f16x3_mul_broadcast")
    return out


def mul_broadcast_c8(feat, occ, out=None):
    _c8_check(feat, "feat")
    _gpu(occ, "occ")
    occ = occ.contiguous()
    n, g = feat.shape[0], feat.shape[1]
    s = math.prod(feat.shape[2:5])
    if occ.dtype != torch.float32 or occ.numel() != n * s:
        raise RuntimeError("occupancy must be float32 [N,1,D,H,W] matching the feature volume")
    if out is None:
        out = torch.empty_like(feat)
    else:
        _c8_check(out, "out")
        if tuple(out.shape) != tuple(feat.shape):
            raise RuntimeError("mul_broadcast_c8 `out` must have feat's shape")
        _written(out)
    if feat.numel() == 0:
        return out
    with torch.cuda.device(feat.device):
        check(_lib.lib().snvc_f16_mul_broadcast(_ptr(feat), _ptr(occ), _ptr(out), n, 8 * g, s, _batch_stride(feat),
                                                _batch_stride(out), _stream(feat)), "snvc_f16_mul_broadcast")
    return out
# ... 70 lines not shown
```

Measured before the change: 515.5.

## Fuse sheared cost-volume expansion into the first 3D conv's LDS producer

Adds a source mode to the x3q 3D conv kernel that builds the split f16 input tile directly in LDS. It sums interleaved sheared-gather and plane tensors, applies affine and ReLU, and splits the result into hi/lo halves inside the conv. This replaces reading a materialized v1s volume. The 2D conv epilogue also gains an interleaved-layout write so the prep kernels emit gi/p_il directly. The goal is to remove the full-volume write and re-read of the first cost volume, at the price of extra ALU work interleaved with the MFMA schedule and a lazy fallback expansion path.

```diff
diff --git a/include/snvc_fused.h b/include/snvc_fused.h
--- /dev/null
+++ b/include/snvc_fused.h
@@ -0,0 +1,35 @@
+#ifndef SNVC_FUSED_H
+#define SNVC_FUSED_H
+
+#include <stdint.h>
+
+#include "snvc_hip.h"
+
+#ifdef __cplusplus
+extern "C" {
+#endif
+
+SNVC_API int snvc_fused_abi_version(void);
+
+SNVC_API int64_t snvc_fused_il_index(int mode, int64_t oc, int64_t C, int64_t H, int64_t pitch, int64_t lp, int64_t cls0,
+                                     int64_t h, int64_t x);
+
+SNVC_API int snvc_fused_sheared_prep_x3(const float *right, int64_t N, int64_t C, int64_t H, int64_t W, int q, int64_t WU, int off,
+                                        int64_t WU2, int off2, const void *packed_g, const void *packed_col, int64_t Cout3,
+                                        float out_mul_g, float out_mul_col, void *rq_split, void *rq2_split, void *scratch8,
+                                        float *mul_dev, float *g, float *gcol, float *gi, int64_t pitch, int64_t lp, void *stream);
+
+SNVC_API int snvc_fused_planes_from_f32(const float *x, int64_t N, int64_t C, int64_t H, int64_t W, const void *packed, int64_t cout,
+                                        float out_mul, float *y, float *p_il, void *ws_split, void *scratch8, float *mul_dev,
+                                        void *stream);
+
+SNVC_API int snvc_fused_first_conv3d_forward(const snvc_conv3d_desc *desc, const void *packed_weight, const float *scale,
+                                             const float *bias, void *y_hi, void *y_lo, const float *head, float *y_head,
+                                             float head_mul, int *overflow, const float *gi, int64_t pitch, int64_t lp,
+                                             const float *p_il, const float *v_scale, const float *v_bias, int q, int m0, int off,
+                                             int off2, int v_flags, void *stream);
+
+#ifdef __cplusplus
+}
+#endif
+#endif
diff --git a/snvc_amd/_fused.py b/snvc_amd/_fused.py
--- /dev/null
+++ b/snvc_amd/_fused.py
@@ -0,0 +1,36 @@
+import ctypes
+
+from . import _lib
+
+_ABI = 1
+
+c_i64 = ctypes.c_int64
+c_p = ctypes.c_void_p
+c_int = ctypes.c_int
+c_f = ctypes.c_float
+
+SIGNATURES = {
+    "snvc_fused_abi_version": (c_int, []),
+    "snvc_fused_il_index": (c_i64, [c_int] + [c_i64] * 8),
+    "snvc_fused_sheared_prep_x3": (c_int, [c_p, c_i64, c_i64, c_i64, c_i64, c_int, c_i64, c_int, c_i64, c_int, c_p, c_p, c_i64, c_f, c_f]
+                                   + [c_p] * 7 + [c_i64, c_i64, c_p]),
+    "snvc_fused_planes_from_f32": (c_int, [c_p, c_i64, c_i64, c_i64, c_i64, c_p, c_i64, c_f] + [c_p] * 6),
+    "snvc_fused_first_conv3d_forward": (c_int, [ctypes.POINTER(_lib.Conv3dDesc)] + [c_p] * 7 + [c_f, c_p, c_p, c_i64, c_i64, c_p, c_p, c_p]
+                                        + [c_int] * 5 + [c_p]),
+}
+
+_bound = None
+
+
+def lib() -> ctypes.CDLL:
+    global _bound
+    if _bound is None:
+        handle = _lib.lib()
+        for name, (res, args) in SIGNATURES.items():
+            fn = getattr(handle, name)
+            fn.restype = res
+            fn.argtypes = args
+        if handle.snvc_fused_abi_version() != _ABI:
+            raise RuntimeError("libsnvc_hip.so fused first layer ABI version mismatch; rebuild it")
+        _bound = handle
+    return _bound
diff --git a/snvc_amd/csrc/conv3d_f16.hip b/snvc_amd/csrc/conv3d_f16.hip
--- a/snvc_amd/csrc/conv3d_f16.hip
+++ b/snvc_amd/csrc/conv3d_f16.hip
@@ -2,6 +2,7 @@
 
 #include "common.hpp"
 #include "elementwise_internal.hpp"
+#include "snvc_fused.h"
 
 namespace snvc {
 namespace {
@@ -46,6 +47,26 @@
     int N, cls_mode;
     int64_t cls_wstride;
     int64_t x_bs, y_bs, r_bs, yf_bs;
+};
+
+template <class I>
+__host__ __device__ __forceinline__ I il_index(int mode, I oc, I C, I H, I pitch, I lp, I cls0, I h, I x) {
+    const I cls = mode ? oc % 3 : oc / C, co = mode ? oc / 3 : oc % C, groups = (C + 7) / 8;
+    return ((((cls0 + cls) * groups + (co >> 3)) * H + h) * pitch + lp + x) * 8 + (co & 7);
+}
+
+struct F16IlArgs : F16Args {
+    float *y_il;
+    int64_t il_bs;
+    int il_mode, il_C, il_pitch, il_lp, il_cls0;
+};
+
+struct F16SrcArgs : F16Args {
+    const float *gi;
+    const float *p_il;
+    const float *v_scale, *v_bias;
+    int64_t gi_bs;
+    int v_pitch, v_lp, v_q, v_m0, v_off, v_off2, v_flags;
 };
 
 
@@ -590,6 +611,7 @@
 }
 
 typedef float f32x4q __attribute__((ext_vector_type(4)));
+typedef _Float16 h4q __attribute__((ext_vector_type(4)));
 
 struct X3QCfg {
     static constexpr int TD = 4, TH = 4, NB = 4, IN_D = 6, IN_H = 6, IN_W = 34, VOX = IN_D * IN_H * IN_W, GB = VOX * 16;
@@ -611,9 +633,15 @@
                  : "memory");
 }
 
-template <int EPI>
+template <int SRC, class A>
+__device__ __forceinline__ const F16SrcArgs &src_args_of(const A &a) {
+    if constexpr (SRC == 1) return a;
+    else return *reinterpret_cast<const F16SrcArgs *>(&a);
+}
+
+template <int EPI, int SRC = 0>
 __global__ void __launch_bounds__(256, 2)
-conv3d_x3q_kernel(const F16Args a) {
+conv3d_x3q_kernel(const std::conditional_t<SRC == 1, F16SrcArgs, F16Args> a) {
     using Cfg = X3QCfg;
     constexpr int NB = Cfg::NB, TH = Cfg::TH, IN_H = Cfg::IN_H, IN_W = Cfg::IN_W, VOX = Cfg::VOX, NIT = Cfg::NIT, NQ = Cfg::NQ;
     constexpr int ITEMS = Cfg::ITEMS, PF = Cfg::PF;
@@ -688,7 +716,86 @@
     }
 
     const unsigned lds_base = (unsigned)(uintptr_t)(__attribute__((address_space(3))) char *)lds;
-    issue(0, 0);
+    constexpr int COLS = IN_H * IN_W;
+    const F16SrcArgs &aa = src_args_of<SRC>(a);
+    struct {
+        unsigned g_off, p_off, w_off, g_slab, p_slab;
+        float hi, lo, vmax;
+        const char *gb, *pb;
+        f32x4q g, p, bi[2];
+        float sc[8];
+        h4q chi, clo;
+    } pr{};
+    auto prod_setup = [&]() {
+        const int cid = tid < COLS ? tid : tid - COLS;
+        const int hh = cid / IN_W, ww = cid - hh * IN_W;
+        const int gh = ih0 + hh, gw = iw0 + ww;
+        const bool col_ok = (unsigned)gh < (unsigned)aa.Hin && (unsigned)gw < (unsigned)aa.Win;
+        const int ghc = gh < 0 ? 0 : (gh < aa.Hin ? gh : aa.Hin - 1), gwc = gw < 0 ? 0 : (gw < aa.Win ? gw : aa.Win - 1);
+        const bool last = gwc == aa.Win - 1;
+        const int i0 = last ? aa.v_q * (aa.Win - 1) - aa.v_m0 + aa.v_off2 : aa.v_q * gwc - aa.v_m0 + aa.v_off;
+        pr.g_off = (unsigned)((((last ? 3 * aa.CGin : 0) * aa.Hin + ghc) * aa.v_pitch + aa.v_lp + i0) * 32);
+        pr.p_off = (unsigned)((ghc * aa.Win + gwc) * 32);
+        pr.g_slab = (unsigned)(aa.Hin * aa.v_pitch * 32);
+        pr.p_slab = (unsigned)(aa.Hin * aa.Win * 32);
+        pr.w_off = (unsigned)(cid * 16);
+        pr.hi = col_ok ? 65504.0f : 0.0f;
+        pr.lo = (col_ok && !(aa.v_flags & SNVC_EPI_RELU)) ? -65504.0f : 0.0f;
+        pr.gb = reinterpret_cast<const char *>(aa.gi + n * aa.gi_bs);
+        pr.pb = reinterpret_cast<const char *>(aa.p_il + n * 3 * (int64_t)aa.CGin * aa.Hin * aa.Win * 8);
+    };
+    auto prod_affine = [&](int group) {
+        int z = 0;
+        asm volatile("" : "+v"(z));
+        const f32x4q *s = reinterpret_cast<const f32x4q *>(aa.v_scale + group * 8 + z), *b = reinterpret_cast<const f32x4q *>(aa.v_bias + group * 8 + z);
+        const f32x4q s0 = s[0], s1 = s[1];
+        pr.bi[0] = b[0]; pr.bi[1] = b[1];
+#pragma unroll
+        for (int e = 0; e < 8; ++e)
+            pr.sc[e] = __builtin_bit_cast(float, __builtin_amdgcn_readfirstlane(__builtin_bit_cast(int, e < 4 ? s0[e & 3] : s1[e & 3])));
+    };
+    auto prod_load = [&](int group, int j) {
+        const int gd = id0 + (j >> 1);
+        const int gdc = gd < 0 ? 0 : (gd < aa.Din ? gd : aa.Din - 1);
+        const int cls = gdc == aa.Din - 1 ? 2 : (gdc == 0 ? 0 : 1);
+        const unsigned slab = (unsigned)(cls * aa.CGin + group);
+        pr.g = *reinterpret_cast<const f32x4q *>(pr.gb + (pr.g_off + (slab * pr.g_slab - (unsigned)gdc * 32u + 16u * (j & 1))));
+        pr.p = *reinterpret_cast<const f32x4q *>(pr.pb + (pr.p_off + (slab * pr.p_slab + 16u * (j & 1))));
+    };
+    auto prod_form = [&](int buf, int j) {
+        const int dd = j >> 1, half = j & 1;
+        const bool d_ok = (unsigned)(id0 + dd) < (unsigned)aa.Din;
+        const float hb = d_ok ? pr.hi : 0.0f, lb = d_ok ? pr.lo : 0.0f;
+        h4q o, ol;
+#pragma unroll
+        for (int e = 0; e < 4; ++e) {
+            const float t = __builtin_fmaf(pr.g[e] + pr.p[e], pr.sc[4 * half + e], pr.bi[half][e]);
+            const float tc = __builtin_amdgcn_fmed3f(t, lb, hb);
+            pr.vmax = __builtin_fmaxf(pr.vmax, __builtin_fabsf(tc));
+            o[e] = (_Float16)tc;
+            ol[e] = (_Float16)(tc - (float)o[e]);
+        }
+        if (half == 0) {
+            pr.chi = o;
+            pr.clo = ol;
+        } else {
+            char *const dst = lds + pr.w_off + buf * Cfg::IMG_BYTES + dd * (COLS * 16);
+            *reinterpret_cast<h8 *>(dst) = __builtin_shufflevector(pr.chi, o, 0, 1, 2, 3, 4, 5, 6, 7);
+            *reinterpret_cast<h8 *>(dst + Cfg::PLANE_BYTES) = __builtin_shufflevector(pr.clo, ol, 0, 1, 2, 3, 4, 5, 6, 7);
+        }
+    };
+    constexpr int NHP = 2 * Cfg::IN_D;
+    if constexpr (SRC == 1) {
+        prod_setup();
+        prod_affine(0);
+#pragma unroll
+        for (int j = 0; j < NHP; ++j) {
+            prod_load(0, j);
+            prod_form(0, j);
+        }
+    } else {
+        issue(0, 0);
+    }
     __syncthreads();
     h8 epc[6];
     auto run_chunk = [&](const int chunk, auto last_tag) {
@@ -714,7 +821,7 @@
                 if (hs == 2 * Cfg::FILL_STEP) {
 #pragma unroll
                     for (int i = 0; i < PF; ++i) asm volatile("" ::"v"(q_[i][0]), "v"(q_[i][1]), "v"(q_[i][2]), "v"(q_[i][3]));
-                    if constexpr (!LAST) issue(chunk + 1, (chunk + 1) & 1);
+                    if constexpr (!LAST && SRC == 0) issue(chunk + 1, (chunk + 1) & 1);
                 }
 #pragma unroll
                 for (int m = 0; m < 4; ++m) af[m] = q_[0][m];
@@ -722,6 +829,9 @@
                 for (int i = 0; i + 1 < PF; ++i)
 #pragma unroll
                     for (int m = 0; m < 4; ++m) q_[i][m] = q_[i + 1][m];
+                if constexpr (!LAST && SRC == 1) {
+                    if (hs == 0) prod_affine(chunk + 1);
+                }
                 if constexpr (!LAST) {
 #pragma unroll
                     for (int m = 0; m < 4; ++m) q_[PF - 1][m] = wq[m * 64];
@@ -751,6 +861,11 @@
                 wait_lgkm_for<0>(bfr[cur]);
             }
             __builtin_amdgcn_sched_barrier(0);
+            constexpr bool FORM = !LAST && SRC == 1;
+            if constexpr (FORM) {
+                if (hs >= 1 && hs <= NHP) prod_form((chunk + 1) & 1, hs - 1);
+                if (hs < NHP) prod_load(chunk + 1, hs);
+            }
 #pragma unroll
             for (int term = 0; term < 3; ++term)
 #pragma unroll
@@ -764,12 +879,26 @@
                             acc[2 * (hs & 1) + rr][ph][h] =
                                 __builtin_amdgcn_mfma_f32_16x16x32_f16(aw, bx, acc[2 * (hs & 1) + rr][ph][h], 0, 0, 0);
                         }
+            if constexpr (FORM) {
+                if (hs >= 1 && hs <= NHP) {
+#pragma unroll
+                    for (int k = 0; k < 12; ++k) {
+                        __builtin_amdgcn_sched_group_barrier(0x008, 1, 0);
+                        __builtin_amdgcn_sched_group_barrier(0x002, 4, 0);
+                    }
+                    __builtin_amdgcn_sched_group_barrier(0x020, 2, 0);
+                    __builtin_amdgcn_sched_group_barrier(0x200, 2, 0);
+                }
+            }
             __builtin_amdgcn_sched_barrier(0);
         }
         __syncthreads();
     };
     for (int chunk = 0; chunk + 1 < a.nchunks; ++chunk) run_chunk(chunk, std::false_type{});
     run_chunk(a.nchunks - 1, std::true_type{});
+    if constexpr (SRC == 1) {
+        if (pr.vmax >= 65504.0f && a.overflow) atomicOr(a.overflow, 1);
+    }
     if (has_aff) asm volatile("" ::"v"(epc[0]), "v"(epc[1]), "v"(epc[2]), "v"(epc[3]));
     if constexpr (EPI == 3) asm volatile("" ::"v"(epc[4]), "v"(epc[5]));
 
@@ -887,9 +1016,9 @@
     static_assert(NQ > PF, "the refill is issued PF k-steps before the chunk ends");
 };
 
-template <class Cfg>
+template <class Cfg, int IL = 0>
 __global__ void __launch_bounds__(256, 2)
-conv2d_x3q_kernel(const F16Args a) {
+conv2d_x3q_kernel(const std::conditional_t<IL == 1, F16IlArgs, F16Args> a) {
     constexpr int NB = Cfg::NB, IN_W = Cfg::IN_W, VOX = Cfg::VOX, NIT = Cfg::NIT, NQ = Cfg::NQ;
     constexpr int ITEMS = Cfg::ITEMS, PF = Cfg::PF;
     extern __shared__ __attribute__((aligned(16))) char lds[];
@@ -1038,11 +1167,24 @@
             const int pw = ow0 + 16 * ph + col;
             if (phh < a.nh && pw < a.nw) {
                 float *yp = yn + (int64_t)phh * a.Wout + pw;
+                float v8[8];
 #pragma unroll
                 for (int e = 0; e < 8; ++e) {
                     float v = __builtin_fmaf(acc[nb][ph][e >> 2][e & 3], sc[e], bi[e]);
                     if (relu) v = __builtin_fmaxf(v, 0.0f);
                     yp[e * out_hw] = v;
+                    v8[e] = v;
+                }
+                if constexpr (IL == 1) {
+                    float *il = a.y_il + n * a.il_bs;
+                    if (a.il_mode == 0) {
+                        float *dst = il + il_index<int>(0, c0, a.il_C, a.Hout, a.il_pitch, a.il_lp, a.il_cls0, phh, pw);
+                        *reinterpret_cast<f32x4q *>(dst) = f32x4q{v8[0], v8[1], v8[2], v8[3]};
+                        *reinterpret_cast<f32x4q *>(dst + 4) = f32x4q{v8[4], v8[5], v8[6], v8[7]};
+                    } else {
+#pragma unroll
+                        for (int e = 0; e < 8; ++e) il[il_index<int>(1, c0 + e, a.il_C, a.Hout, a.il_pitch, a.il_lp, a.il_cls0, phh, pw)] = v8[e];
+                    }
                 }
             }
         }
@@ -2103,7 +2245,7 @@
                          const float *scale, const float *bias, const void *res_hi, const void *res_lo, void *y_hi,
                          void *y_lo, float *y_f32, const float *head, float *y_head, float head_mul, float res_mul,
                          int *overflow, const void *tail_w, float *t_out, float tail_mul, void *stream, double *stats = nullptr,
-                         int64_t *stats_slots = nullptr, const float *x_mul = nullptr) {
+                         int64_t *stats_slots = nullptr, const float *x_mul = nullptr, const snvc::F16SrcArgs *src = nullptr) {
     using namespace snvc;
     F16Plan p;
     if (!d) return fail(SNVC_ERR_INVALID_ARGUMENT, "snvc_f16x3_conv3d_forward: null desc");
@@ -2116,7 +2258,7 @@
     const bool plane = d->Cout == 1;
     const bool to_f32 = y_f32 != nullptr;
     if (plane && !to_f32) return fail(SNVC_ERR_INVALID_ARGUMENT, "snvc_f16x3_conv3d_forward: a one-channel layer writes y_f32");
-    if (!x_hi || !x_lo || !packed_weight || (!tail && !to_f32 && (!y_hi || !y_lo)))
+    if ((!src && (!x_hi || !x_lo)) || !packed_weight || (!tail && !to_f32 && (!y_hi || !y_lo)))
         return fail(SNVC_ERR_INVALID_ARGUMENT, "snvc_f16x3_conv3d_forward: null pointer");
     if ((scale == nullptr) != (bias == nullptr))
         return fail(SNVC_ERR_INVALID_ARGUMENT, "snvc_f16x3_conv3d_forward: scale and bias must both be given or both be NULL");
@@ -2205,6 +2347,8 @@
             if (e != hipSuccess) return fail(SNVC_ERR_HIP, "snvc_f16x3_conv3d_forward_stats: hipMemsetAsync failed");
         }
     }
+    if (src && p.kind != FK3XQ)
+        return fail(SNVC_ERR_UNSUPPORTED, "snvc_fused_first_conv3d_forward: a 3x3x3 stride-1 layer on the 16x16x32 form (SNVC_ALGO_X3_Q16)");
 #define SNVC_X3_LAUNCH(CFG) do { if (to_f32) launch_f16<CFG, 2>(a, grid, st); else launch_f16<CFG, 0>(a, grid, st); } while (0)
     switch (p.kind) {
         case FK3X:
@@ -2256,6 +2400,14 @@
             if (resflags || (to_f32 && head)) return fail(SNVC_ERR_UNSUPPORTED, "snvc_f16x3_conv3d_forward: the 16x16x32 form has no split residual, no side head beside a float32 result");
             if (ntiles * p.cblocks >= ((int64_t)1 << 30)) return fail(SNVC_ERR_UNSUPPORTED, "snvc_f16x3_conv3d_forward: too many tiles");
             grid = dim3((unsigned)(ntiles * p.cblocks), 1, (unsigned)d->N);
+            if (src) {
+                if (to_f32) return fail(SNVC_ERR_UNSUPPORTED, "snvc_fused_first_conv3d_forward: a split C8 output");
+                F16SrcArgs b = *src;
+                static_cast<F16Args &>(b) = a;
+                if (head) launch_lds<conv3d_x3q_kernel<3, 1>>(grid, 256, X3QCfg::LDS_BYTES, st, b);
+                else launch_lds<conv3d_x3q_kernel<0, 1>>(grid, 256, X3QCfg::LDS_BYTES, st, b);
+                break;
+            }
             if (to_f32) launch_lds<conv3d_x3q_kernel<2>>(grid, 256, X3QCfg::LDS_BYTES, st, a);
             else if (head) launch_lds<conv3d_x3q_kernel<3>>(grid, 256, X3QCfg::LDS_BYTES, st, a);
             else launch_lds<conv3d_x3q_kernel<0>>(grid, 256, X3QCfg::LDS_BYTES, st, a);
@@ -2273,6 +2425,31 @@
                               int *overflow, void *stream) {
     return f16x3_forward(d, x_hi, x_lo, packed_weight, scale, bias, res_hi, res_lo, y_hi, y_lo, y_f32, head, y_head, head_mul, res_mul,
                          overflow, nullptr, nullptr, 0.0f, stream);
+}
+
+int snvc_fused_first_conv3d_forward(const snvc_conv3d_desc *d, const void *packed_weight, const float *scale, const float *bias, void *y_hi,
+                                    void *y_lo, const float *head, float *y_head, float head_mul, int *overflow, const float *gi,
+                                    int64_t pitch, int64_t lp, const float *p_il, const float *v_scale, const float *v_bias, int q, int m0,
+                                    int off, int off2, int v_flags, void *stream) {
+    using namespace snvc;
+    if (!d || !gi || !p_il || !v_scale || !v_bias) return fail(SNVC_ERR_INVALID_ARGUMENT, "snvc_fused_first_conv3d_forward: null pointer");
+    if (d->transposed || d->ksize != 3 || d->stride != 1 || d->pad != 1 || d->dilation != 1 || d->Cin % 8 || d->Din < 1 || d->Hin < 1 || d->Win < 1 ||
+        (q != 1 && q != 2) || (v_flags & ~SNVC_EPI_RELU))
+        return fail(SNVC_ERR_UNSUPPORTED, "snvc_fused_first_conv3d_forward: a 3x3x3 / stride 1 / pad 1 layer, Cin % 8 == 0, q = 1 | 2");
+    if ((reinterpret_cast<uintptr_t>(gi) | reinterpret_cast<uintptr_t>(p_il) | reinterpret_cast<uintptr_t>(v_scale) | reinterpret_cast<uintptr_t>(v_bias)) & 31)
+        return fail(SNVC_ERR_INVALID_ARGUMENT, "snvc_fused_first_conv3d_forward: gi / p_il / v_scale / v_bias must be 32-byte aligned");
+    const int64_t D = d->Din, H = d->Hin, W = d->Win, CG = d->Cin / 8;
+    const int64_t lo_g = -(D - 1) - m0 + off, hi_g = (int64_t)q * (W - 2) - m0 + off;
+    const int64_t lo_c = (int64_t)q * (W - 1) - (D - 1) - m0 + off2, hi_c = (int64_t)q * (W - 1) - m0 + off2;
+    if (lp < 0 || pitch <= 0 || lp + lo_c < 0 || lp + hi_c >= pitch || (W > 1 && (lp + lo_g < 0 || lp + hi_g >= pitch)))
+        return fail(SNVC_ERR_INVALID_ARGUMENT, "snvc_fused_first_conv3d_forward: pitch / lp do not cover the G indices of this shape");
+    if (6 * CG * H * pitch * 32 >= ((int64_t)1 << 31) || 3 * CG * H * W * 32 >= ((int64_t)1 << 31))
+        return fail(SNVC_ERR_UNSUPPORTED, "snvc_fused_first_conv3d_forward: one sample of gi / p_il must stay below 2 GiB");
+    F16SrcArgs s{};
+    s.gi = gi; s.p_il = p_il; s.v_scale = v_scale; s.v_bias = v_bias; s.gi_bs = 6 * CG * H * pitch * 8;
+    s.v_pitch = (int)pitch; s.v_lp = (int)lp; s.v_q = q; s.v_m0 = m0; s.v_off = off; s.v_off2 = off2; s.v_flags = v_flags;
+    return f16x3_forward(d, nullptr, nullptr, packed_weight, scale, bias, nullptr, nullptr, y_hi, y_lo, nullptr, head, y_head, head_mul, 1.0f,
+                         overflow, nullptr, nullptr, 0.0f, stream, nullptr, nullptr, nullptr, &s);
 }
 
 static int64_t f16x3_stats_slots(const snvc_conv3d_desc &d, const snvc::F16Plan &p) {
@@ -2364,9 +2541,25 @@
     return check_launch("snvc_f16x3_conv2d_pack_weights");
 }
 
+struct snvc_il_out {
+    float *y_il;
+    int64_t bs, pitch, lp, cls0, classes;
+    int mode;
+};
+
+static int f16x3_conv2d_forward(const void *x_hi, const void *x_lo, const void *packed_weight, const float *scale, const float *bias,
+                                float *y, int64_t N, int64_t Cin, int64_t Cout, int64_t H, int64_t W, int kh, int kw, float out_mul,
+                                const float *x_mul_dev, int flags, void *stream, const snvc_il_out *il);
+
 int snvc_f16x3_conv2d_forward(const void *x_hi, const void *x_lo, const void *packed_weight, const float *scale, const float *bias,
                               float *y, int64_t N, int64_t Cin, int64_t Cout, int64_t H, int64_t W, int kh, int kw, float out_mul,
                               const float *x_mul_dev, int flags, void *stream) {
+    return f16x3_conv2d_forward(x_hi, x_lo, packed_weight, scale, bias, y, N, Cin, Cout, H, W, kh, kw, out_mul, x_mul_dev, flags, stream, nullptr);
+}
+
+static int f16x3_conv2d_forward(const void *x_hi, const void *x_lo, const void *packed_weight, const float *scale, const float *bias,
+                                float *y, int64_t N, int64_t Cin, int64_t Cout, int64_t H, int64_t W, int kh, int kw, float out_mul,
+                                const float *x_mul_dev, int flags, void *stream, const snvc_il_out *il) {
     using namespace snvc;
     if (N < 0 || H <= 0 || W <= 0 || snvc_f16x3_conv2d_packed_weight_bytes((int)Cout, (int)Cin, kh, kw) < 0)
         return fail(SNVC_ERR_UNSUPPORTED, "snvc_f16x3_conv2d_forward: 3x7 or 3x3 kernels, Cin % 8 == 0, Cout % 32 == 0");
@@ -2393,7 +2586,23 @@
     if (jobs >= ((int64_t)1 << 30)) return fail(SNVC_ERR_UNSUPPORTED, "snvc_f16x3_conv2d_forward: too many tiles");
     const dim3 grid((unsigned)jobs, 1, (unsigned)N);
     hipStream_t st = as_stream(stream);
-    if (kw == 7) {
+    if (il) {
+        const int64_t C = Cout / 3, need = il->classes * ((C + 7) / 8) * H * il->pitch * 8;
+        if (!il->y_il || Cout % 3 || (il->mode == 0 && C % 8) || il->lp < 0 || il->lp + W > il->pitch || il->cls0 < 0 || il->cls0 + 3 > il->classes ||
+            need > il->bs || need >= ((int64_t)1 << 31) || (reinterpret_cast<uintptr_t>(il->y_il) & 31) || il->bs % 8)
+            return fail(SNVC_ERR_INVALID_ARGUMENT, "snvc_fused: the interleaved output does not hold the layer's result");
+        F16IlArgs b{};
+        static_cast<F16Args &>(b) = a;
+        b.y_il = il->y_il; b.il_bs = il->bs; b.il_mode = il->mode; b.il_C = (int)C; b.il_pitch = (int)il->pitch; b.il_lp = (int)il->lp;
+        b.il_cls0 = (int)il->cls0;
+        if (kw == 7) {
+            using C7 = X2QCfg<3, 7>;
+            launch_lds<conv2d_x3q_kernel<C7, 1>>(grid, 256, C7::LDS_BYTES, st, b);
+        } else {
+            using C3 = X2QCfg<3, 3>;
+            launch_lds<conv2d_x3q_kernel<C3, 1>>(grid, 256, C3::LDS_BYTES, st, b);
+        }
+    } else if (kw == 7) {
         using C = X2QCfg<3, 7>;
         launch_lds<conv2d_x3q_kernel<C>>(grid, 256, C::LDS_BYTES, st, a);
     } else {
@@ -2404,10 +2613,34 @@
 }
 
 extern "C" int snvc_sheared_upsample_split(const float *, void *, void *, const float *, int64_t, int64_t, int64_t, int64_t, int, int64_t, int, void *);
+static int sheared_prep_x3(const float *right, int64_t N, int64_t C, int64_t H, int64_t W, int q, int64_t WU, int off, int64_t WU2, int off2,
+                           const void *packed_g, const void *packed_col, int64_t Cout3, float out_mul_g, float out_mul_col, void *rq_split,
+                           void *rq2_split, void *scratch8, float *mul_dev, float *g, float *gcol, void *stream, float *gi, int64_t pitch,
+                           int64_t lp);
+
 int snvc_sheared_prep_x3(const float *right, int64_t N, int64_t C, int64_t H, int64_t W, int q, int64_t WU, int off, int64_t WU2, int off2,
                          const void *packed_g, const void *packed_col, int64_t Cout3, float out_mul_g, float out_mul_col, void *rq_split,
                          void *rq2_split, void *scratch8, float *mul_dev, float *g, float *gcol, void *stream) {
+    return sheared_prep_x3(right, N, C, H, W, q, WU, off, WU2, off2, packed_g, packed_col, Cout3, out_mul_g, out_mul_col, rq_split, rq2_split,
+                           scratch8, mul_dev, g, gcol, stream, nullptr, 0, 0);
+}
+
+int snvc_fused_sheared_prep_x3(const float *right, int64_t N, int64_t C, int64_t H, int64_t W, int q, int64_t WU, int off, int64_t WU2,
+                               int off2, const void *packed_g, const void *packed_col, int64_t Cout3, float out_mul_g, float out_mul_col,
+                               void *rq_split, void *rq2_split, void *scratch8, float *mul_dev, float *g, float *gcol, float *gi,
+                               int64_t pitch, int64_t lp, void *stream) {
+    if (!gi || Cout3 != 3 * C) return snvc::fail(SNVC_ERR_INVALID_ARGUMENT, "snvc_fused_sheared_prep_x3: gi is NULL or Cout3 != 3 * C");
+    return sheared_prep_x3(right, N, C, H, W, q, WU, off, WU2, off2, packed_g, packed_col, Cout3, out_mul_g, out_mul_col, rq_split, rq2_split,
+                           scratch8, mul_dev, g, gcol, stream, gi, pitch, lp);
+}
+
+static int sheared_prep_x3(const float *right, int64_t N, int64_t C, int64_t H, int64_t W, int q, int64_t WU, int off, int64_t WU2, int off2,
+                           const void *packed_g, const void *packed_col, int64_t Cout3, float out_mul_g, float out_mul_col, void *rq_split,
+                           void *rq2_split, void *scratch8, float *mul_dev, float *g, float *gcol, void *stream, float *gi, int64_t pitch,
+                           int64_t lp) {
     using namespace snvc;
+    const int64_t gi_bs = 6 * (C / 8) * H * pitch * 8;
+    const snvc_il_out il_g{gi, gi_bs, pitch, lp, 0, 6, 0}, il_col{gi, gi_bs, pitch, lp, 3, 6, 0};
     if (!right || !packed_g || !packed_col || !rq_split || !rq2_split || !scratch8 || !mul_dev || !g || !gcol)
         return fail(SNVC_ERR_INVALID_ARGUMENT, "snvc_sheared_prep_x3: null pointer");
     if (N <= 0 || C % 8 || Cout3 % 32) return fail(SNVC_ERR_UNSUPPORTED, "snvc_sheared_prep_x3: C % 8 == 0, 3 * Cout % 32 == 0");
@@ -2417,12 +2650,37 @@
     _Float16 *a = reinterpret_cast<_Float16 *>(rq_split), *b = reinterpret_cast<_Float16 *>(rq2_split);
     rc = snvc_sheared_upsample_split(right, a, a + G * H * WU * 8, mul_dev, N, C, H, W, q, WU, off, stream);
     if (rc) return rc;
-    rc = snvc_f16x3_conv2d_forward(a, a + G * H * WU * 8, packed_g, nullptr, nullptr, g, N, C, Cout3, H, WU, 3, 7, out_mul_g, mul_dev, 0, stream);
+    rc = f16x3_conv2d_forward(a, a + G * H * WU * 8, packed_g, nullptr, nullptr, g, N, C, Cout3, H, WU, 3, 7, out_mul_g, mul_dev, 0, stream,
+                              gi ? &il_g : nullptr);
     if (rc) return rc;
     rc = snvc_sheared_upsample_split(right, b, b + G * H * WU2 * 8, mul_dev, N, C, H, W, q, WU2, off2, stream);
     if (rc) return rc;
-    return snvc_f16x3_conv2d_forward(b, b + G * H * WU2 * 8, packed_col, nullptr, nullptr, gcol, N, C, Cout3, H, WU2, 3, 7, out_mul_col, mul_dev, 0,
-                                     stream);
+    return f16x3_conv2d_forward(b, b + G * H * WU2 * 8, packed_col, nullptr, nullptr, gcol, N, C, Cout3, H, WU2, 3, 7, out_mul_col, mul_dev, 0,
+                                stream, gi ? &il_col : nullptr);
+}
+
+int snvc_fused_abi_version(void) { return 1; }
+
+int64_t snvc_fused_il_index(int mode, int64_t oc, int64_t C, int64_t H, int64_t pitch, int64_t lp, int64_t cls0, int64_t h, int64_t x) {
+    if ((mode != 0 && mode != 1) || C <= 0 || oc < 0 || oc >= 3 * C || H <= 0 || h < 0 || h >= H || lp < 0 || x < 0 || lp + x >= pitch || cls0 < 0)
+        return -1;
+    return snvc::il_index<int64_t>(mode, oc, C, H, pitch, lp, cls0, h, x);
+}
+
+extern "C" int snvc_f16x3_from_ncdhw(const float *, void *, void *, int64_t, int64_t, int64_t, int64_t, int64_t, float, const float *, void *);
+int snvc_fused_planes_from_f32(const float *x, int64_t N, int64_t C, int64_t H, int64_t W, const void *packed, int64_t cout, float out_mul,
+                               float *y, float *p_il, void *ws_split, void *scratch8, float *mul_dev, void *stream) {
+    using namespace snvc;
+    if (!x || !packed || !y || !p_il || !ws_split || !scratch8 || !mul_dev)
+        return fail(SNVC_ERR_INVALID_ARGUMENT, "snvc_fused_planes_from_f32: null pointer");
+    if (N <= 0 || C % 8 || cout != 3 * C) return fail(SNVC_ERR_UNSUPPORTED, "snvc_fused_planes_from_f32: C % 8 == 0, cout == 3 * C");
+    int rc = snvc_f16x3_split_scale(x, N * C * H * W, scratch8, mul_dev, stream);
+    if (rc) return rc;
+    _Float16 *a = reinterpret_cast<_Float16 *>(ws_split);
+    rc = snvc_f16x3_from_ncdhw(x, a, a + C * H * W, N, C, H * W, 0, 0, 1.0f, mul_dev, stream);
+    if (rc) return rc;
+    const snvc_il_out il{p_il, 3 * (C / 8) * H * W * 8, W, 0, 0, 3, 1};
+    return f16x3_conv2d_forward(a, a + C * H * W, packed, nullptr, nullptr, y, N, C, cout, H, W, 3, 3, out_mul, mul_dev, 0, stream, &il);
 }
 
 extern "C" int snvc_f16x3_from_ncdhw(const float *, void *, void *, int64_t, int64_t, int64_t, int64_t, int64_t, float, const float *, void *);
diff --git a/snvc_amd/models/stereo_volume.py b/snvc_amd/models/stereo_volume.py
--- a/snvc_amd/models/stereo_volume.py
+++ b/snvc_amd/models/stereo_volume.py
@@ -73,6 +73,8 @@
     def last_first_layer(self) -> torch.Tensor:
         ws = self.__dict__.get("_snvc_ws", {})
         which = self.__dict__.get("_snvc_last_v1", "v1")
+        if which == "v1s_lazy":
+            return ops.from_split(ws[("v1s_lazy", (), None)](), self.__dict__["_snvc_x3"]["exp"]["v1"])
         for k, v in ws.items():
             if k[0] == which:
                 return ops.from_split(v, self.__dict__["_snvc_x3"]["exp"]["v1"]) if which == "v1s" else v
@@ -95,6 +97,7 @@
 
     arithmetic = "auto"
     stream_out = False
+    fused_first = True
     split_prep = True
     fused_tail = True
 
@@ -161,14 +164,23 @@
             return None
         return st if self.split_guard(device, mode) is not None else None
 
-    def _tail_x3(self, st, v1s, timing=None):
+    def _tail_x3(self, st, v1s, timing=None, fused=None):
         L, A, E, flag = st["layers"], st["affine"], st["exp"], st["flag"]
-        n, dev = v1s.size(0), v1s.device
-        d, h, w = v1s.shape[3:6]
+        if fused is not None:
+            (n, _, d, h, w), dev = fused[0], fused[1]
+        else:
+            n, dev = v1s.size(0), v1s.device
+            d, h, w = v1s.shape[3:6]
         hg = self.hg_conv3d
         _mark(timing, "conv2", 0)
-        v2s, hv = L["conv2"](v1s, E["v1"], *A["conv2"], flags=EPI_RELU, out_exp=E["conv2"], head=self.classifier.weight, overflow=flag,
-                             out=self._buffer("v2s", (n, 2, 4, d, h, w, 8), dev, torch.float16))
+        v2_out = self._buffer("v2s", (n, 2, 4, d, h, w, 8), dev, torch.float16)
+        if fused is not None:
+            v2s, hv = L["conv2"].forward_fused_first(n=n, in_sp=(d, h, w), x_exp=E["v1"], scale=A["conv2"][0], bias=A["conv2"][1], flags=EPI_RELU,
+                                                     out_exp=E["conv2"], head=self.classifier.weight, overflow=flag, out=v2_out, **fused[2])
+            _ROUTES["fused_first_conv"] += 1
+        else:
+            v2s, hv = L["conv2"](v1s, E["v1"], *A["conv2"], flags=EPI_RELU, out_exp=E["conv2"], head=self.classifier.weight, overflow=flag,
+                                 out=v2_out)
         _mark(timing, "conv2", 1)
         _ROUTES["side_head"] += 1
         o = L["h1"](v2s, E["conv2"], *A["h1"], flags=EPI_RELU, out_exp=E["h1"], overflow=flag)
@@ -612,8 +624,15 @@
             lx = plans.get("left2d_x3")
             if lx is None:
                 lx = plans["left2d_x3"] = ops.Conv2dLayerX3(self._left_planes_weight(w.detach()[:, :c]))
-            planes = ops.conv2d_x3_from_f32(left, [lx], prep_ws.setdefault("planes", {}))[0]
+            st_f = self._x3_select(left.device, arithmetic)
+            fuse = bool(self.fused_first and sheared and conv.out_channels == c and isinstance(bn, nn.BatchNorm3d) and left.size(0) > 0
+                        and st_f["layers"]["conv2"].fused_first_form(left.size(0), (shift.size(1),) + tuple(left.shape[2:])))
+            if fuse:
+                planes, p_il = ops.planes_x3_il(left, lx, prep_ws.setdefault("planes_il", {}))
+            else:
+                planes = ops.conv2d_x3_from_f32(left, [lx], prep_ws.setdefault("planes", {}))[0]
         else:
+            fuse = False
             planes = self._left_planes_layer(plans, w.detach()[:, :c])(left.unsqueeze(2))
         planes = planes.view(left.size(0), c, 3, left.size(2), left.size(3))
         shape = (left.size(0), c, shift.size(1)) + tuple(left.shape[2:])
@@ -622,14 +641,20 @@
             off, wu, off_col, wu_col = sheared_geometry(q, m0, shift.size(1), left.size(3))
             if split_prep:
                 lx_g, lx_col = self._sheared_layers_x3(plans, w.detach()[:, c:], q)
+                if fuse and q in (1, 2):
+                    pitch, lp = ops.fused_il_geometry(q, m0, shift.size(1), left.size(3), wu, off, wu_col, off_col)
+                    g, gcol, gi = ops.sheared_prep_x3_il(right, q, wu, off, wu_col, off_col, lx_g, lx_col, prep_ws.setdefault("sheared_il", {}),
+                                                         pitch, lp)
+                    _ROUTES["sheared_prep_x3"] += 1
+                    return g, gcol, off, off_col, (gi, pitch, lp)
                 g, gcol = ops.sheared_prep_x3(right, q, wu, off, wu_col, off_col, lx_g, lx_col, prep_ws.setdefault("sheared", {}))
                 _ROUTES["sheared_prep_x3"] += 1
-                return g, gcol, off, off_col
+                return g, gcol, off, off_col, None
             lay_g, lay_col = self._sheared_layers(plans, w.detach()[:, c:], q)
             if not self.prep_streams:
                 g = lay_g(ops.sheared_upsample(right, q, wu, off).unsqueeze(2)).squeeze(2)
                 gcol = lay_col(ops.sheared_upsample(right, q, wu_col, off_col).unsqueeze(2)).squeeze(2)
-                return g, gcol, off, off_col
+                return g, gcol, off, off_col, None
             cur = torch.cuda.current_stream(left.device)
             s1, s2 = self._side_streams(left.device)
             start = torch.cuda.Event()
@@ -645,7 +670,7 @@
                 out.append((t, done))
             for _, done in out:
                 cur.wait_event(done)
-            return out[0][0], out[1][0], off, off_col
+            return out[0][0], out[1][0], off, off_col, None
 
         def commuted_inputs():
             if split_prep and (9 * conv.out_channels) % 32 == 0:
@@ -690,10 +715,25 @@
             if ready is None or tuple(guess[:2]) != tuple(structure):
                 _mark(timing, "volume", 0)
                 ready = sheared_inputs(q, m0)
-            g, gcol, off, off_col = ready
+            g, gcol, off, off_col, il = ready
             _mark(timing, "volume", 1)
             _mark(timing, "conv1", 0)
             st = self._x3_select(left.device, arithmetic)
+            if st is not None and il is not None:
+                _mark(timing, "conv1", 1)
+                _ROUTES["sheared_first_conv"] += 1
+                v1_sc, v1_bi = self._x3_v1_affine(st, scale, bias)
+
+                def expand():
+                    t = self._buffer("v1s", (shape[0], 2, c // 8) + tuple(shape[2:]) + (8,), left.device, torch.float16)
+                    ops.sheared_expand_split(g, gcol, planes, v1_sc, v1_bi, t, q, m0, off, off_col, ops.EPI_RELU, None)
+                    return t
+                self.__dict__["_snvc_ws"] = self.__dict__.get("_snvc_ws", {})
+                self.__dict__["_snvc_ws"][("v1s_lazy", (), None)] = expand
+                self.__dict__["_snvc_last_v1"] = "v1s_lazy"
+                return self._tail_x3(st, None, timing, fused=(shape, left.device, dict(
+                    gi=il[0], pitch=il[1], lp=il[2], p_il=p_il, v_scale=v1_sc, v_bias=v1_bi, q=q, m0=m0, off=off, off_col=off_col,
+                    v_flags=ops.EPI_RELU)))
             if st is not None and c % 8 == 0:
                 v1s = self._buffer("v1s", (shape[0], 2, c // 8) + tuple(shape[2:]) + (8,), left.device, torch.float16)
                 try:
diff --git a/snvc_amd/ops.py b/snvc_amd/ops.py
--- a/snvc_amd/ops.py
+++ b/snvc_amd/ops.py
@@ -7,7 +7,7 @@
 
 import torch
 
-from . import _derived, _lib
+from . import _derived, _fused, _lib
 from ._lib import (EPI_ADD_POST, EPI_ADD_PRE, EPI_RELU, EPI_SIGMOID, EPI_STREAM_OUT, F32, F64, Conv3dDesc,
                    Unsupported, check)
 
@@ -1422,6 +1422,62 @@
                                                     ws["c_mul"], ws["c_y"], _ptr(ws["split"]), _ptr(scratch), _ptr(ws["mul"]), _stream(x)),
               "snvc_f16x3_conv2d_from_f32")
     return ws["y"]
+
+
+
+def il_index(mode: int, oc: int, c: int, h_dim: int, pitch: int, lp: int, cls0: int, h: int, x: int) -> int:
+    return int(_fused.lib().snvc_fused_il_index(mode, oc, c, h_dim, pitch, lp, cls0, h, x))
+
+
+def fused_il_geometry(q: int, m0: int, d: int, w: int, wu: int, off: int, wu_col: int, off_col: int):
+    lo = min(0, q * (w - 1) - (d - 1) - m0 + off_col, -(d - 1) - m0 + off if w > 1 else 0)
+    hi = max(wu - 1, wu_col - 1, q * (w - 1) - m0 + off_col, q * (w - 2) - m0 + off if w > 1 else 0)
+    return hi - lo + 1, -lo
+
+
+def sheared_prep_x3_il(right, q: int, wu: int, off: int, wu_col: int, off_col: int, lay_g: "Conv2dLayerX3", lay_col: "Conv2dLayerX3", ws: dict,
+                       pitch: int, lp: int):
+    _gpu(right, "right")
+    right = right.contiguous()
+    n, c, h, w = right.shape
+    key = (n, c, h, w, wu, wu_col, pitch, lp, right.device)
+    if ws.get("key") != key:
+        dev = right.device
+        ws.clear()
+        ws.update(key=key, rq=torch.empty(n * 2 * c * h * wu, dtype=torch.float16, device=dev),
+                  rq2=torch.empty(n * 2 * c * h * wu_col, dtype=torch.float16, device=dev), mul=torch.empty(1, dtype=torch.float32, device=dev),
+                  g=torch.empty((n, lay_g.cout, h, wu), dtype=torch.float32, device=dev),
+                  gcol=torch.empty((n, lay_col.cout, h, wu_col), dtype=torch.float32, device=dev),
+                  gi=torch.zeros((n, 6, c // 8, h, pitch, 8), dtype=torch.float32, device=dev))
+    scratch = _scale_scratch(right.device)
+    with torch.cuda.device(right.device):
+        check(_fused.lib().snvc_fused_sheared_prep_x3(_ptr(right), n, c, h, w, int(q), int(wu), int(off), int(wu_col), int(off_col),
+                                                      _ptr(lay_g.packed), _ptr(lay_col.packed), lay_g.cout, float(2.0 ** -lay_g.w_exp),
+                                                      float(2.0 ** -lay_col.w_exp), _ptr(ws["rq"]), _ptr(ws["rq2"]), _ptr(scratch), _ptr(ws["mul"]),
+                                                      _ptr(ws["g"]), _ptr(ws["gcol"]), _ptr(ws["gi"]), int(pitch), int(lp), _stream(right)),
+              "snvc_fused_sheared_prep_x3")
+    return ws["g"], ws["gcol"], ws["gi"]
+
+
+def planes_x3_il(x, layer: "Conv2dLayerX3", ws: dict):
+    _gpu(x, "x")
+    x = x.contiguous()
+    if x.dtype != torch.float32 or x.dim() != 4:
+        raise RuntimeError("planes_x3_il needs a float32 [N,C,H,W] tensor")
+    n, c, h, w = x.shape
+    key = (n, c, h, w, id(layer), "il", x.device)
+    if ws.get("key") != key:
+        ws.clear()
+        ws.update(key=key, split=torch.empty(n * 2 * c * h * w, dtype=torch.float16, device=x.device),
+                  mul=torch.empty(1, dtype=torch.float32, device=x.device),
+                  y=[torch.empty((n, layer.cout, h, w), dtype=torch.float32, device=x.device)],
+                  p_il=torch.empty((n, 3, c // 8, h, w, 8), dtype=torch.float32, device=x.device), layers=[layer])
+    scratch = _scale_scratch(x.device)
+    with torch.cuda.device(x.device):
+        check(_fused.lib().snvc_fused_planes_from_f32(_ptr(x), n, c, h, w, _ptr(layer.packed), layer.cout, float(2.0 ** -layer.w_exp),
+                                                      _ptr(ws["y"][0]), _ptr(ws["p_il"]), _ptr(ws["split"]), _ptr(scratch), _ptr(ws["mul"]),
+                                                      _stream(x)), "snvc_fused_planes_from_f32")
+    return ws["y"][0], ws["p_il"]
 
 
 def from_split(x: torch.Tensor, exp: int = 0, channels: Optional[int] = None) -> torch.Tensor:
@@ -1593,6 +1649,37 @@
             return out_f32
         return (out, y_head) if head is not None else out
 
+    def fused_first_form(self, n: int, sp) -> bool:
+        return (self.ksize == 3 and self.stride == 1 and not self.transposed and self.w_mul_dev is None and self.cin % 8 == 0
+                and x3_form(self.cout, 3, 1, self.dilation, False, n, tuple(sp), True, False, self.forced_algo) == _lib.ALGO_X3_Q16)
+
+    def forward_fused_first(self, gi, pitch: int, lp: int, p_il, v_scale, v_bias, q: int, m0: int, off: int, off_col: int, v_flags: int,
+                            n: int, in_sp, x_exp: int = 0, scale=None, bias=None, flags: int = 0, out=None, out_exp: int = 0, head=None,
+                            overflow=None):
+        in_sp = tuple(int(v) for v in in_sp)
+        if not self.fused_first_form(n, in_sp):
+            raise Unsupported("forward_fused_first: the layer does not run on the 16x16x32 form at this size")
+        algo = self.algo = _lib.ALGO_X3_Q16
+        packed = self._pack(algo)
+        out_sp = self.out_spatial(in_sp)
+        out = _result(out, (n, 2, self.cout // 8) + out_sp + (8,), torch.float16, gi.device,
+                      "conv3d `out` must be a split C8 tensor of the output shape", _split_check)
+        y_head = None
+        if head is not None:
+            head = head.detach().reshape(-1).float().contiguous()
+            y_head = torch.empty((n, 1) + out_sp, dtype=torch.float32, device=gi.device)
+        sc, bi = self.folded(scale, bias, x_exp, out_exp)
+        if n == 0:
+            return (out, y_head) if head is not None else out
+        d = self._desc(n, in_sp, flags, algo, 0, _batch_stride(out), 0)
+        with torch.cuda.device(gi.device):
+            check(_fused.lib().snvc_fused_first_conv3d_forward(ctypes.byref(d), _ptr(packed), _ptr(sc), _ptr(bi), _ptr(out), _lo_ptr(out),
+                                                               _ptr(head), _ptr(y_head), float(2.0 ** -out_exp), _ptr(overflow), _ptr(gi),
+                                                               int(pitch), int(lp), _ptr(p_il), _ptr(v_scale), _ptr(v_bias), int(q), int(m0),
+                                                               int(off), int(off_col), int(v_flags), _stream(gi)),
+                  "snvc_fused_first_conv3d_forward")
+        return (out, y_head) if head is not None else out
+
     def forward_f32(self, x, x_mul_dev, residual_f32: Optional[torch.Tensor] = None, relu: bool = False):
         _split_check(x, "x")
         if self.w_mul_dev is None or x.size(2) * 8 != self.cin:
```

Result: faster. 533.4, median of 6 (+3.5%).
